# dryman/HashMergeJoin

Measured on AMD Instinct MI355X. Metric: probe-side tuples/s + achieved HBM GB/s, |R|=|S|=2^28 u64 keys, higher is better.
Workload: dtype u64

## Files before the change

hashmergejoin_amd/__init__.py:

```python
from ._lib import (HMJ_BUILD_ANTI, HMJ_BUILD_OUTER, HMJ_BUILD_SEMI, HMJ_CHECKSUM, HMJ_COLS_HASHED, HMJ_COLS_NO_ROW, HMJ_COLS_PACKED, HMJ_FIRST_WINS, HMJ_FULL_OUTER, HMJ_JOIN_ANTI, HMJ_JOIN_INNER, HMJ_JOIN_PROBE_OUTER, HMJ_JOIN_SEMI, HMJ_KIND_BUILD_SIDE, HMJ_KIND_PROBE_SIDE, HMJ_MATERIALIZE, HMJ_ORDERED, HMJ_PATH_CHUNKED_BUILD, HMJ_PATH_DENSE_BUILD,
                   HMJ_PATH_EXACT, HMJ_PATH_GLOBAL_TABLE, HMJ_PATH_HOST_PIPELINE, HMJ_PATH_HOT_KEY_HINT, HMJ_PATH_LOOKBACK_TIMEOUT, HMJ_PATH_ORDER_BY_KEY, HMJ_PATH_ORDER_BY_RANK_SORT, HMJ_PATH_ORDER_DEFERRED, HMJ_PATH_ORDERED_EXPANSION, HMJ_PATH_LDS_TABLE,
                   HMJ_PATH_KEY_RANGES, HMJ_PATH_PREPARED, HMJ_PATH_PRESORTED, HMJ_PATH_RANK_RUNS, HMJ_PATH_SORT_MSD, HMJ_PATH_SLAB, HMJ_PATH_SLAB_ONE_PASS, HMJ_PATH_SLAB_PROBE, HMJ_PATH_SORTED_FK, HMJ_PATH_SORTED_FK_HALF, HMJ_PATH_SORTED_FK_WIDE, HMJ_PATH_SORTED_WRITE, HMJ_PATH_SPLIT, HMJ_PATH_UNIQ_WRITE, HMJ_PATH_WINDOW,
                   HMJ_KEY_FIXED, HMJ_KEY_LARGE_STRING, HMJ_MAX_KEY_COLS, HMJ_MAX_TAKE_COLS, HMJ_STR_NO_ROW, HMJ_SUM_PROBE, HMJ_TAKE_NO_ROW, BuildJoinOpts, ColsJoinOpts, ColsKindOpts, ColsRel, ColsResult, ExchangeKindOpts, HmjError, JoinOpts, JoinResult, KeyCol, KindCounts, MixedCol, MixedOpts, MixedRel, StrJoinOpts, StrKindOpts, StrRel, StrResult, TakeDst, TakeOpts, TakeSrc, TakeStrDst, TakeStrOpts, TakeStrSrc, Timing, Validity,
                   lib_path, load_library)
from .join import Executor, HashMergeJoin, cols_key64, mixed_key64, pack_strings, pack_validity, plan, unpack_strings, unpack_validity

__all__ = ["Executor", "HashMergeJoin", "plan", "HmjError", "JoinResult", "Timing", "load_library",
           "lib_path", "HMJ_MATERIALIZE", "HMJ_ORDERED", "HMJ_FIRST_WINS", "HMJ_CHECKSUM",
           "HMJ_SUM_PROBE", "JoinOpts", "HMJ_JOIN_INNER", "HMJ_JOIN_SEMI", "HMJ_JOIN_ANTI", "HMJ_JOIN_PROBE_OUTER",
           "BuildJoinOpts", "HMJ_BUILD_SEMI", "HMJ_BUILD_ANTI", "HMJ_BUILD_OUTER", "HMJ_FULL_OUTER",
           "ExchangeKindOpts", "KindCounts", "HMJ_KIND_PROBE_SIDE", "HMJ_KIND_BUILD_SIDE",
           "pack_strings", "StrRel", "StrJoinOpts", "StrResult", "StrKindOpts", "HMJ_STR_NO_ROW",
           "KeyCol", "ColsRel", "ColsJoinOpts", "ColsResult", "HMJ_COLS_PACKED", "HMJ_COLS_HASHED", "HMJ_MAX_KEY_COLS",
           "cols_key64", "ColsKindOpts", "HMJ_COLS_NO_ROW", "Validity", "pack_validity",
           "TakeSrc", "TakeDst", "TakeOpts", "HMJ_TAKE_NO_ROW", "HMJ_MAX_TAKE_COLS", "unpack_validity",
           "TakeStrSrc", "TakeStrDst", "TakeStrOpts", "unpack_strings",
           "MixedCol", "MixedRel", "MixedOpts", "HMJ_KEY_FIXED", "HMJ_KEY_LARGE_STRING", "mixed_key64"]
```

hashmergejoin_amd/_lib.py:

```python
import ctypes as C
import os

HMJ_MATERIALIZE = 0x01
HMJ_ORDERED = 0x02
HMJ_FIRST_WINS = 0x04
HMJ_CHECKSUM = 0x08
HMJ_SUM_PROBE = 0x10
HMJ_E_RCCL, HMJ_E_PEER, HMJ_E_TIMEOUT = -6, -7, -8
HMJ_PATH_SLAB, HMJ_PATH_EXACT, HMJ_PATH_UNIQ_WRITE, HMJ_PATH_SPLIT, HMJ_PATH_WINDOW = 0x1, 0x2, 0x4, 0x8, 0x10
HMJ_PATH_ORDER_DEFERRED, HMJ_PATH_ORDER_BY_KEY, HMJ_PATH_PREPARED, HMJ_PATH_CHUNKED_BUILD = 0x20, 0x40, 0x80, 0x100
HMJ_PATH_HOT_KEY_HINT = 0x200
HMJ_PATH_SLAB_PROBE = 0x400
HMJ_PATH_SORTED_WRITE = 0x800
HMJ_PATH_SORTED_FK = 0x1000
HMJ_PATH_DENSE_BUILD = 0x2000
HMJ_PATH_GLOBAL_TABLE = 0x100000
HMJ_PATH_ORDER_BY_RANK_SORT = 0x200000
HMJ_PATH_ORDERED_EXPANSION = 0x400000
HMJ_PATH_LDS_TABLE = 0x800000
HMJ_PATH_RANK_RUNS = 0x1000000
HMJ_PATH_RANK_LOOKUP_IN_PASS = 0x2000000
HMJ_PATH_SORT_MSD = 0x4000000
HMJ_PATH_KEY_RANGES = 0x8000000
HMJ_PATH_SLAB_ONE_PASS = 0x80000
HMJ_PATH_HOST_PIPELINE = 0x4000
HMJ_PATH_SORTED_FK_HALF = 0x8000
HMJ_PATH_LOOKBACK_TIMEOUT = 0x10000
HMJ_PATH_SORTED_FK_WIDE = 0x20000
HMJ_PATH_PRESORTED = 0x40000

_HERE = os.path.dirname(os.path.abspath(__file__))
_U64P = C.POINTER(C.c_uint64)


class HmjError(RuntimeError):
    def __init__(self, code, msg):
        super().__init__("hmj error %d: %s" % (code, msg))
        self.code = code


class JoinResult(C.Structure):
    _fields_ = [("n_matches", C.c_uint64), ("sum_r", C.c_uint64), ("sum_s", C.c_uint64),
                ("xor_fold", C.c_uint64), ("mix_sum", C.c_uint64), ("sum_probe_all", C.c_uint64),
                ("key", C.c_void_p), ("rval", C.c_void_p), ("sval", C.c_void_p)]

    def checks(self):
        return {k: int(getattr(self, k)) for k in ("n_matches", "sum_r", "sum_s", "xor_fold", "mix_sum")}


HMJ_JOIN_INNER, HMJ_JOIN_SEMI, HMJ_JOIN_ANTI, HMJ_JOIN_PROBE_OUTER = 0, 1, 2, 3


class JoinOpts(C.Structure):
    _fields_ = [("struct_size", C.c_uint32), ("kind", C.c_uint32), ("outer_fill", C.c_uint64),
                ("n_probe_matched", C.c_uint64), ("n_probe_unmatched", C.c_uint64)]


HMJ_BUILD_SEMI, HMJ_BUILD_ANTI, HMJ_BUILD_OUTER, HMJ_FULL_OUTER = 1, 2, 3, 4


class BuildJoinOpts(C.Structure):
    _fields_ = [("struct_size", C.c_uint32), ("kind", C.c_uint32), ("build_fill", C.c_uint64), ("probe_fill", C.c_uint64),
# ... 150 lines not shown
                ("radix_bits", C.c_int), ("radix_passes", C.c_int),
                ("n_scatter_launches", C.c_int), ("n_split_retries", C.c_int),
                ("bytes_scatter", C.c_uint64), ("bytes_hist", C.c_uint64),
                ("bytes_probe_count", C.c_uint64), ("bytes_probe_write", C.c_uint64),
                ("path", C.c_uint32), ("key_prefix_bits", C.c_int32), ("key_window_low", C.c_int32),
                ("n_probe_items", C.c_uint32), ("ms_scatter_pass0", C.c_float), ("ms_scatter_pass1", C.c_float)]

    def as_dict(self):
        return {n: getattr(self, n) for n, _ in self._fields_}


class PlanDesc(C.Structure):
    _fields_ = [("struct_size", C.c_uint32), ("path", C.c_uint32), ("radix_bits", C.c_int32), ("radix_passes", C.c_int32),
                ("pass_bits", C.c_int32 * 4), ("key_prefix_bits", C.c_int32), ("key_window_low", C.c_int32),
                ("n_partitions", C.c_uint32), ("probe_items", C.c_uint32), ("attempts", C.c_uint32), ("refused", C.c_uint32),
                ("cooling", C.c_uint32), ("workload", C.c_uint64)]

    def as_dict(self):
        d = {n: getattr(self, n) for n, _ in self._fields_}
        d["pass_bits"] = list(self.pass_bits)
        return d


HMJ_REFUSED_GTABLE_SHAPE, HMJ_REFUSED_GTABLE_COOLING, HMJ_REFUSED_GTABLE_GAVE_UP = 0x1, 0x2, 0x4
HMJ_REFUSED_RANK_SORT_MODEL, HMJ_REFUSED_RANK_SORT_COOLING, HMJ_REFUSED_RANK_SORT_GAVE_UP = 0x8, 0x10, 0x20
HMJ_REFUSED_SLAB_SHAPE, HMJ_REFUSED_SLAB_COOLING, HMJ_REFUSED_SLAB_SORTED_INPUT, HMJ_REFUSED_SLAB_OVERFLOW = 0x40, 0x80, 0x100, 0x200
HMJ_REFUSED_FAST_WRITE_COOLING, HMJ_REFUSED_FAST_WRITE_GAVE_UP = 0x400, 0x800
HMJ_REFUSED_SLAB_PROBE_COOLING, HMJ_REFUSED_SLAB_PROBE_OVERFLOW = 0x1000, 0x2000
HMJ_REFUSED_PREFIX_VIOLATED, HMJ_REFUSED_EXPANSION_GAVE_UP = 0x4000, 0x8000
HMJ_COOL_UNIQ_WRITE, HMJ_COOL_SORTED_WRITE, HMJ_COOL_GTABLE, HMJ_COOL_GTABLE_WRITE = 0x1, 0x2, 0x4, 0x8
HMJ_COOL_RANK_SORT, HMJ_COOL_RANK_SORT_SLAB, HMJ_COOL_EXPANSION, HMJ_COOL_SORT_SLAB = 0x10, 0x20, 0x40, 0x80
HMJ_COOL_SLAB, HMJ_COOL_SLAB_PROBE, HMJ_COOL_ONE_PASS_WRITE, HMJ_COOL_EXACT_PREFIX = 0x100, 0x200, 0x400, 0x800
HMJ_COOL_RANK_RUNS = 0x1000


class PlaceInfo(C.Structure):
    _fields_ = [("name", C.c_char * 16), ("bytes", C.c_uint64), ("fill_TBps", C.c_float), ("candidates", C.c_int),
                ("ms_search", C.c_float), ("searched", C.c_int), ("aborted", C.c_int), ("budget_ms", C.c_float),
                ("cand_ms_alloc", C.c_float * 4), ("cand_ms_fill", C.c_float * 4), ("cand_TBps", C.c_float * 4)]


def lib_path():
    return os.environ.get("HMJ_LIB") or os.path.join(_HERE, "libhmj_hip.so")


class ExchangeInfo(C.Structure):
    _fields_ = [("n_ranks", C.c_int), ("owner_mode", C.c_int), ("rounds_build", C.c_uint32), ("rounds_probe", C.c_uint32),
                ("recv_build", C.c_uint64), ("recv_probe", C.c_uint64), ("ms_split", C.c_float),
                ("ms_exchange_build", C.c_float), ("ms_exchange_probe", C.c_float), ("ms_local", C.c_float),
                ("ms_total", C.c_float), ("digit_bits", C.c_int32), ("digit_low", C.c_int32), ("n_subjoins", C.c_uint32),
                ("fallback", C.c_uint32), ("sample_max_share", C.c_float), ("ms_kernels", C.c_float),
                ("ms_exposed", C.c_float)]

    def as_dict(self):
        return {n: getattr(self, n) for n, _ in self._fields_}


HMJ_MAX_RANKS, HMJ_MAX_ROUNDS = 16, 16


class DigitPlan(C.Structure):
    _fields_ = [("usable", C.c_int32), ("digit_bits", C.c_int32), ("digit_low", C.c_int32), ("n_rounds", C.c_uint32),
                ("owner_first", C.c_uint32 * (HMJ_MAX_RANKS + 1)),
                ("round_first", (C.c_uint32 * (HMJ_MAX_ROUNDS + 1)) * HMJ_MAX_RANKS), ("max_share", C.c_float)]


# ... 149 lines not shown
```

hashmergejoin_amd/csrc/api.hip:

```cpp
#include <hip/hip_runtime.h>
#include <sys/mman.h>

#include <algorithm>
#include <cstdio>
#include <cstdlib>
#include <chrono>
#include <cmath>
#include <cstring>
#include <mutex>
#include <string>
#include <thread>
#include <vector>

#include "hmj_ctx.h"

using hmj::u32;
using hmj::u64;
using namespace hmj_host;

namespace hmj_host {

constexpr int kMaxEvents = 1024;

int fail(hmj_ctx* c, int code, const char* what, hipError_t e) {
// ... 29 lines not shown
  acc->ms_scatter_pass[0] += t.ms_scatter_pass[0];
  acc->ms_scatter_pass[1] += t.ms_scatter_pass[1];
  if (t.radix_passes) {
    acc->radix_bits = t.radix_bits;
    acc->radix_passes = t.radix_passes;
    acc->key_prefix_bits = t.key_prefix_bits;
    acc->key_window_low = t.key_window_low;
  }
  acc->n_probe_items += t.n_probe_items;
}

static int ilog2_u64(uint64_t v) { return v ? 63 - __builtin_clzll(v) : 0; }
uint64_t workload_signature(uint64_t n_build, uint64_t n_probe, uint32_t flags, int kind) {
  const uint32_t mode = ((flags & HMJ_ORDERED) ? 4u : 0u) | ((flags & (HMJ_MATERIALIZE | HMJ_ORDERED)) ? 2u : 0u) |
                        ((flags & HMJ_FIRST_WINS) ? 1u : 0u);
  return ((uint64_t)(kind & 31) << 20) | ((uint64_t)mode << 16) | ((uint64_t)ilog2_u64(n_build) << 8) | (uint64_t)ilog2_u64(n_probe);
}
WorkloadMemo* memo_for(hmj_ctx* c, uint64_t sig) {
  auto it = c->memos.find(sig);
  if (it == c->memos.end()) {
    if (c->memos.size() >= 1024) c->memos.clear();
    it = c->memos.emplace(sig, c->memo_init).first;
  }
  c->wm = &it->second;
  c->wm_sig = sig;
  return c->wm;
}
uint32_t WorkloadMemo::cooling() const {
  return (uniq_cooldown ? HMJ_COOL_UNIQ_WRITE : 0u) | (sorted_cooldown ? HMJ_COOL_SORTED_WRITE : 0u) | (gtable_cooldown ? HMJ_COOL_GTABLE : 0u) |
         (gtable_write_cooldown ? HMJ_COOL_GTABLE_WRITE : 0u) | (gtable_sort_cooldown ? HMJ_COOL_RANK_SORT : 0u) |
         (gtable_sort_slab_cooldown ? HMJ_COOL_RANK_SORT_SLAB : 0u) | (expand_cooldown ? HMJ_COOL_EXPANSION : 0u) |
         (sort_slab_cooldown ? HMJ_COOL_SORT_SLAB : 0u) | (slab_cooldown ? HMJ_COOL_SLAB : 0u) | (slab_probe_cooldown ? HMJ_COOL_SLAB_PROBE : 0u) |
         (one_pass_write_cooldown ? HMJ_COOL_ONE_PASS_WRITE : 0u) | (exact_prefix_joins ? HMJ_COOL_EXACT_PREFIX : 0u) |
         (rank_runs_cooldown ? HMJ_COOL_RANK_RUNS : 0u) | (sort_msd_cooldown ? HMJ_COOL_SORT_MSD : 0u);
}

int wait_arrival(hmj_ctx* c, hipEvent_t ev) {
  if (c->arrive_wait) return c->arrive_wait(c, ev);
  HIP_TRY(hipStreamWaitEvent(c->stream, ev, 0));
  return HMJ_OK;
}

int ensure_dev(hmj_ctx* c, DevBuf& b, size_t bytes) {
  if (bytes <= b.cap) return HMJ_OK;
  if (c && (&b == &c->rbuf[0] || &b == &c->rbuf[1] || &b == &c->r_off || &b == &c->slab_br || &b == &c->cnt_br))
    c->prep.valid = false;
  if (b.p) {
    hipError_t e = hipFree(b.p);
    b.p = nullptr;
    b.cap = 0;
    if (e != hipSuccess) return fail(c, HMJ_E_HIP, "hipFree", e);
  }
  size_t want = bytes + (bytes >> 4) + 256;
#ifdef HMJ_DEV
  if (const char* e = getenv("HMJ_ALLOC_PAD_KB")) want += (size_t)atoll(e) << 10;
  if (const char* e = getenv("HMJ_ALLOC_ROUND_MB")) {
    const size_t g = (size_t)atoll(e) << 20;
    if (g) want = (want + g - 1) / g * g;
  }
#endif
  const auto t_alloc0 = std::chrono::steady_clock::now();
  hipError_t e = hipMalloc(&b.p, want);
  if (e != hipSuccess) {
    b.p = nullptr;
    (void)hipGetLastError();
    return fail(c, HMJ_E_OOM, "hipMalloc", e);
  }
// ... 357 lines not shown
      size_t it = 0;
      for (size_t ci = t; ci < nchunks; ci += T, it++) {
        const int slot = (int)(it & 1);
        hipEvent_t ev = c->up_events[2 * t + slot];
        char* pin = static_cast<char*>(c->up_slots[2 * t + slot].p);
        if (it >= 2 && hipEventSynchronize(ev) != hipSuccess) { status[t] = 1; return; }
        const size_t off = ci * kUpChunk, len = (bytes - off < kUpChunk) ? bytes - off : kUpChunk;
        std::memcpy(pin, static_cast<const char*>(src_host) + off, len);
        if (hipMemcpyAsync(static_cast<char*>(dst_dev) + off, pin, len, hipMemcpyHostToDevice, st) != hipSuccess ||
            hipEventRecord(ev, st) != hipSuccess) { status[t] = 1; return; }
      }
      if (hipStreamSynchronize(st) != hipSuccess) status[t] = 1;
    });
  }
  for (auto& x : th) x.join();
  for (int t = 0; t < T; t++)
    if (status[t]) return fail(c, HMJ_E_HIP, "staged host-to-device copy failed");
  return HMJ_OK;
}

int check_rel(hmj_ctx* c, const void* p, uint64_t n, const char* name) {
  if (n > 0xFFFFFFFFull) return fail(c, HMJ_E_ARG, "more than 2^32-1 rows in one call");
  if (n && !p) return fail(c, HMJ_E_ARG, name);
  if (((uintptr_t)p & 15) != 0) return fail(c, HMJ_E_ARG, "relation pointer must be 16-byte aligned");
  return HMJ_OK;
}

constexpr int kRetryNoWinOrdered = 1003;
constexpr int kRetryNoFastWrite = 1002;
constexpr int kRetryNoSlab = 1001;
constexpr int kRetryNoSlabProbe = 1004;
constexpr int kRetryMoreBits = 1005;
constexpr int kRetryNoPrefix = 1000;

static int read_accum(hmj_ctx* c, u64** h) {
  u64* hh = (u64*)c->h_accum.p;
  HIP_TRY(hipMemcpyAsync(hh, c->accum.p, 8 * sizeof(u64), hipMemcpyDeviceToHost, c->stream));
  HIP_TRY(hipStreamSynchronize(c->stream));
  *h = hh;
  return HMJ_OK;
}
static void result_sums(hmj_result* out, const u64* h) {
  out->n_matches = h[hmj::ACC_N];
  out->sum_r = h[hmj::ACC_SUM_R];
  out->sum_s = h[hmj::ACC_SUM_S];
  out->xor_fold = h[hmj::ACC_XOR];
  out->mix_sum = h[hmj::ACC_MIX];
  out->sum_probe_all = h[hmj::ACC_SUM_P];
}

static int deliver_columns(hmj_ctx* c, hmj_result* out, bool to_host, const void* key, const void* rval, const void* sval,
                           size_t bytes, bool sync_always) {
  if (to_host) {
    RC_TRY(ensure_host(c, c->h_key, bytes, false));
    if (rval) RC_TRY(ensure_host(c, c->h_rval, bytes, false));
    if (sval) RC_TRY(ensure_host(c, c->h_sval, bytes, false));
    const int s = span_begin(c, K_D2H, -1);
    HIP_TRY(hipMemcpyAsync(c->h_key.p, key, bytes, hipMemcpyDeviceToHost, c->stream));
    if (rval) HIP_TRY(hipMemcpyAsync(c->h_rval.p, rval, bytes, hipMemcpyDeviceToHost, c->stream));
    if (sval) HIP_TRY(hipMemcpyAsync(c->h_sval.p, sval, bytes, hipMemcpyDeviceToHost, c->stream));
    span_end(c, s);
  }
  if (to_host || sync_always) HIP_TRY(hipStreamSynchronize(c->stream));
  out->key = (const uint64_t*)(to_host ? c->h_key.p : key);
  out->rval = rval ? (const uint64_t*)(to_host ? c->h_rval.p : rval) : nullptr;
  out->sval = sval ? (const uint64_t*)(to_host ? c->h_sval.p : sval) : nullptr;
// ... 623 lines not shown

static int run_slab_join(hmj_ctx* c, const JoinCall& j, const JoinPlan& p) {
  const bool materialize = j.materialize(), first = j.first(), extra = j.extra();
  const u32 nb = j.nb, np = j.np, np_plan = p.np_plan, P = p.P;
  const int* pass_bits = p.pass_bits;
  hmj::SlabGeom gr, gs;
  if (p.allow_slab && c->slab_mode && c->wm->slab_cooldown == 0 && !c->prepare_only && !(c->timing.path & HMJ_PATH_SLAB) &&
      !((!materialize || p.fast_write) && p.Q == 1 && p.probe_fits && p.passes == 2 && pass_bits[0] <= hmj::SLAB_MAX_BITS &&
        pass_bits[1] <= hmj::SLAB_MAX_BITS && p.dense_scale <= 2.5))
    c->plan.refused |= HMJ_REFUSED_SLAB_SHAPE;
  if (!(p.allow_slab && c->slab_mode && c->wm->slab_cooldown == 0 && (!materialize || p.fast_write) && p.Q == 1 &&
        p.probe_fits &&
        p.passes == 2 && pass_bits[0] <= hmj::SLAB_MAX_BITS && pass_bits[1] <= hmj::SLAB_MAX_BITS &&
        slab_sizes_ok(c, nb, np_plan, materialize || np_plan < nb) &&
        p.dense_scale <= 2.5 &&
        hmj::slab_geometry(nb, pass_bits[0], pass_bits[1], &gr, 0, 1.0, p.dense_scale) &&
        hmj::slab_geometry(np_plan, pass_bits[0], pass_bits[1], &gs, 0,
                           (nb && np_plan > nb) ? (double)np_plan / (double)nb : 1.0, p.dense_scale)))
    return kPlanNotTaken;
  const bool reuse = c->prep.valid && c->prep.slab && c->prep.ptr == j.R && c->prep.n == nb &&
                     c->prep.low == p.low && c->prep.B == p.B;
  c->prep.valid = false;
  c->timing.path |= HMJ_PATH_SLAB | (reuse ? HMJ_PATH_PREPARED : 0u);
  c->timing.n_probe_items = P;
  const int ba = pass_bits[0], bb = pass_bits[1];
  const u64 rows_a = gr.rows_a > gs.rows_a ? gr.rows_a : gs.rows_a;
  const u32 wa = gr.WA > gs.WA ? gr.WA : gs.WA;
  RC_TRY(ensure_dev(c, c->slab_a, rows_a * 16));
  RC_TRY(ensure_dev(c, c->cnt_a, ((size_t)wa << ba) * 4));
  RC_TRY(ensure_dev(c, c->slab_br, gr.rows_b * 16));
  RC_TRY(ensure_dev(c, c->slab_bs, gs.rows_b * 16));
  RC_TRY(ensure_dev(c, c->cnt_br, (size_t)P * gr.KB * 4));
  RC_TRY(ensure_dev(c, c->cnt_bs, (size_t)P * gs.KB * 4));
  if (!reuse) RC_TRY(slab_passes(c, j.R, nb, 0, p.low, ba, bb, gr, c->slab_br, c->cnt_br, false));
  if (!c->prepare_only) RC_TRY(slab_passes(c, j.S, np, 1, p.low, ba, bb, gs, c->slab_bs, c->cnt_bs, !c->arrive_ev.empty()));
  u64* hh;
  if (c->prepare_only) {
    RC_TRY(read_accum(c, &hh));
    if (hh[hmj::ACC_ERR] & hmj::ERR_SLAB) {
      c->wm->slab_cooldown = 8;
      return kRetryNoSlab;
    }
    c->prep.valid = true;
    c->prep.slab = true;
    c->prep.ptr = j.R;
    c->prep.n = nb;
    c->prep.low = p.low;
    c->prep.B = p.B;
    return HMJ_OK;
  }
  hmj::ProbeArgs sa = slab_probe_args(c, &gr, nullptr, c->slab_bs, c->cnt_bs, gs.CB, P, 1);
  if (p.fast_write)
    return unique_key_write(c, sa, true, nb, np, p.low, extra, p.verify_pfx ? p.prefix : 0, p.pfx_ref, j.ordered(), j.to_host,
                            p.fk_wide_plan, p.dense_scale, j.out);
#ifdef HMJ_DEV
  sa.debug = c->dev_ablate;
#endif
  int sp = span_begin(c, K_PROBE_COUNT, -1);
  if (first || extra) {
    sa.extra = (extra ? 1u : 0u) | (first ? 2u : 0u);
    HIP_TRY(hmj::launch_probe_count_ext(sa, nullptr, nullptr, true, c->num_cus, c->stream));
  } else {
    HIP_TRY(hmj::launch_probe_count_slab(sa, c->num_cus, c->stream));
  }
  span_end(c, sp);
  c->timing.bytes_probe_count = 16ull * ((u64)nb + np);
  RC_TRY(read_accum(c, &hh));
// ... 1170 lines not shown
  p.path = c->timing.path;
  p.radix_bits = c->timing.radix_bits;
  p.radix_passes = c->timing.radix_passes;
  p.key_prefix_bits = c->timing.key_prefix_bits;
  p.key_window_low = c->timing.key_window_low;
  p.n_partitions = (c->timing.path & (HMJ_PATH_GLOBAL_TABLE | HMJ_PATH_LDS_TABLE)) ? 0u : (p.radix_bits < 32 ? 1u << p.radix_bits : 0u);
  p.probe_items = c->timing.n_probe_items;
  p.cooling = c->wm->cooling();
  p.workload = c->wm_sig;
  return rc;
}
static int join_device_planned(hmj_ctx* c, const void* R, uint64_t n_build, const void* S, uint64_t n_probe, uint32_t flags,
                               hmj_result* out, bool to_host) {
  const bool kinds = c->join_kind != 0;
  if (!kinds) {
    bool done = false;
    int rc = try_global_table(c, R, n_build, S, n_probe, flags, out, to_host, &done);
    if (rc != HMJ_OK || done) return rc;
    rc = try_small_build_ordered(c, R, n_build, S, n_probe, flags, out, to_host, &done);
    if (rc != HMJ_OK || done) return rc;
  }
  bool auto_prefix = true, slab = !kinds, fast_write = !kinds, win_ordered = true, prefix_unsafe = false, slab_probe = !kinds;
  if ((flags & HMJ_ORDERED) && c->wm->exact_prefix_joins > 0) {
    c->wm->exact_prefix_joins--;
    prefix_unsafe = true;
  }
  bool forced_here = false;
  struct Unforce {
    hmj_ctx* c;
    bool* on;
    ~Unforce() {
      if (*on) c->force_bits = -1;
      c->expand_allow_rebits = true;
    }
  } unforce{c, &forced_here};
  for (int attempt = 0; attempt < 8; attempt++) {
    c->plan.attempts = (uint32_t)attempt + 1;
    int rc = join_device_impl(c, R, n_build, S, n_probe, flags, out, to_host, auto_prefix, slab, fast_write,
                              win_ordered, prefix_unsafe, slab_probe);
    c->plan.refused |= rc == kRetryNoSlab ? HMJ_REFUSED_SLAB_OVERFLOW : rc == kRetryNoPrefix ? HMJ_REFUSED_PREFIX_VIOLATED
                       : rc == kRetryNoFastWrite ? HMJ_REFUSED_FAST_WRITE_GAVE_UP : rc == kRetryNoSlabProbe ? HMJ_REFUSED_SLAB_PROBE_OVERFLOW
                       : rc == kRetryMoreBits ? HMJ_REFUSED_EXPANSION_GAVE_UP : 0u;
    if (c->trace)
      std::fprintf(stderr, "[hmj] join nb=%llu np=%llu flags=%#x attempt %d: rc=%d bits=%d passes=%d path=%#x prefix=%d low=%d items=%u%s\n",
                   (unsigned long long)n_build, (unsigned long long)n_probe, flags, attempt, rc, c->timing.radix_bits,
                   c->timing.radix_passes, c->timing.path, c->timing.key_prefix_bits, c->timing.key_window_low,
                   c->timing.n_probe_items,
                   rc == kRetryNoSlab ? " -> retry without the slab path (a slab overflowed)"
                   : rc == kRetryNoPrefix ? " -> retry: a row outside the sampled key prefix"
                   : rc == kRetryNoFastWrite ? " -> retry without the unique-key write mode"
                   : rc == kRetryNoWinOrdered ? " -> retry without the key window"
                   : rc == kRetryNoSlabProbe ? " -> retry without probe-side slabs (one overflowed)"
                   : rc == kRetryMoreBits ? " -> retry with one more radix bit (a partition did not fit the ordered expansion)" : "");
    if (rc == kRetryNoSlab || rc == kRetryNoPrefix || rc == kRetryNoFastWrite || rc == kRetryNoWinOrdered || rc == kRetryNoSlabProbe ||
        rc == kRetryMoreBits) {
      std::vector<Span> keep;
      for (const Span& sp : c->spans)
        if (sp.kind == K_TOTAL || sp.kind == K_H2D) keep.push_back(sp);
      c->spans.swap(keep);
      std::memset(&c->timing, 0, sizeof(c->timing));
      if (rc == kRetryNoSlab) slab = false;
      else if (rc == kRetryMoreBits) {
        c->force_bits = c->expand_rebits;
        c->expand_allow_rebits = false;
        forced_here = true;
      }
      else if (rc == kRetryNoSlabProbe) slab_probe = false;
      else if (rc == kRetryNoFastWrite) fast_write = false;
      else if (rc == kRetryNoWinOrdered) win_ordered = false;
      else if (!prefix_unsafe && win_ordered) {
        prefix_unsafe = true;
        c->wm->exact_prefix_joins = 32;
      }
      else auto_prefix = false;
      continue;
    }
    return rc;
  }
  return fail(c, HMJ_E_HIP, "join could not be planned");
}

int prepare_build(hmj_ctx* c, const void* R, uint64_t n_build, uint64_t n_probe_hint) {
  hmj_result dummy;
  c->prepare_only = true;
  c->probe_hint = n_probe_hint;
  c->prep.valid = false;
  const int rc = join_device(c, R, n_build, nullptr, 0, 0, &dummy, false);
  c->prepare_only = false;
  return rc;
}

int join_device_kind(hmj_ctx* c, const JoinKind& k, const void* R, uint64_t n_build, const void* S, uint64_t n_probe,
                     uint32_t flags, hmj_result* out, hmj_kind_counts* counts) {
  std::memset(counts, 0, sizeof(*counts));
// ... 16 lines not shown
    const u64 unmatched = k.kind == HMJ_JOIN_SEMI ? n_probe - out->n_matches : filled;
    counts->n_probe_matched = n_probe - unmatched;
    counts->n_probe_unmatched = unmatched;
  } else {
    const u64 b_unmatched = k.kind == HMJ_BUILD_SEMI ? n_build - swept : swept;
    counts->n_build_matched = n_build - b_unmatched;
    counts->n_build_unmatched = b_unmatched;
    if (k.kind == HMJ_FULL_OUTER) {
      counts->n_probe_matched = n_probe - filled;
      counts->n_probe_unmatched = filled;
    }
  }
  return HMJ_OK;
}

}

extern "C" {

int hmj_create(hmj_ctx** out, int device_id) {
  if (!out) return HMJ_E_ARG;
  *out = nullptr;
  int ndev = 0;
  if (hipGetDeviceCount(&ndev) != hipSuccess || ndev <= 0) {
    (void)hipGetLastError();
    return HMJ_E_NODEV;
  }
  if (device_id < 0 && hipGetDevice(&device_id) != hipSuccess) return HMJ_E_NODEV;
  if (device_id >= ndev) return HMJ_E_ARG;
  if (hipSetDevice(device_id) != hipSuccess) return HMJ_E_NODEV;
  hmj_ctx* c = new hmj_ctx();
  c->device = device_id;
  if (const char* e = getenv("HMJ_SLAB")) c->slab_mode = atoi(e);
  if (const char* e = getenv("HMJ_ONE_PASS_SLAB")) c->one_pass_slab = atoi(e) != 0;
  if (const char* e = getenv("HMJ_GTABLE")) c->gtable_mode = atoi(e) != 0;
  if (const char* e = getenv("HMJ_RANK_RUNS")) c->rank_runs_mode = atoi(e) != 0;
  if (const char* e = getenv("HMJ_RANK_RUNS_MAX_CUT")) c->rank_runs_max_cut = atoi(e) < 0 ? 0 : atoi(e) > 16 ? 16 : atoi(e);
  if (const char* e = getenv("HMJ_RANK_RUNS_MAX_GROUP")) c->rank_runs_max_group = atoi(e) < 0 ? 0 : atoi(e) > 4 ? 4 : atoi(e);
  if (const char* e = getenv("HMJ_PROMOTE_TO_ORDERED")) c->promote_to_ordered = atoi(e) != 0;
  if (const char* e = getenv("HMJ_KEY_RANGES")) c->key_ranges = atoi(e) != 0;
  if (const char* e = getenv("HMJ_KEY_RANGES_FORCE")) c->key_ranges_force = atoi(e) < 0 ? 0 : atoi(e) > 4 ? 4 : atoi(e);
  if (const char* e = getenv("HMJ_RANK_RUNS_WAVE")) c->rank_runs_wave = atoi(e) != 0;
  if (const char* e = getenv("HMJ_RANK_RUNS_MAX_LEVEL")) c->rank_runs_max_level = atoi(e) < 0 ? 0 : atoi(e) > 2 ? 2 : atoi(e);
  if (const char* e = getenv("HMJ_GTABLE_SORT")) c->gtable_sort_mode = atoi(e) != 0;
  if (const char* e = getenv("HMJ_EXPAND_FK_FANOUT")) c->expand_fk_fanout = atoi(e) > 0 ? (u32)atoi(e) : 0u;
  if (const char* e = getenv("HMJ_SORT_MSD")) c->sort_msd = atoi(e) != 0;
  if (const char* e = getenv("HMJ_SORT_MSD_MEAN")) c->sort_msd_mean = atof(e) >= 64.0 ? atof(e) : c->sort_msd_mean;
  if (const char* e = getenv("HMJ_SORT_MSD_MAX_BITS")) c->sort_msd_max_bits = atoi(e) < 2 ? 2 : atoi(e) > 18 ? 18 : atoi(e);
  if (const char* e = getenv("HMJ_SORT_MSD_MIN_LOG2")) {
    const int l = atoi(e);
    if (l >= 16 && l <= 32) c->sort_msd_min = 1ull << l;
  }
  if (const char* e = getenv("HMJ_SORT_SLAB_MIN_LOG2")) {
    const int l = atoi(e);
    if (l >= 12 && l <= 32) c->sort_slab_min = 1ull << l;
  }
  if (const char* e = getenv("HMJ_GTABLE_SORT_SLAB_MIN_LOG2")) {
    const int l = atoi(e);
    if (l >= 12 && l <= 32) c->gtable_sort_slab_min = 1ull << l;
  }
  if (const char* e = getenv("HMJ_GTABLE_SORT_FANOUT")) c->gtable_sort_fanout = atoi(e) > 0 ? (u32)atoi(e) : 1u;
  if (const char* e = getenv("HMJ_PLACE")) {
    c->place_tune = atoi(e) != 0;
    if (atoi(e) > 0) {
      c->place_tries = atoi(e);
      c->place_search_always = true;
// ... 858 lines not shown
```

hashmergejoin_amd/csrc/hmj_ctx.h:

```cpp
#pragma once
#include <hip/hip_runtime.h>

#include <string>
#include <unordered_map>
#include <vector>

#include "../../include/hmj.h"
#include "hmj_dev.h"
#include "hmj_launch.h"

struct hmj_comm;

namespace hmj_host {

struct DevBuf {
  void* p = nullptr;
  size_t cap = 0;
};
struct HostBuf {
  void* p = nullptr;
  size_t cap = 0;
  bool pinned = true;
};

// ... 15 lines not shown
    for (DevBuf* b : {&rows_r, &rows_s, &flags, &blk, &blk_off, &list, &runs, &acc, &mark_r, &mark_s, &amb, &cmp_r, &cmp_s, &vblk}) f(*b);
    each_result_buf(f);
  }
};

enum Kind {
  K_TOTAL = 0, K_H2D, K_D2H, K_HIST, K_SCAN, K_SCATTER, K_OFFSETS, K_PROBE_COUNT, K_OUT_SCAN,
  K_PROBE_WRITE, K_ORDER, K_NKINDS
};
struct Span {
  int kind, rel, e0, e1;
  int pass;
};

struct WorkloadMemo {
  int uniq_cooldown = 0;
  int sorted_cooldown = 0;
  bool sorted_chained = false;
  bool sorted_wide = true;
  bool sorted_fk = false;
  int sorted_fk_age = 0;
  int gtable_cooldown = 0;
  int gtable_write_cooldown = 0;
  int gtable_sort_cooldown = 0;
  int gtable_sort_slab_cooldown = 0;
  int rank_runs_cooldown = 0;
  int rank_lookup_cooldown = 0;
  int expand_cooldown = 0;
  int sort_slab_cooldown = 0;
  int sort_msd_cooldown = 0;
  int slab_cooldown = 0;
  int slab_probe_cooldown = 0;
  int one_pass_write_cooldown = 0;
  int exact_prefix_joins = 0;
  uint32_t cooling() const;
};

}

namespace hmj_host {
struct OrderedCostModel {
  double part_fixed_ms = 0.15;
  double part_ns = 0.030, part_ns_per_f = 0.00023;
  double part_bucket_ns = 0.043, part_bucket_ns_per_f = 0.0001;
  double part_epilogue_ns = 0.25;
  double comp_fixed_ms = 0.65;
  double comp_ns_chain = 0.060, comp_ns_exact = 0.072;
  double comp_ns_wide = 0.145;
  double comp_ns_beyond_l2 = 0.02;
  double runs_fixed_ms = 0.25, runs_ns = 0.0215, runs_ns_per_run = 7.5;
  double runs_ns_per_log2_build = 0.0023;
  double runs_wave_ns_per_run = 1.2, runs_wave_ns = 0.007;
  double runs_range_ns = 0.0;
};
}

struct hmj_ctx {
  using DevBuf = hmj_host::DevBuf;
  using HostBuf = hmj_host::HostBuf;
  using Span = hmj_host::Span;
  using WorkloadMemo = hmj_host::WorkloadMemo;
  using u32 = hmj::u32;
  using u64 = hmj::u64;
  int device = 0, num_cus = 256;
  hipStream_t own_stream = nullptr, stream = nullptr;
  DevBuf rbuf[2], sbuf[2], in_r, in_s, hist, totals, r_off, s_off, part_count, part_out_off, accum,
// ... 54 lines not shown
  uint64_t gtable_max_rows = 1ull << 17;
  u32 gtable_min_fanout = 0;
  uint64_t gtable_min_probe = 1;
  int gtable_wg_per_cu = 8;
  u32 gtable_slots_per_row = 16;
  int gtable_max_log_cap = 18;
  bool ltable_mode = true;
  bool gtable_sort_mode = true;
  u32 gtable_sort_fanout = 128;
  bool rank_runs_mode = true;
  int rank_runs_max_cut = 10;
  int rank_runs_max_group = 3;
  int rank_runs_max_level = 2;
  uint64_t big_join_rows = 1ull << 29;
  bool promote_to_ordered = true;
  bool key_ranges = true;
  int key_ranges_force = 0;
  bool rank_runs_wave = true;
  bool build_sort_msd = true;
  bool gtable_sort_slab = true;
  u64 gtable_sort_slab_min = 1ull << 25;
  bool expand_mode = true;
  u32 fk_payload_buckets = 24;
  u32 expand_fk_fanout = 0;
  bool expand_allow_rebits = true;
  int expand_rebits = 0;
  bool sort_msd = true;
  double sort_msd_mean = 1200.0;
  int sort_msd_max_bits = 18;
  u64 sort_msd_min = 1ull << 22;
  bool sort_slab = true;
  u64 sort_slab_min = 1ull << 25;
  int slab_mode = 1;
  bool staged_upload = false;
  bool host_pipeline = true;
  hipStream_t copy_stream = nullptr;
  std::vector<hipEvent_t> copy_ev;
  bool split_mode = true;
  bool window_mode = true;
  u32 slab_min_rows = 1u << 21;
  u32 slab_probe_kb = 0;
  bool one_pass_slab = true;
  int scatter_variant = 1;
  bool profiling = false;
  bool trace = false;
#ifdef HMJ_DEV
  u32 dev_ablate = 0;
#endif
  std::vector<hipEvent_t> events;
  std::vector<Span> spans;
  int ev_used = 0;
  hmj_timing timing;
  std::string last_error;
  hmj_comm* comm = nullptr;
  std::vector<u64> arrive_rows;
  std::vector<hipEvent_t> arrive_ev;
  bool sample_build_only = false;
  int (*arrive_wait)(hmj_ctx*, hipEvent_t) = nullptr;
};


namespace hmj_host {
int fail(hmj_ctx* c, int code, const char* what, hipError_t e = hipSuccess);
#define HIP_TRY(expr)                                                        \
  do {                                                                       \
    hipError_t _e = (expr);                                                  \
// ... 38 lines not shown
```

hashmergejoin_amd/csrc/hmj_dev.h:

```cpp
#pragma once
#include <hip/hip_runtime.h>
#include <stdint.h>

namespace hmj {

typedef unsigned long long u64;
typedef unsigned int u32;
typedef unsigned short u16;

struct __attribute__((aligned(16))) Tup {
  u64 key;
  u64 val;
};

constexpr int kWave = 64;
#ifndef HMJ_SCAN_DPP
#define HMJ_SCAN_DPP 1
#endif

#ifndef HMJ_STREAM_POLICY
#define HMJ_STREAM_POLICY 2
#endif
typedef u64 u64x2_t __attribute__((ext_vector_type(2)));
__device__ __forceinline__ void store_stream(Tup* p, const Tup& v) {
// ... 51 lines not shown
          slot[r] = (slot[r] + 1) & mask;
          any_live = true;
        }
      }
    }
  }
}

constexpr int RP_THREADS = 512;
constexpr int RP_WAVES = RP_THREADS / kWave;
constexpr int RP_ITEMS = 8;
constexpr int RP_TILE = RP_THREADS * RP_ITEMS;
constexpr int RP_MAX_BITS = 9;
constexpr int RP_MAXD = 1 << RP_MAX_BITS;
constexpr int RP_MAX_BLOCKS = 2048;

constexpr int PB_THREADS = 1024;
constexpr int PB_CAP = 5120;
constexpr int PB_LOG_NB = 12;
constexpr int PB_TARGET_AVG = 4096;
constexpr int PB_PLAN_SLACK = 256;

constexpr int SLAB_KB = 4;
constexpr int SLAB_MAX_BITS = 9;

enum { ACC_N = 0, ACC_SUM_R, ACC_SUM_S, ACC_XOR, ACC_MIX, ACC_SUM_P, ACC_ERR, ACC_PAD };
constexpr u64 ERR_SLAB = 2;
constexpr u64 ERR_ORDER_DEFER = 16;
constexpr u64 ERR_ORDER_FAIL = 32;
constexpr u64 ERR_SORTED = 64;
constexpr u64 ERR_FASTPATH = 8;
constexpr u64 ERR_GTABLE = 128;
constexpr u64 ERR_PREFIX = 4;

__device__ __forceinline__ u64 mix64(u64 x) {
  x ^= x >> 30;
  x *= 0xBF58476D1CE4E5B9ull;
  x ^= x >> 27;
  x *= 0x94D049BB133111EBull;
  x ^= x >> 31;
  return x;
}

__device__ __forceinline__ u64 tmix(u64 key, u64 rval, u64 sval) {
  u64 t = mix64(key);
  t = mix64(t ^ rval);
  t = mix64(t + sval);
  return t;
}

__device__ __forceinline__ int lane_id() {
  return __builtin_amdgcn_mbcnt_hi(~0u, __builtin_amdgcn_mbcnt_lo(~0u, 0u));
}

__device__ __forceinline__ u32 popc_below(u64 m) {
  return __builtin_amdgcn_mbcnt_hi((u32)(m >> 32), __builtin_amdgcn_mbcnt_lo((u32)m, 0u));
}

__device__ __forceinline__ u32 wave_incl_scan_u32(u32 v, int ) {
#if HMJ_SCAN_DPP
  v += (u32)__builtin_amdgcn_update_dpp(0, (int)v, 0x111, 0xF, 0xF, false);
  v += (u32)__builtin_amdgcn_update_dpp(0, (int)v, 0x112, 0xF, 0xF, false);
  v += (u32)__builtin_amdgcn_update_dpp(0, (int)v, 0x114, 0xF, 0xF, false);
  v += (u32)__builtin_amdgcn_update_dpp(0, (int)v, 0x118, 0xF, 0xF, false);
  v += (u32)__builtin_amdgcn_update_dpp(0, (int)v, 0x142, 0xA, 0xF, false);
  v += (u32)__builtin_amdgcn_update_dpp(0, (int)v, 0x143, 0xC, 0xF, false);
// ... 72 lines not shown
```

hashmergejoin_amd/csrc/hmj_launch.h:

```cpp
#pragma once
#include <hip/hip_runtime.h>
#include <stddef.h>
#include <stdint.h>

#include <atomic>

namespace hmj {
typedef unsigned long long u64;
typedef unsigned int u32;

struct SmemAttrOnce {
  std::atomic<unsigned long long> devices{0};
};
inline hipError_t ensure_max_smem(SmemAttrOnce& once, const void* kernel, size_t bytes) {
  int dev = 0;
  hipError_t e = hipGetDevice(&dev);
  if (e != hipSuccess) return e;
  const unsigned long long bit = 1ull << (dev & 63);
  if (dev < 64 && (once.devices.load(std::memory_order_acquire) & bit)) return hipSuccess;
  e = hipFuncSetAttribute(kernel, hipFuncAttributeMaxDynamicSharedMemorySize, (int)bytes);
  if (e != hipSuccess) return e;
  if (dev < 64) once.devices.fetch_or(bit, std::memory_order_release);
  return hipSuccess;
}

constexpr int kMaxRanks = 16;
struct OwnerFn {
  u32 mode;
  u32 G;
  u64 spl[kMaxRanks - 1];
};
int radix_tile_rows(int bits, int variant);
void radix_pass_geometry(u32 n, int tile, u32* nblk, u32* rows_per_block);
size_t radix_scatter_smem_bytes();
hipError_t launch_radix_hist(const void* in, u32 n, int tile, int shift, int bits, u32* hist,
                             u32 nblk, u32 rows_per_block, hipStream_t st, const OwnerFn* own = nullptr);
hipError_t launch_owner_scatter(const void* in, void* out, u32 n, int bits, const OwnerFn& own,
                                const u32* hist_scanned, const u32* totals, u32 nblk, u32 rows_per_block,
                                u64* offsets_out, hipStream_t st);
hipError_t launch_radix_rowscan(u32* hist, u32 nblk, int bits, u32* totals, hipStream_t st);
hipError_t launch_radix_scatter(const void* in, void* out, u32 n, int variant, int shift, int bits,
                                const u32* hist_scanned, const u32* totals, u32 nblk,
                                u32 rows_per_block, u64* offsets_out, hipStream_t st);
struct SlabGeom {
  u32 WA, rpw, CA, CB, KB;
  u64 rows_a, rows_b;
};
bool slab_geometry(u32 n, int bits_a, int bits_b, SlabGeom* g, u32 kb = 0, double fan = 1.0, double density = 1.0);
bool slab_geometry_one_pass(u32 n, int bits, double keys_per_digit, u32 max_workers, SlabGeom* g, double density = 1.0);
u32 slab_capacity(double mean, double fan);
hipError_t launch_slab_a(const void* in, u32 n, int shift, int bits, const SlabGeom& g, void* slab_a, u64 slab_a_rows,
                         u32* cnt_a, u64 cnt_a_n, u64* accum, hipStream_t st, u32 w_begin = 0, u32 w_end = 0xFFFFFFFFu);
hipError_t launch_slab_b(const void* slab_a, const u32* cnt_a, int bits_a, int shift, int bits,
                         const SlabGeom& g, void* slab_b, u64 slab_b_rows, u32* cnt_b, u64 cnt_b_n, u64* accum, hipStream_t st);
hipError_t launch_key_sample(const void* R, u32 nb, const void* S, u32 np, u64* out, hipStream_t st);
hipError_t launch_key_exact(const void* R, u32 nb, const void* S, u32 np, u64 ref, u64* out, int num_cus, hipStream_t st,
                            bool ref_is_first_key = false);
hipError_t launch_check_partitioned(const void* a, u32 n, int low, int bits, u32* flag, int num_cus, hipStream_t st);
hipError_t launch_part_offsets(const void* a, u32 n, int low, int bits, u32* off, hipStream_t st);

struct ProbeArgs {
  const void* R;
  const u32* r_off;
  const void* S;
  const u32* s_off;
  u32 P;
  u32 Q;
  u64* part_count;
  const u64* part_out_off;
  u64* out_key;
  u64* out_rval;
  u64* out_sval;
  u64 out_cap;
  u64* accum;
  const u32* item_list;
  const u32* n_item_list;
  const u32* r_cnt;
  const u32* s_cnt;
  u32 r_cap, s_cap;
  u32 s_wa, s_ppi;
  u64 r_cnt_n, s_cnt_n;
  u64 r_rows, s_rows;
  const u64* item_base;
  const u32* r_end;
  const u32* s_end;
  u32 extra;
  u32 pfx_shift;
  u64 pfx_val;
  u32* matched;
  u32 debug;
};
hipError_t launch_probe(const ProbeArgs& a, int mode, bool first_wins, bool extra, int grid,
                        hipStream_t st);
int probe_default_grid(int num_cus);
hipError_t launch_probe_kind(const ProbeArgs& a, int mode, int kind, bool first_wins, u64 fill, int grid, hipStream_t st);
hipError_t launch_probe_build_kind(const ProbeArgs& a, int mode, int kind, u64 fill, u32* bmark, int grid, hipStream_t st);
hipError_t launch_build_sweep(const ProbeArgs& a, const u32* r_off, u32 P, const u32* vstart, u64* sweep_n, int mode,
                              bool set, u64 fill, int num_cus, hipStream_t st);
hipError_t launch_probe_count_ext(const ProbeArgs& a, u32* irregular, u32* n_irregular, bool slab,
                                  int num_cus, hipStream_t st);
hipError_t launch_probe_count_slab(const ProbeArgs& a, int num_cus, hipStream_t st);
hipError_t launch_probe_write_sorted(const ProbeArgs& a, bool slab, bool fk, int shape, u64* lookback, bool chained, int key_low,
                                     int num_cus, hipStream_t st);
hipError_t launch_probe_write_uniq(const ProbeArgs& a, bool slab, int num_cus, hipStream_t st);
hipError_t launch_slab_np(const u32* cnt, u32 P, u64* out, hipStream_t st);
hipError_t launch_probe_count_fast(const ProbeArgs& a, u32* irregular, u32* n_irregular, bool big,
                                   bool per_partition_counts, int num_cus, hipStream_t st);
hipError_t launch_scan_u64(const u64* in, u64* out_excl, u32 n, hipStream_t st);
hipError_t launch_probe_expand_ordered(const ProbeArgs& a, int key_low, int num_cus, hipStream_t st);
hipError_t launch_order(const u64* part_out_off, const u32* vstart, const u32* in_base32, const u64* in_base64, u32 P, u32 Q,
                        int low, const u64* akey, const u64* arval, const u64* asval, u64* bkey, u64* brval,
                        u64* bsval, u64* accum, u32 defer_rows, bool many_per_key, int grid, hipStream_t st);
hipError_t launch_compact(const u64* part_out_off, const u32* in_base32, const u64* in_base64, u32 P, const u64* akey,
                          const u64* arval, const u64* asval, u64* bkey, u64* brval, u64* bsval, int grid, hipStream_t st);
hipError_t launch_rekey(void* pairs, u64 n, const u64* col, hipStream_t st);

hipError_t launch_gtable_build(const void* R, u32 nb, void* tab, int log_cap, u64* accum, bool first, int num_cus,
                               hipStream_t st);
hipError_t launch_gtable_probe(const void* S, u32 np, const void* tab, int log_cap, const void* R, u64* accum, bool first,
                               bool extra, int num_cus, int wg_per_cu, hipStream_t st);
hipError_t launch_gtable_write(const void* S, u32 np, const void* tab, int log_cap, const void* R, u64* accum, u64* out_key,
                               u64* out_rval, u64* out_sval, bool first, bool extra, int num_cus, int wg_per_cu, hipStream_t st);

hipError_t launch_ltable_probe(const void* R, u32 nb, const void* S, u32 np, u64* accum, bool first, bool extra, int num_cus, hipStream_t st);
int ltable_max_rows();
hipError_t launch_sval_range(const void* S, u32 np, u64* out2 , int num_cus, hipStream_t st,
                             u32 every = 1 );
hipError_t launch_gtable_emit(const void* S, u32 np, const void* tab, int log_cap, u64 svmin, int range_bits, u64* accum,
                              void* pairs, bool extra, bool wide, int num_cus, int wg_per_cu, hipStream_t st);
hipError_t launch_gtable_swap(const void* in, void* out, u64 n, int num_cus, hipStream_t st);
hipError_t launch_gtable_emit_ranks(const void* S, u32 np, const void* tab, int log_cap, u64* accum, void* pairs, bool extra, int num_cus,
                                    int wg_per_cu, hipStream_t st);
int rank_sort_max_run(int level = 0);
hipError_t launch_sort_runs_write(const void* slabs, const u32* cnt, u32 cap, u32 P, const u64* out_off, void* out, u64* accum, int level,
// ... 36 lines not shown
```

hashmergejoin_amd/csrc/probe.hip:

```cpp
#include "hmj_dev.h"
#include "hmj_launch.h"
#include <type_traits>

namespace hmj {

constexpr u32 PB_NB = 1u << PB_LOG_NB;
constexpr u32 NIL = 0xFFFFu;
static_assert(PB_CAP < 0xFFFF, "chain links are 16-bit");

struct ProbeSmem {
  u64 key[PB_CAP];
  u64 val[PB_CAP];
  u32 head[PB_NB];
  u32 aux[PB_CAP];
  u16 next[PB_CAP];
  u32 scratch[PB_THREADS / kWave + 1];
  u64 pcount;
  u64 red[8];
  u64 obase;
  u32 wtot[PB_THREADS / kWave];
  u32 nslot;
};
constexpr u32 PB_BATCH = 2 * PB_THREADS;
static_assert(PB_BATCH <= PB_CAP, "a batch must fit an empty table");
// ... 860 lines not shown
};

template <int LOG_NB>
__device__ __forceinline__ u32 fast_hash(u64 k) {
  u32 x = (u32)k ^ ((u32)(k >> 32) * 0x85EBCA6Bu);
  x *= 0x9E3779B1u;
  return x >> (32 - LOG_NB);
}

template <int THREADS, int ROWS = FP_ROWS>
__device__ __forceinline__ void fp_load(Tup (&t)[ROWS], const Tup* __restrict__ base, u32 n,
                                        int tid) {
#pragma unroll
  for (int k = 0; k < ROWS; k++) {
    u32 i = k * THREADS + tid;
    t[k] = base[i < n ? i : n - 1];
  }
}

static_assert(SLAB_KB == 4, "fp_load_slab / fp_load_pieces / slab_np_kernel unroll exactly four pieces per partition");
template <int THREADS, int ROWS = FP_ROWS>
__device__ __forceinline__ void fp_load_slab(Tup (&t)[ROWS], const Tup* __restrict__ base, u32 cap,
                                             u32 p1, u32 p2, u32 p3, u32 n, int tid) {
#pragma unroll
  for (int k = 0; k < ROWS; k++) {
    u32 i = k * THREADS + tid;
    i = i < n ? i : n - 1;
    const u32 j = (i >= p1) + (i >= p2) + (i >= p3);
    const u32 pre = j == 0 ? 0u : (j == 1 ? p1 : (j == 2 ? p2 : p3));
    t[k] = base[(u64)j * cap + (i - pre)];
  }
}

template <int THREADS>
__device__ __forceinline__ void fp_load_pieces(Tup (&t)[FP_ROWS], const Tup* __restrict__ base, u32 cap, u32 cnt_mine, int tid) {
  constexpr int QT = THREADS / 4;
  const u32 g = (u32)tid / QT, l = (u32)tid % QT;
  const Tup* __restrict__ piece = base + (u64)g * cap;
  const u32 last = cnt_mine ? cnt_mine - 1 : 0;
#pragma unroll
  for (int k = 0; k < FP_ROWS; k++) {
    const u32 r = l + (u32)k * QT;
    t[k] = piece[r < last ? r : last];
  }
}

template <int THREADS, int LOG_NB, bool PCOUNT, bool SLAB, int OUT>
__global__ __launch_bounds__(THREADS, 4) void probe_count_fast_kernel(
    ProbeArgs a, u32* __restrict__ irregular, u32* __restrict__ n_irregular) {
  typedef FastSmem<THREADS, LOG_NB> Smem;
  constexpr u32 CAP = Smem::CAP, NB = 1u << LOG_NB;
  constexpr bool PIECES = SLAB && OUT == 0 && !PCOUNT && HMJ_PROBE_PIECES;
  constexpr u32 QT = THREADS / 4, PIECE_CAP = FP_ROWS * QT;
  extern __shared__ __attribute__((aligned(16))) unsigned char smem_raw[];
  Smem& sm = *reinterpret_cast<Smem*>(smem_raw);
  const Tup* __restrict__ R = static_cast<const Tup*>(a.R);
  const Tup* __restrict__ S = static_cast<const Tup*>(a.S);
  const u32* __restrict__ r_off = a.r_off;
  const u32* __restrict__ s_off = a.s_off;
  const u32* __restrict__ r_end = (SLAB || a.r_end == nullptr) ? a.r_off + 1 : a.r_end;
  const u32* __restrict__ s_end = (SLAB || a.s_end == nullptr) ? a.s_off + 1 : a.s_end;
  const u32 P = a.P;
  const int tid = threadIdx.x;
  u64 acc_n = 0, acc_r = 0, acc_s = 0, acc_x = 0, acc_m = 0, acc_p = 0;
  bool pfx_bad = false, giveup = false;
  for (u32 i = tid; i < NB; i += THREADS) sm.head[i] = 0;
  if (tid < 2) sm.itemcnt[tid] = 0;
  u32 epoch = 0;
  u32 prev_p = 0xFFFFFFFFu, parity = 0;

  u32 p = blockIdx.x;
  u32 rb = 0, nb = 0, sb = 0, np = 0;
  bool regular = false;
  Tup br[FP_ROWS], pr[FP_ROWS], pq[FP_ROWS];
  u32 r1 = 0, r2 = 0, r3 = 0, s1 = 0, s2 = 0, s3 = 0, r1n = 0, r2n = 0, r3n = 0, s1n = 0, s2n = 0, s3n = 0;
  u32 rm = 0, sm_ = 0, rmn = 0, smn = 0;
  const u32 my_piece = (u32)tid / QT;
  bool slab_bad = false;
  if (p < P) {
    if (SLAB) {
      const u32* rc = a.r_cnt + (u64)p * SLAB_KB;
      const u32* sc = a.s_cnt + (u64)p * SLAB_KB;
      r1 = rc[0]; r2 = r1 + rc[1]; r3 = r2 + rc[2]; nb = r3 + rc[3];
      s1 = sc[0]; s2 = s1 + sc[1]; s3 = s2 + sc[2]; np = s3 + sc[3];
      if (nb > CAP || np > CAP) slab_bad = true;
      if (PIECES) {
        rm = my_piece == 0 ? rc[0] : my_piece == 1 ? rc[1] : my_piece == 2 ? rc[2] : rc[3];
        sm_ = my_piece == 0 ? sc[0] : my_piece == 1 ? sc[1] : my_piece == 2 ? sc[2] : sc[3];
        if (rc[0] > PIECE_CAP || rc[1] > PIECE_CAP || rc[2] > PIECE_CAP || rc[3] > PIECE_CAP || sc[0] > PIECE_CAP ||
            sc[1] > PIECE_CAP || sc[2] > PIECE_CAP || sc[3] > PIECE_CAP) {
          slab_bad = true;
          nb = CAP + 1;
        }
      }
    } else {
      rb = r_off[p]; nb = r_end[p] - rb;
      sb = s_off[p]; np = s_end[p] - sb;
    }
    regular = nb && np && nb <= CAP && np <= CAP;
    if (regular) {
      if (PIECES) {
        fp_load_pieces<THREADS>(br, R + (u64)p * SLAB_KB * a.r_cap, a.r_cap, rm, tid);
        fp_load_pieces<THREADS>(pr, S + (u64)p * SLAB_KB * a.s_cap, a.s_cap, sm_, tid);
      } else if (SLAB) {
        fp_load_slab<THREADS>(br, R + (u64)p * SLAB_KB * a.r_cap, a.r_cap, r1, r2, r3, nb, tid);
        if (OUT == 0) fp_load_slab<THREADS>(pr, S + (u64)p * SLAB_KB * a.s_cap, a.s_cap, s1, s2, s3, np, tid);
      } else {
        fp_load<THREADS>(br, R + rb, nb, tid);
        if (OUT == 0) fp_load<THREADS>(pr, S + sb, np, tid);
      }
    }
  }
  const Tup* __restrict__ dummy = reinterpret_cast<const Tup*>(a.accum);
  auto load_build = [&](Tup (&t)[FP_ROWS], bool ok, u32 pp, u32 rb_, u32 nb_, u32 q1, u32 q2, u32 q3, u32 mine) {
    if (PIECES)
      fp_load_pieces<THREADS>(t, ok ? R + (u64)pp * SLAB_KB * a.r_cap : dummy, ok ? a.r_cap : 0u, ok ? mine : 1u, tid);
    else if (SLAB)
      fp_load_slab<THREADS>(t, ok ? R + (u64)pp * SLAB_KB * a.r_cap : dummy, ok ? a.r_cap : 0u, ok ? q1 : 1u, ok ? q2 : 1u,
                            ok ? q3 : 1u, ok ? nb_ : 1u, tid);
    else
      fp_load<THREADS>(t, ok ? R + rb_ : dummy, ok ? nb_ : 1u, tid);
  };
  auto load_probe = [&](Tup (&t)[FP_ROWS], bool ok, u32 pp, u32 sb_, u32 np_, u32 q1, u32 q2, u32 q3, u32 mine) {
    if (PIECES)
      fp_load_pieces<THREADS>(t, ok ? S + (u64)pp * SLAB_KB * a.s_cap : dummy, ok ? a.s_cap : 0u, ok ? mine : 1u, tid);
    else if (SLAB)
      fp_load_slab<THREADS>(t, ok ? S + (u64)pp * SLAB_KB * a.s_cap : dummy, ok ? a.s_cap : 0u, ok ? q1 : 1u, ok ? q2 : 1u,
                            ok ? q3 : 1u, ok ? np_ : 1u, tid);
    else
      fp_load<THREADS>(t, ok ? S + sb_ : dummy, ok ? np_ : 1u, tid);
  };
  const int tid_outer = tid;
  while (p < P) {
    int tid = tid_outer;
    if constexpr (OUT != 0) asm volatile("" : "+v"(tid));
    u64 out_base = (u64)sb;
    if constexpr (OUT == 1 && SLAB) {
      const u64* ibp = a.item_base + p;
      asm volatile("s_load_dwordx2 %0, %1, 0x0\n\ts_waitcnt lgkmcnt(0)" : "=s"(out_base) : "s"(ibp) : "memory");
    }
    const u32 pn = __builtin_amdgcn_readfirstlane(p + gridDim.x);
    u32 rb2 = 0, nb2 = 0, sb2 = 0, np2 = 0;
    bool regular2 = false;
    if (pn < P) {
      if (SLAB) {
        const u32* rc = a.r_cnt + (u64)pn * SLAB_KB;
        const u32* sc = a.s_cnt + (u64)pn * SLAB_KB;
        r1n = rc[0]; r2n = r1n + rc[1]; r3n = r2n + rc[2]; nb2 = r3n + rc[3];
        s1n = sc[0]; s2n = s1n + sc[1]; s3n = s2n + sc[2]; np2 = s3n + sc[3];
        if (nb2 > CAP || np2 > CAP) slab_bad = true;
        if (PIECES) {
          rmn = my_piece == 0 ? rc[0] : my_piece == 1 ? rc[1] : my_piece == 2 ? rc[2] : rc[3];
          smn = my_piece == 0 ? sc[0] : my_piece == 1 ? sc[1] : my_piece == 2 ? sc[2] : sc[3];
          if (rc[0] > PIECE_CAP || rc[1] > PIECE_CAP || rc[2] > PIECE_CAP || rc[3] > PIECE_CAP || sc[0] > PIECE_CAP ||
              sc[1] > PIECE_CAP || sc[2] > PIECE_CAP || sc[3] > PIECE_CAP) {
            slab_bad = true;
            nb2 = CAP + 1;
          }
        }
      } else {
        rb2 = r_off[pn]; nb2 = r_end[pn] - rb2;
        sb2 = s_off[pn]; np2 = s_end[pn] - sb2;
      }
      regular2 = nb2 && np2 && nb2 <= CAP && np2 <= CAP;
    }
    if (OUT == 0) {
      load_probe(pq, regular2, pn, sb2, np2, s1n, s2n, s3n, smn);
    } else if (regular) {
      if (SLAB)
        fp_load_slab<THREADS>(pr, S + (u64)p * SLAB_KB * a.s_cap, a.s_cap, s1, s2, s3, np, tid);
      else
        fp_load<THREADS>(pr, S + sb, np, tid);
    }
    if (regular) {
      lds_barrier();
      if (PCOUNT && prev_p != 0xFFFFFFFFu && tid == 0) {
        a.part_count[prev_p] = sm.itemcnt[parity ^ 1];
        sm.itemcnt[parity ^ 1] = 0;
      }
      if (PCOUNT) prev_p = 0xFFFFFFFFu;
      epoch++;
      if (epoch == 0x10000u) {
        for (u32 i = tid; i < NB; i += THREADS) sm.head[i] = 0;
        epoch = 1;
        lds_barrier();
      }
      const u32 tag = epoch << 16;
      if (!HMJ_ABLATE(1u)) {
        u32 old[FP_ROWS];
#pragma unroll
        for (int k = 0; k < FP_ROWS; k++) {
          const u32 i = k * THREADS + tid;
          old[k] = tag | NIL;
          if (PIECES ? ((u32)tid % QT + (u32)k * QT < rm) : (i < nb)) {
            if (a.pfx_shift && (br[k].key >> a.pfx_shift) != a.pfx_val) pfx_bad = true;
            sm.key[i] = br[k].key;
            sm.val[i] = br[k].val;
            old[k] = atomicExch(&sm.head[fast_hash<LOG_NB>(br[k].key)], tag | i);
          }
        }
#pragma unroll
        for (int k = 0; k < FP_ROWS; k++) {
          const u32 i = k * THREADS + tid;
          if (PIECES ? ((u32)tid % QT + (u32)k * QT < rm) : (i < nb)) sm.next[i] = ((old[k] >> 16) == epoch) ? (u16)old[k] : (u16)NIL;
        }
      } else {
#pragma unroll
        for (int k = 0; k < FP_ROWS; k++) acc_r += br[k].key;
      }
      load_build(br, regular2, pn, rb2, nb2, r1n, r2n, r3n, rmn);
      lds_barrier();
      const u64 n_before = acc_n;
      if (!HMJ_ABLATE(1u)) {
        u32 cur[FP_ROWS];
        u32 cnt[FP_ROWS], first[FP_ROWS];
#pragma unroll
        for (int k = 0; k < FP_ROWS; k++) {
          const u32 j = k * THREADS + tid;
          cur[k] = NIL;
          cnt[k] = 0;
          first[k] = OUT == 2 ? NIL : 0;
          if (PIECES ? ((u32)tid % QT + (u32)k * QT < sm_) : (j < np)) {
            if (a.pfx_shift && (pr[k].key >> a.pfx_shift) != a.pfx_val) pfx_bad = true;
            if (OUT >= 1 && (a.extra & 1u)) acc_p += pr[k].val;
            const u32 hv = sm.head[fast_hash<LOG_NB>(pr[k].key)];
            cur[k] = ((hv >> 16) == epoch) ? (hv & 0xFFFFu) : NIL;
          }
        }
        for (; !HMJ_ABLATE(2u);) {
          bool any = false;
#pragma unroll
          for (int k = 0; k < FP_ROWS; k++) any |= (cur[k] != NIL);
          if (!__any(any)) break;
#pragma unroll
          for (int k = 0; k < FP_ROWS; k++) {
            if (cur[k] != NIL) {
              const u32 i = cur[k];
              const u64 kk = sm.key[i], vv = sm.val[i];
              cur[k] = sm.next[i];
              if (kk == pr[k].key) {
                if (OUT == 2 && (a.extra & 2u)) {
                  first[k] = i < first[k] ? i : first[k];
                } else {
                  acc_n++;
                  acc_r += vv;
                  acc_s += pr[k].val;
                  if (OUT == 1) {
                    if (cnt[k] == 0) first[k] = i;
                    cnt[k]++;
                  }
                  if (OUT >= 1 && (a.extra & 1u)) {
                    const u64 m = tmix(kk, vv, pr[k].val);
                    acc_x ^= m;
                    acc_m += m;
                  }
                }
              }
            }
          }
        }
        if (OUT == 2 && (a.extra & 2u)) {
#pragma unroll
          for (int k = 0; k < FP_ROWS; k++) {
            if (first[k] != NIL) {
              const u64 vv = sm.val[first[k]];
              acc_n++;
              acc_r += vv;
              acc_s += pr[k].val;
              if (a.extra & 1u) {
                const u64 m = tmix(pr[k].key, vv, pr[k].val);
                acc_x ^= m;
                acc_m += m;
              }
            }
          }
        }
        if (OUT == 1) {
          u64 packed = 0;
          bool cx = false;
#pragma unroll
          for (int k = 0; k < FP_ROWS; k++) {
            cx |= cnt[k] > 1;
            packed |= (u64)(cnt[k] ? 1u : 0u) << (12 * k);
          }
          const int lane = tid & 63, wv = tid >> 6;
          const bool wave_dup = __any(cx);
          u64 incl = packed;
#pragma unroll
          for (int o = 1; o < kWave; o <<= 1) {
            u64 t = __shfl_up(incl, o, kWave);
            if (lane >= o) incl += t;
          }
          if (lane == 63) {
            sm.wscan[wv] = incl;
            sm.wdup[wv] = wave_dup ? 1u : 0u;
          }
          lds_barrier();
          u64 pre = 0, tot = 0;
          u32 dup = 0;
#pragma unroll
          for (int q = 0; q < THREADS / kWave; q++) {
            const u64 ws = sm.wscan[q];
            dup |= sm.wdup[q];
            if (q < wv) pre += ws;
            tot += ws;
          }
          const u64 ex = pre + incl - packed;
          if (dup) {
            giveup = true;
          } else {
            u64 o = out_base;
            u32 total = 0;
#pragma unroll
            for (int k = 0; k < FP_ROWS; k++) {
              if (cnt[k]) {
                const u64 d = o + ((ex >> (12 * k)) & 0xFFFu);
                a.out_key[d] = pr[k].key;
                a.out_rval[d] = sm.val[first[k]];
                a.out_sval[d] = pr[k].val;
              }
              const u32 tk = (u32)((tot >> (12 * k)) & 0xFFFu);
              o += tk;
              total += tk;
            }
            if (tid == 0) a.part_count[p] = total;
          }
        }
      } else {
#pragma unroll
        for (int k = 0; k < FP_ROWS; k++) acc_r += pr[k].key;
      }
      if (PCOUNT) {
        const u32 mine = (u32)(acc_n - n_before);
        const u32 ws = (u32)wave_sum_u64(mine);
        if ((tid & 63) == 0 && ws) atomicAdd(&sm.itemcnt[parity], ws);
        prev_p = p;
        parity ^= 1;
      }
    } else {
      if ((PCOUNT || OUT == 1) && tid == 0 && !(nb && np)) a.part_count[p] = 0;
      if (OUT == 1 && nb && np) giveup = true;
      if (OUT >= 1 && (a.extra & 1u) && !nb) {
        if (SLAB) {
          const Tup* base = S + (u64)p * SLAB_KB * a.s_cap;
          for (u32 j = tid; j < np; j += THREADS) {
            const u32 pc = (j >= s1) + (j >= s2) + (j >= s3);
            const u32 pre = pc == 0 ? 0 : pc == 1 ? s1 : pc == 2 ? s2 : s3;
            acc_p += base[(u64)pc * a.s_cap + (j - pre)].val;
          }
        } else {
          for (u32 j = tid; j < np; j += THREADS) acc_p += S[sb + j].val;
        }
      }
      if (OUT != 1 && !SLAB && tid == 0 && nb && np) irregular[atomicAdd(n_irregular, 1u)] = p;
      load_build(br, regular2, pn, rb2, nb2, r1n, r2n, r3n, rmn);
    }
    if (OUT == 0) {
#pragma unroll
      for (int k = 0; k < FP_ROWS; k++) pr[k] = pq[k];
    }
    p = pn; rb = rb2; nb = nb2; sb = sb2; np = np2; regular = regular2;
    r1 = r1n; r2 = r2n; r3 = r3n; s1 = s1n; s2 = s2n; s3 = s3n;
    rm = rmn; sm_ = smn;
  }
  if (SLAB && slab_bad && tid == 0) atomicOr(&a.accum[ACC_ERR], ERR_SLAB);
  if (OUT == 1 && __any(giveup) && (tid & 63) == 0) atomicOr(&a.accum[ACC_ERR], ERR_FASTPATH);
  if (__any(pfx_bad) && (tid & 63) == 0) atomicOr(&a.accum[ACC_ERR], ERR_PREFIX);
  lds_barrier();
  if (PCOUNT && prev_p != 0xFFFFFFFFu && tid == 0) a.part_count[prev_p] = sm.itemcnt[parity ^ 1];
  if (tid < 8) sm.red[tid] = 0;
  lds_barrier();
  const u64 v[6] = {acc_n, acc_r, acc_s, acc_x, acc_m, acc_p};
  block_accumulate(sm.red, a.accum, v, 1u << ACC_XOR);
}

constexpr int SW_LOGB = 12, SW_NB = 1 << SW_LOGB, SW_MAXBUCKET = 32;
constexpr u64 LB_AGG = 1ull << 62, LB_PFX = 2ull << 62, LB_MASK = (1ull << 62) - 1;
constexpr u32 LB_SPIN_LIMIT = 1u << 22;

template <int THREADS>
struct SortedSmem {
  static constexpr int CAP = THREADS * FP_ROWS, CAPB = CAP, LOGB = SW_LOGB;
  u64 key[CAP];
  u64 val[CAP];
  u64 sval[CAP];
  u32 cnt[SW_NB];
  u16 bstart[SW_NB + 2];
  u16 perm[CAP];
  u32 mbits[2][CAP / 32];
  u32 scratch[THREADS / kWave + 1];
  u32 tick[2];
  u32 flag;
  u64 obase;
  u64 red[8];
};

constexpr int SWF_LOGB = 11, SWF_CAPB = 4608, SWF_MAXDUP = 1024;
constexpr int SWF_HALF_THREADS = 512, SWF_HALF_ROWS = 6, SWF_HALF_CAPB = 2048, SWF_HALF_LOGB = 10;
constexpr int SWF_WIDE_ROWS = 6, SWF_WIDE_CAPB = 2560;
template <int THREADS, int ROWS = FP_ROWS, int CAPB_ = SWF_CAPB, int LOGB_ = SWF_LOGB>
// ... 1094 lines not shown
      vr_beg[v] = rb + b;
      vr_end[v] = rb + e;
    }
    if (ns == 1) {
      vs_beg[v] = sb;
      vs_end[v] = sb + np;
    } else {
      const u32 step = (np + ns - 1) / ns;
      const u32 b = qs * step, e = (b + step < np) ? b + step : np;
      vs_beg[v] = sb + (b < np ? b : np);
      vs_end[v] = sb + e;
    }
  }
}
hipError_t launch_split_parts(const u32* r_off, const u32* s_off, u32 P, u32 thr_rows, u32 slice_rows, u32 build_thr,
                              u32 build_slice, u32 cap_v, u32* vstart, u32* vr_beg, u32* vr_end, u32* vs_beg,
                              u32* vs_end, u32* nv_out, hipStream_t st) {
  hipLaunchKernelGGL(split_count_kernel, dim3(1), dim3(1024), 0, st, r_off, s_off, P, thr_rows, slice_rows, build_thr,
                     build_slice, cap_v, vstart, nv_out);
  hipLaunchKernelGGL(split_fill_kernel, dim3((cap_v + 255) / 256), dim3(256), 0, st, r_off, s_off, P, thr_rows,
                     slice_rows, build_thr, build_slice, cap_v, vstart, vr_beg, vr_end, vs_beg, vs_end);
  return hipGetLastError();
}

template <int MODE, bool FIRST, bool EXTRA>
static hipError_t launch_probe_t(const ProbeArgs& a, int grid, hipStream_t st) {
  static SmemAttrOnce attr_once;
  if (hipError_t e = ensure_max_smem(attr_once, reinterpret_cast<const void*>(probe_kernel<MODE, FIRST, EXTRA>), (size_t)sizeof(ProbeSmem)); e != hipSuccess) return e;
  hipLaunchKernelGGL((probe_kernel<MODE, FIRST, EXTRA>), dim3(grid), dim3(PB_THREADS),
                     sizeof(ProbeSmem), st, a);
  return hipGetLastError();
}

template <int THREADS, int LOG_NB, bool PCOUNT, bool SLAB = false, int OUT = 0>
static hipError_t launch_fast_t(const ProbeArgs& a, u32* irregular, u32* n_irregular, int grid,
                                hipStream_t st) {
  typedef FastSmem<THREADS, LOG_NB> Smem;
  static SmemAttrOnce attr_once;
  if (hipError_t e = ensure_max_smem(attr_once, reinterpret_cast<const void*>(probe_count_fast_kernel<THREADS, LOG_NB, PCOUNT, SLAB, OUT>), (size_t)sizeof(Smem)); e != hipSuccess) return e;
  if ((u32)grid > a.P) grid = (int)a.P;
  if (grid < 1) grid = 1;
  hipLaunchKernelGGL((probe_count_fast_kernel<THREADS, LOG_NB, PCOUNT, SLAB, OUT>), dim3(grid), dim3(THREADS),
                     sizeof(Smem), st, a, irregular, n_irregular);
  return hipGetLastError();
}

hipError_t launch_probe_count_fast(const ProbeArgs& a, u32* irregular, u32* n_irregular, bool big,
                                   bool per_partition_counts, int num_cus, hipStream_t st) {
  if (per_partition_counts) {
    if (big) return launch_fast_t<1024, BIG_LOG_NB, true>(a, irregular, n_irregular, num_cus * 4, st);
    return launch_fast_t<512, 11, true>(a, irregular, n_irregular, num_cus * 3 * 4, st);
  }
  if (big) return launch_fast_t<1024, BIG_LOG_NB, false>(a, irregular, n_irregular, num_cus * 4, st);
  return launch_fast_t<512, 11, false>(a, irregular, n_irregular, num_cus * 3 * 4, st);
}

static bool slab_operands_ok(const ProbeArgs& a) {
  const u64 pieces = (u64)a.P * SLAB_KB;
  return a.r_cnt && a.s_cnt && a.r_cnt_n >= pieces && a.s_cnt_n >= pieces && a.r_rows >= pieces * a.r_cap &&
         a.s_rows >= pieces * a.s_cap;
}

hipError_t launch_probe_write_uniq(const ProbeArgs& a, bool slab, int num_cus, hipStream_t st) {
  if (slab && !slab_operands_ok(a)) return hipErrorInvalidValue;
  if (slab) return launch_fast_t<1024, BIG_LOG_NB, false, true, 1>(a, nullptr, nullptr, num_cus * 4, st);
  return launch_fast_t<1024, BIG_LOG_NB, false, false, 1>(a, nullptr, nullptr, num_cus * 4, st);
}

template <bool SLAB, bool FK, bool EXTRA, bool PB = false>
static hipError_t launch_sorted_t(const ProbeArgs& a, u64* lookback, bool chained, int key_low, int grid, hipStream_t st) {
  typedef typename std::conditional<FK, SortedFkSmem<1024>, SortedSmem<1024>>::type Smem;
  static_assert(sizeof(Smem) <= 160 * 1024, "one workgroup's LDS");
  if constexpr (FK && !PB) {
    if (a.extra & 4u) return launch_sorted_t<SLAB, FK, EXTRA, true>(a, lookback, chained, key_low, grid, st);
  }
// ... 38 lines not shown
  if (grid < 1) grid = 1;
  if (fk && shape == 1)
    return launch_sorted_shape<SWF_HALF_THREADS, SWF_HALF_ROWS, SWF_HALF_CAPB, SWF_HALF_LOGB>(a, slab, lookback, chained, key_low, grid, st);
  if (fk && shape == 2)
    return launch_sorted_shape<1024, SWF_WIDE_ROWS, SWF_WIDE_CAPB, SWF_LOGB>(a, slab, lookback, chained, key_low, grid, st);
  if (slab) return fk ? launch_sorted_x<true, true>(a, lookback, chained, key_low, grid, st)
                      : launch_sorted_x<true, false>(a, lookback, chained, key_low, grid, st);
  return fk ? launch_sorted_x<false, true>(a, lookback, chained, key_low, grid, st)
            : launch_sorted_x<false, false>(a, lookback, chained, key_low, grid, st);
}

__global__ void slab_np_kernel(const u32* __restrict__ cnt, u32 P, u64* __restrict__ out) {
  u32 p = blockIdx.x * blockDim.x + threadIdx.x;
  if (p < P) {
    const u32* q = cnt + (u64)p * SLAB_KB;
    out[p] = (u64)q[0] + q[1] + q[2] + q[3];
  }
}
hipError_t launch_slab_np(const u32* cnt, u32 P, u64* out, hipStream_t st) {
  hipLaunchKernelGGL(slab_np_kernel, dim3((P + 255) / 256), dim3(256), 0, st, cnt, P, out);
  return hipGetLastError();
}

hipError_t launch_probe_count_ext(const ProbeArgs& a, u32* irregular, u32* n_irregular, bool slab,
                                  int num_cus, hipStream_t st) {
  if (slab && !slab_operands_ok(a)) return hipErrorInvalidValue;
  if (slab) return launch_fast_t<1024, BIG_LOG_NB, false, true, 2>(a, nullptr, nullptr, num_cus * 4, st);
  return launch_fast_t<1024, BIG_LOG_NB, false, false, 2>(a, irregular, n_irregular, num_cus * 4, st);
}

hipError_t launch_probe_count_slab(const ProbeArgs& a, int num_cus, hipStream_t st) {
  if (!slab_operands_ok(a)) return hipErrorInvalidValue;
  return launch_fast_t<1024, BIG_LOG_NB, false, true>(a, nullptr, nullptr, num_cus * 4, st);
}

hipError_t launch_probe(const ProbeArgs& a, int mode, bool first_wins, bool extra, int grid,
                        hipStream_t st) {
  if (!a.item_list && (u64)grid > (u64)a.P * a.Q) grid = (int)((u64)a.P * a.Q);
  if (grid < 1) grid = 1;
  if (a.s_ppi) {
    if (!a.s_cnt || (mode != 0 && mode != 3) || (mode == 3 && (!a.out_key || !a.out_rval || !a.out_sval || a.out_cap == 0)) || (first_wins && !a.matched) || a.s_wa == 0 || (u64)a.P * a.s_wa * a.s_cap > 0xFFFFFFFFull || (u64)a.Q * a.s_ppi < a.s_wa || (u64)(a.Q - 1) * a.s_ppi >= a.s_wa ||
        a.s_cnt_n < (u64)a.P * a.s_wa || a.s_rows < (u64)a.P * a.s_wa * a.s_cap)
      return hipErrorInvalidValue;
  } else if (a.s_cnt && (a.s_cnt_n < (u64)a.P * a.Q || a.s_rows < (u64)a.P * a.Q * a.s_cap || (u64)a.P * a.Q * a.s_cap > 0xFFFFFFFFull))
    return hipErrorInvalidValue;
#define HMJ_DISPATCH(M)                                                          \
  if (first_wins)                                                                \
    return extra ? launch_probe_t<M, true, true>(a, grid, st)                    \
                 : launch_probe_t<M, true, false>(a, grid, st);                  \
  else                                                                           \
    return extra ? launch_probe_t<M, false, true>(a, grid, st)                   \
                 : launch_probe_t<M, false, false>(a, grid, st);
  if (mode == 3 && !a.s_ppi) return hipErrorInvalidValue;
  if (mode == 0) {
    HMJ_DISPATCH(0)
  } else if (mode == 3) {
    HMJ_DISPATCH(3)
  } else if (mode == 1) {
    HMJ_DISPATCH(1)
  } else {
    if (first_wins) return launch_probe_t<2, true, false>(a, grid, st);
    return launch_probe_t<2, false, false>(a, grid, st);
  }
#undef HMJ_DISPATCH
}

// ... 426 lines not shown
```

hashmergejoin_amd/csrc/radix.hip:

```cpp
#include <cstdlib>
#include <cstring>

#include <type_traits>

#include "hmj_dev.h"
#include "hmj_launch.h"

namespace hmj {

template <int OWN>
__device__ __forceinline__ u32 owner_digit(u64 key, int shift, u32 mask, const OwnerFn& f) {
  if (OWN == 1) return (u32)__umul64hi(mix64(key), (u64)f.G);
  if (OWN == 2) {
    u32 d = 0;
#pragma unroll
    for (int i = 0; i < kMaxRanks - 1; i++) d += ((u32)i + 1 < f.G && key >= f.spl[i]) ? 1u : 0u;
    return d;
  }
  return (u32)(key >> shift) & mask;
}

template <int OWN>
__global__ __launch_bounds__(RP_THREADS) void radix_hist_kernel(const Tup* __restrict__ in, u32 n,
                                                                int shift, u32 mask,
// ... 176 lines not shown
#pragma unroll
    for (int h = 0; h < 2; h++) {
      Tup v[RP_ITEMS / 2];
#pragma unroll
      for (int r = 0; r < RP_ITEMS / 2; r++) {
        const u32 i = (h * (RP_ITEMS / 2) + r) * RP_THREADS + tid;
        if (FULL || i < tile_n) v[r] = sm.stage[i];
      }
      if (h == 0) {
#pragma unroll
        for (int r = 0; r < RP_ITEMS / 2; r++) {
          Tup z;
          z.key = 0;
          z.val = 0;
          sm.stage[r * RP_THREADS + tid] = z;
        }
      }
#pragma unroll
      for (int r = 0; r < RP_ITEMS / 2; r++) {
        const u32 i = (h * (RP_ITEMS / 2) + r) * RP_THREADS + tid;
        if (FULL || i < tile_n) {
          const u32 d = OWN ? owner_digit<OWN>(v[r].key, shift, mask, own) : digit_of<HI>(v[r].key, shift, mask);
          store_stream(&out[sm.delta[d] + i], v[r]);
        }
      }
    }
    for (int i = tid; i < RP_WAVES * RP_MAXD / 2; i += RP_THREADS)
      reinterpret_cast<u32*>(&sm.wcnt[0][0])[i] = 0;
    lds_barrier();
  }
}

constexpr int WC_ITEMS = 4;
constexpr int WC_LINE = 8;

#ifndef HMJ_WC_PLAN1
#define HMJ_WC_PLAN1 0
#endif
#ifndef HMJ_WC_FULLTILE
#define HMJ_WC_FULLTILE 1
#endif
#ifndef HMJ_WC_NOBAR5
#define HMJ_WC_NOBAR5 1
#endif
#ifdef HMJ_STAMPS
__device__ unsigned long long g_wc_stamps[32];
struct WcStamps {
  u32 acc[14];
  u64 last;
  int base;
  __device__ __forceinline__ void begin() {
    asm volatile("s_waitcnt vmcnt(0)" ::: "memory");
    last = __builtin_amdgcn_s_memtime();
  }
  __device__ __forceinline__ void mark(int i) {
    const u64 now = __builtin_amdgcn_s_memtime();
    acc[i] += (u32)(now - last);
    last = now;
  }
  __device__ __forceinline__ void flush() {
    if ((threadIdx.x & 63) == 0)
      for (int i = 0; i < 14; i++) atomicAdd(&g_wc_stamps[base + i], (unsigned long long)acc[i]);
  }
};
#define WC_STAMP_ARG , WcStamps& stamps
#define WC_STAMP_PASS , stamps
#define WC_MARK(i) stamps.mark(i)
#define WC_VMWAIT() asm volatile("s_waitcnt vmcnt(0)" ::: "memory")
#else
#define WC_STAMP_ARG
#define WC_STAMP_PASS
#define WC_MARK(i)
#define WC_VMWAIT()
#endif

template <int THREADS, int MAXD>
struct WcSmem {
  static constexpr int TILE = THREADS * WC_ITEMS;
  static constexpr int WAVES = THREADS / kWave;
  static constexpr int ZROWS = WAVES * MAXD * 8 / 16;
  static constexpr int MAXLINES = TILE / WC_LINE + 2 * MAXD;
  static_assert(ZROWS <= TILE && ZROWS % THREADS == 0, "lane masks must alias whole row slabs");
  static_assert(MAXD <= THREADS && MAXD * WC_LINE == TILE, "one digit per thread; carry == tile slots");
  union {
    Tup stage[TILE];
    u64 lanemask[WAVES][MAXD];
  };
  Tup carry[MAXD][WC_LINE];
  u16 wcnt[WAVES][MAXD];
  u32 tile_off[MAXD];
  u32 cflush[MAXD];
  static constexpr bool HAS_CF_TILE = MAXD <= 256;
  u32 cf_tile[HAS_CF_TILE ? MAXD : 1];
  u32 plan[MAXD];
  u32 pend[MAXD];
  u32 line_off[MAXD];
  u16 line_tab[MAXLINES];
  u32 total_lines;
  u32 scratch[WAVES + 1];
};

struct NoLimit {
  __device__ __forceinline__ u32 operator()(u32) const { return 0xFFFFFFFFu; }
};
template <int THREADS, int MAXD, bool HI, bool ALLVALID, bool LIMIT, typename Prefetch, typename Limit>
__device__ __forceinline__ void wc_tile(WcSmem<THREADS, MAXD>& sm, Tup (&t)[WC_ITEMS], u32 tile_n,
                                        Tup* __restrict__ out, int shift, u32 mask, u32 D,
                                        Prefetch&& prefetch, const Limit& limit, bool* ovf WC_STAMP_ARG) {
  typedef WcSmem<THREADS, MAXD> Smem;
  constexpr int WAVES = Smem::WAVES;
  const int tid = threadIdx.x, lane = tid & 63, w = tid >> 6;
  u16* wc = &sm.wcnt[w][0];
  u64* lm = &sm.lanemask[w][0];
  const u64 lanebit = 1ull << lane;
  const u32 wbase = (u32)w * (WC_ITEMS * 64) + lane;

  u32 dr[WC_ITEMS];
#ifdef HMJ_STAMPS
  stamps.last = __builtin_amdgcn_s_memtime();
  WC_VMWAIT();
  WC_MARK(0);
  stamps.acc[11]++;
#endif
#pragma unroll
  for (int r = 0; r < WC_ITEMS; r++) {
    u32 d = 0, rank = 0;
    if (ALLVALID || wbase + r * 64 < tile_n) {
      d = digit_of<HI>(t[r].key, shift, mask);
      __hip_atomic_fetch_or(&lm[d], lanebit, __ATOMIC_RELAXED, __HIP_MEMORY_SCOPE_WORKGROUP);
      const u64 m = __hip_atomic_load(&lm[d], __ATOMIC_RELAXED, __HIP_MEMORY_SCOPE_WORKGROUP);
      const u32 old = __hip_atomic_load(&wc[d], __ATOMIC_RELAXED, __HIP_MEMORY_SCOPE_WORKGROUP);
      const u32 below = popc_below(m);
      if (below == 0) {
        __hip_atomic_store(&lm[d], 0ull, __ATOMIC_RELAXED, __HIP_MEMORY_SCOPE_WORKGROUP);
        __hip_atomic_store(&wc[d], (u16)(old + (u32)__popcll(m)), __ATOMIC_RELAXED,
                           __HIP_MEMORY_SCOPE_WORKGROUP);
      }
      rank = old + below;
    }
    dr[r] = (d << 16) | rank;
  }
  WC_MARK(1);
  lds_barrier();
  WC_MARK(2);

#if HMJ_WC_PLAN1
  if (w == 0) {
    constexpr int DPL = MAXD / kWave;
    u32 cnt[DPL], nl[DPL], pd[DPL], cf[DPL], fl[DPL];
#pragma unroll
    for (int j = 0; j < DPL; j++) {
      const u32 d = (u32)j * kWave + lane;
      cnt[j] = nl[j] = pd[j] = cf[j] = fl[j] = 0;
      if (d < D) {
        u32 c[WAVES];
#pragma unroll
        for (int k = 0; k < WAVES; k++) c[k] = sm.wcnt[k][d];
        u32 run = 0;
#pragma unroll
        for (int k = 0; k < WAVES; k++) {
          sm.wcnt[k][d] = (u16)run;
          run += c[k];
        }
        cnt[j] = run;
        pd[j] = sm.pend[d];
        cf[j] = sm.cflush[d];
        u32 avail = pd[j] + run;
        if (LIMIT && cf[j] + avail > limit(d)) {
          *ovf = true;
          avail = 0;
          pd[j] = 0;
        }
        const u32 tail = (cf[j] + avail) & (WC_LINE - 1);
        fl[j] = (tail >= avail) ? 0u : avail - tail;
        nl[j] = fl[j] ? (((cf[j] & (WC_LINE - 1)) + fl[j] + WC_LINE - 1) >> 3) : 0u;
        sm.pend[d] = avail - fl[j];
        sm.cflush[d] = cf[j] + fl[j];
      }
    }
    u32 running = 0;
#pragma unroll
    for (int j = 0; j < DPL; j++) {
      const u32 d = (u32)j * kWave + lane;
      const u32 v = (nl[j] << 16) | cnt[j];
      const u32 incl = wave_incl_scan_u32(v, lane);
      const u32 sc = running + incl - v;
      running += (u32)__builtin_amdgcn_readlane((int)incl, 63);
      if (d < D) {
        const u32 loff = sc >> 16;
        sm.tile_off[d] = sc & 0xFFFFu;
        if constexpr (Smem::HAS_CF_TILE) sm.cf_tile[d] = cf[j];
        sm.plan[d] = (fl[j] << 8) | pd[j];
        sm.line_off[d] = loff;
        for (u32 l = 0; l < nl[j]; l++) sm.line_tab[loff + l] = (u16)d;
      }
    }
    if (lane == 0) sm.total_lines = running >> 16;
  }
#else
  {
    u32 cnt = 0, nl = 0, pd = 0, cf = 0, fl = 0;
    if ((u32)tid < D) {
#pragma unroll
      for (int k = 0; k < WAVES; k++) {
        u32 c = sm.wcnt[k][tid];
        sm.wcnt[k][tid] = (u16)cnt;
        cnt += c;
      }
      pd = sm.pend[tid];
      cf = sm.cflush[tid];
      u32 avail = pd + cnt;
      if (LIMIT && cf + avail > limit((u32)tid)) {
        *ovf = true;
        avail = 0;
        pd = 0;
      }
      const u32 tail = (cf + avail) & (WC_LINE - 1);
      fl = (tail >= avail) ? 0u : avail - tail;
      nl = fl ? (((cf & (WC_LINE - 1)) + fl + WC_LINE - 1) >> 3) : 0u;
      sm.pend[tid] = avail - fl;
      sm.cflush[tid] = cf + fl;
    }
    u32 tot;
    const u32 sc = block_excl_scan_u32<THREADS, false>((nl << 16) | cnt, sm.scratch, &tot);
    if ((u32)tid < D) {
      const u32 loff = sc >> 16;
      sm.tile_off[tid] = sc & 0xFFFFu;
      if constexpr (Smem::HAS_CF_TILE) sm.cf_tile[tid] = cf;
      sm.plan[tid] = (fl << 8) | pd;
      sm.line_off[tid] = loff;
      for (u32 l = 0; l < nl; l++) sm.line_tab[loff + l] = (u16)tid;
    }
    if (tid == 0) sm.total_lines = tot >> 16;
  }
#endif
  WC_MARK(3);
  lds_barrier();
  WC_MARK(4);

#pragma unroll
  for (int r = 0; r < WC_ITEMS; r++) {
    if (ALLVALID || wbase + r * 64 < tile_n) {
      const u32 d = dr[r] >> 16;
      sm.stage[sm.tile_off[d] + sm.wcnt[w][d] + (dr[r] & 0xFFFFu)] = t[r];
    }
  }
  WC_MARK(5);
  prefetch();
  WC_MARK(12);
  lds_barrier();
  WC_MARK(6);

  {
    const u32 TL = sm.total_lines, k = (u32)tid & (WC_LINE - 1);
    for (u32 L = (u32)tid >> 3; L < TL; L += THREADS / WC_LINE) {
      const u32 d = sm.line_tab[L];
      const u32 pl = sm.plan[d], fl = pl >> 8, pd = pl & 0xFFu;
      u32 cfd;
      if constexpr (Smem::HAS_CF_TILE) cfd = sm.cf_tile[d];
      else cfd = sm.cflush[d] - fl;
      const u32 grow = (cfd & ~(u32)(WC_LINE - 1)) + (L - sm.line_off[d]) * WC_LINE + k;
      const u32 j = grow - cfd;
      if (j < fl) store_stream(&out[grow], (j < pd) ? sm.carry[d][j] : sm.stage[sm.tile_off[d] + j - pd]);
    }
  }
  u64 keep_k[WC_ITEMS], keep_v[WC_ITEMS];
  u32 has = 0;
#pragma unroll
  for (int q = 0; q < WC_ITEMS; q++) {
    const u32 s = q * THREADS + tid, d = s >> 3, k = s & (WC_LINE - 1);
    u32 idx = 0;
    if (d < D && k < sm.pend[d]) {
      const u32 pl = sm.plan[d], fl = pl >> 8, pd = pl & 0xFFu;
      if (fl != 0 || k >= pd) {
        idx = sm.tile_off[d] + (fl ? fl - pd + k : k - pd);
        has |= 1u << q;
      }
    }
    const Tup kv = sm.stage[idx];
    keep_k[q] = kv.key;
    keep_v[q] = kv.val;
  }
  WC_MARK(7);
  lds_barrier();
  WC_MARK(8);
#pragma unroll
  for (int q = 0; q < WC_ITEMS; q++) {
    const u32 s = q * THREADS + tid;
    if (has & (1u << q)) {
      Tup kv;
      kv.key = keep_k[q];
      kv.val = keep_v[q];
      sm.carry[s >> 3][s & (WC_LINE - 1)] = kv;
    }
  }
#if HMJ_WC_NOBAR5
  {
    constexpr int ZR = MAXD * 8 / 16;
    Tup z;
    z.key = 0;
    z.val = 0;
#pragma unroll
    for (int r = 0; r < ZR / kWave; r++) sm.stage[w * ZR + r * kWave + lane] = z;
    u32* wz = reinterpret_cast<u32*>(&sm.wcnt[w][0]);
#pragma unroll
    for (int r = 0; r < MAXD / 2 / kWave; r++) wz[r * kWave + lane] = 0;
  }
  WC_MARK(9);
  WC_MARK(10);
#else
#pragma unroll
  for (int r = 0; r < WC_ITEMS; r++) {
    if (r * THREADS < Smem::ZROWS) {
      Tup z;
      z.key = 0;
      z.val = 0;
      sm.stage[r * THREADS + tid] = z;
    }
  }
  for (int i = tid; i < WAVES * MAXD / 2; i += THREADS) reinterpret_cast<u32*>(&sm.wcnt[0][0])[i] = 0;
  WC_MARK(9);
  lds_barrier();
  WC_MARK(10);
#endif
}

template <int THREADS, int MAXD>
__device__ __forceinline__ void wc_flush_carry(WcSmem<THREADS, MAXD>& sm, Tup* __restrict__ out, u32 D) {
  const int tid = threadIdx.x;
  lds_barrier();
#pragma unroll
  for (int q = 0; q < WC_ITEMS; q++) {
    const u32 s = q * THREADS + tid, d = s >> 3, k = s & (WC_LINE - 1);
    if (d < D && k < sm.pend[d]) store_stream(&out[sm.cflush[d] + k], sm.carry[d][k]);
  }
}

template <int THREADS, int MAXD>
__device__ __forceinline__ void wc_clear(WcSmem<THREADS, MAXD>& sm) {
  constexpr int WAVES = WcSmem<THREADS, MAXD>::WAVES;
  const int tid = threadIdx.x;
  for (int i = tid; i < WAVES * MAXD / 2; i += THREADS) reinterpret_cast<u32*>(&sm.wcnt[0][0])[i] = 0;
  for (int i = tid; i < WAVES * MAXD; i += THREADS) (&sm.lanemask[0][0])[i] = 0;
}

template <int THREADS, int MAXD, bool HI, bool FULL>
__global__ __launch_bounds__(THREADS, (THREADS * (MAXD <= 256 ? 2 : 1)) / 256) void radix_scatter_wc_kernel(
    const Tup* __restrict__ in, Tup* __restrict__ out, u32 n, u32 n_full, int shift, int bits,
    u32 rows_per_block, u32 worker_base, const u32* __restrict__ hist_scanned,
    const u32* __restrict__ totals, u32 nblk, u64* __restrict__ offsets_out) {
  typedef WcSmem<THREADS, MAXD> Smem;
  constexpr int TILE = Smem::TILE;
  extern __shared__ __attribute__((aligned(16))) unsigned char smem_raw[];
  Smem& sm = *reinterpret_cast<Smem*>(smem_raw);
  const u32 D = 1u << bits, mask = D - 1;
  const int tid = threadIdx.x, lane = tid & 63, w = tid >> 6;
  const u32 worker = worker_base + blockIdx.x;

  {
    u32 t = ((u32)tid < D) ? totals[tid] : 0, tot;
    u32 base = block_excl_scan_u32<THREADS>(t, sm.scratch, &tot);
    if ((u32)tid < D) {
      sm.cflush[tid] = base + hist_scanned[(u64)tid * nblk + worker];
      sm.pend[tid] = 0;
      if (offsets_out && worker == 0) {
        offsets_out[tid] = base;
        if ((u32)tid == D - 1) offsets_out[D] = n;
      }
    }
    wc_clear(sm);
  }
  __syncthreads();

// ... 123 lines not shown
          for (int r = 0; r < WC_ITEMS; r++) {
            const u32 q = wbase + r * 64;
            t[r] = load_stream(&src[q < tn ? q : tn - 1]);
          }
        }
      };
      if constexpr (!std::is_same<Xform, NoXform>::value) xf(t, tile_n, wbase);
      if (HMJ_WC_FULLTILE && tile_n == (u32)TILE)
        wc_tile<THREADS, MAXD, HI, true, true>(sm, t, tile_n, slab, shift, mask, D, prefetch, limit, &ovf WC_STAMP_PASS);
      else
        wc_tile<THREADS, MAXD, HI, false, true>(sm, t, tile_n, slab, shift, mask, D, prefetch, limit, &ovf WC_STAMP_PASS);
    }
    wc_flush_carry(sm, slab, D);
  }
  if ((u32)tid < D) cnt_out[(u32)tid * WA + worker] = sm.cflush[tid] + sm.pend[tid] - ((u32)tid * WA + worker) * CA;
  if (ovf) atomicOr(&accum[ACC_ERR], ERR_SLAB);
#ifdef HMJ_STAMPS
  stamps.flush();
#endif
}

#ifndef HMJ_B_ADDR
#define HMJ_B_ADDR 2
#endif
#ifndef HMJ_B_NT
#define HMJ_B_NT 0
#endif
#ifdef HMJ_DEV
__device__ u32 g_b_ablate;
static bool g_b_addr_alt = false;
#endif
constexpr int SLAB_MAXSEG = 512;

template <int THREADS, int MAXD, bool HI, int ADDR>
__global__ __launch_bounds__(THREADS, (THREADS * (MAXD <= 256 ? 2 : 1)) / 256) void radix_slab_b_kernel(
    const Tup* __restrict__ slab_a, const u32* __restrict__ cnt_a, u32 CA, u32 WA, int bits_a, int shift,
    int bits, Tup* __restrict__ slab_b, u32 CB, u32* __restrict__ cnt_b, u64* __restrict__ accum, u32 KB) {
  typedef WcSmem<THREADS, MAXD> Smem;
  constexpr int TILE = Smem::TILE;
  static_assert(SLAB_MAXSEG <= THREADS, "one A-slab count per thread in the prologue scan");
  extern __shared__ __attribute__((aligned(16))) unsigned char smem_raw[];
  Smem& sm = *reinterpret_cast<Smem*>(smem_raw);
  u32* pre = reinterpret_cast<u32*>(smem_raw + sizeof(Smem));
  const u32 D = 1u << bits, mask = D - 1;
  const int tid = threadIdx.x, lane = tid & 63, w = tid >> 6;
  const u32 dA = blockIdx.x / KB, k = blockIdx.x % KB;
  const auto limit = [=](u32 d) { return (((d << bits_a) | dA) * KB + k) * CB + CB; };
  const u32 w0 = (u32)((u64)k * WA / KB), w1 = (u32)((u64)(k + 1) * WA / KB), ns = w1 - w0;
  {
    const u32 c = ((u32)tid < ns) ? cnt_a[dA * WA + w0 + tid] : 0;
    u32 tot;
    const u32 ex = block_excl_scan_u32<THREADS>(c, sm.scratch, &tot);
    if ((u32)tid < ns) pre[tid] = ex;
    if (tid == 0) pre[ns] = tot;
    if ((u32)tid < D) {
      sm.cflush[tid] = ((((u32)tid << bits_a) | dA) * KB + k) * CB;
      sm.pend[tid] = 0;
    }
    wc_clear(sm);
  }
  __syncthreads();
  const u32 total = pre[ns];
#ifdef HMJ_DEV
  const u32 abl = g_b_ablate;
#else
  constexpr u32 abl = 0;
#endif
  const u32 wbase = (u32)w * (WC_ITEMS * 64) + lane;
  (void)wbase;
  const Tup* __restrict__ bucket = slab_a + (u64)(dA * WA + w0) * CA;
  bool ovf = false;
#ifdef HMJ_STAMPS
  WcStamps stamps = {};
  stamps.base = 16;
#endif
  if (total) {
    Tup t[WC_ITEMS];
    if constexpr (ADDR != 0) {
    u32 d_s0 = 0, d_b0 = 0, d_b1 = 0, d_b2 = 0, d_b3 = 0;
    const float slabs_per_row = (float)ns / (float)total;
    auto plan1 = [&](u32 tile_begin) {
      u32 q0 = tile_begin + (u32)w * (WC_ITEMS * 64) + (u32)(lane & 3) * 64;
      q0 = q0 < total ? q0 : total - 1;
      u32 g = (u32)((float)q0 * slabs_per_row);
      g = g < ns ? g : ns - 1;
      u32 lo = g >= 3 ? g - 3 : 0;
      u32 pw[8];
#pragma unroll
      for (int i = 0; i < 8; i++) pw[i] = pre[lo + i < ns ? lo + i : ns];
      u32 j = 0;
#pragma unroll
      for (int i = 1; i < 8; i++) j += pw[i] <= q0 ? 1u : 0u;
      const bool bracketed = pw[0] <= q0 && pw[7] > q0;
      lo += j;
      if (__any(!bracketed)) {
        u32 hi = ns;
        lo = 0;
#pragma unroll
        for (int it = 0; it < 9; it++) {
          const u32 mid = (lo + hi) >> 1;
          const bool le = pre[mid] <= q0, act = hi - lo > 1;
          lo = (act && le) ? mid : lo;
          hi = (act && !le) ? mid : hi;
        }
      }
      d_s0 = lo;
      d_b0 = pre[lo];
      d_b1 = pre[lo + 1 < ns ? lo + 1 : ns];
      d_b2 = pre[lo + 2 < ns ? lo + 2 : ns];
      d_b3 = pre[lo + 3 < ns ? lo + 3 : ns];
    };
    auto issue1 = [&](u32 tile_begin) {
      u64 off[WC_ITEMS];
      const u32 wq0 = tile_begin + (u32)w * (WC_ITEMS * 64);
      u32 wlast = wq0 + WC_ITEMS * 64 - 1;
      wlast = wlast < total ? wlast : total - 1;
      const u32 s00 = (u32)__builtin_amdgcn_readlane((int)d_s0, 0), b00 = (u32)__builtin_amdgcn_readlane((int)d_b0, 0),
                b10 = (u32)__builtin_amdgcn_readlane((int)d_b1, 0);
      if (abl == 4) {
#pragma unroll
        for (int r = 0; r < WC_ITEMS; r++) {
          u32 q = wq0 + lane + r * 64;
          off[r] = q < total ? q : total - 1;
        }
      } else if (b10 > wlast) {
        const u64 o0 = (u64)s00 * CA;
#pragma unroll
        for (int r = 0; r < WC_ITEMS; r++) {
          u32 q = wq0 + lane + r * 64;
          q = q < total ? q : total - 1;
          off[r] = abl == 1 ? (u64)q : o0 + (q - (abl == 2 ? b00 & ~7u : b00));
        }
      } else {
#pragma unroll
        for (int r = 0; r < WC_ITEMS; r++) {
          const u32 s0 = (u32)__builtin_amdgcn_readlane((int)d_s0, r), b0 = (u32)__builtin_amdgcn_readlane((int)d_b0, r),
                    b1 = (u32)__builtin_amdgcn_readlane((int)d_b1, r), b2 = (u32)__builtin_amdgcn_readlane((int)d_b2, r),
                    b3 = (u32)__builtin_amdgcn_readlane((int)d_b3, r);
          u32 q = wq0 + lane + r * 64;
          q = q < total ? q : total - 1;
          u32 qlast = wq0 + r * 64 + 63;
          qlast = qlast < total ? qlast : total - 1;
          if (b3 > qlast) {
            const u32 j = (q >= b1 ? 1u : 0u) + (q >= b2 ? 1u : 0u);
            const u32 base = j == 0 ? b0 : (j == 1 ? b1 : b2);
            off[r] = abl == 1 ? (u64)q : (u64)(s0 + j) * CA + (q - (abl == 2 ? base & ~7u : base));
          } else {
            u32 sx = s0;
            while (sx + 1 < ns && pre[sx + 1] <= q) sx++;
            off[r] = (u64)sx * CA + (q - pre[sx]);
          }
        }
      }
#pragma unroll
      for (int r = 0; r < WC_ITEMS; r++) t[r] = HMJ_B_NT ? load_stream(&bucket[off[r]]) : bucket[off[r]];
    };
    u32 u_s0 = 0, u_b0 = 0, u_b1 = 0, u_b2 = 0, u_b3 = 0, u_b4 = 0;
    const u32 wq = (u32)__builtin_amdgcn_readfirstlane(w) * (WC_ITEMS * 64);
    u32 win_lo = 0;
    u32 win_v = pre[(u32)lane < ns ? (u32)lane : ns];
    auto plan2 = [&](u32 tile_begin) {
      u32 q0 = tile_begin + wq;
      q0 = q0 < total ? q0 : total - 1;
      u64 m = __ballot(win_v <= q0);
      u32 j = (u32)__popcll(m) - 1;
      if (!(m & 1) || j > 59) {
        u32 g = (u32)__builtin_amdgcn_readfirstlane((int)(u32)((float)q0 * slabs_per_row));
        g = g < ns ? g : ns - 1;
        win_lo = g >= 8 ? g - 8 : 0;
        win_v = pre[win_lo + (u32)lane < ns ? win_lo + (u32)lane : ns];
        m = __ballot(win_v <= q0);
        j = (u32)__popcll(m) - 1;
        if (!(m & 1) || j > 59) {
          u32 lo = 0, hi = ns;
#pragma unroll
          for (int it = 0; it < 9; it++) {
            const u32 mid = (lo + hi) >> 1;
            const bool le = pre[mid] <= q0, act = hi - lo > 1;
            lo = (act && le) ? mid : lo;
            hi = (act && !le) ? mid : hi;
          }
          win_lo = (u32)__builtin_amdgcn_readfirstlane((int)lo);
          win_v = pre[win_lo + (u32)lane < ns ? win_lo + (u32)lane : ns];
          m = __ballot(win_v <= q0);
          j = (u32)__popcll(m) - 1;
          j = j > 59 ? 59 : j;
        }
      }
      u_s0 = win_lo + j;
      u_b0 = (u32)__builtin_amdgcn_readlane((int)win_v, (int)j);
      u_b1 = (u32)__builtin_amdgcn_readlane((int)win_v, (int)j + 1);
      u_b2 = (u32)__builtin_amdgcn_readlane((int)win_v, (int)j + 2);
      u_b3 = (u32)__builtin_amdgcn_readlane((int)win_v, (int)j + 3);
      u_b4 = (u32)__builtin_amdgcn_readlane((int)win_v, (int)j + 4);
    };
    auto issue2 = [&](u32 tile_begin) {
      u64 off[WC_ITEMS];
      const u32 wq0 = tile_begin + wq;
      u32 wlast = wq0 + WC_ITEMS * 64 - 1;
      wlast = wlast < total ? wlast : total - 1;
      if (abl == 4) {
#pragma unroll
        for (int r = 0; r < WC_ITEMS; r++) {
          u32 q = wq0 + lane + r * 64;
          off[r] = q < total ? q : total - 1;
        }
      } else if (u_b1 > wlast) {
        const u64 o0 = (u64)u_s0 * CA;
#pragma unroll
        for (int r = 0; r < WC_ITEMS; r++) {
          u32 q = wq0 + lane + r * 64;
          q = q < total ? q : total - 1;
          off[r] = o0 + (q - u_b0);
        }
      } else if (u_b4 > wlast) {
#pragma unroll
        for (int r = 0; r < WC_ITEMS; r++) {
          u32 q = wq0 + lane + r * 64;
          q = q < total ? q : total - 1;
          const u32 j = (q >= u_b1 ? 1u : 0u) + (q >= u_b2 ? 1u : 0u) + (q >= u_b3 ? 1u : 0u);
          const u32 base = j == 0 ? u_b0 : (j == 1 ? u_b1 : (j == 2 ? u_b2 : u_b3));
          off[r] = (u64)(u_s0 + j) * CA + (q - base);
        }
      } else {
#pragma unroll
        for (int r = 0; r < WC_ITEMS; r++) {
          u32 q = wq0 + lane + r * 64;
          q = q < total ? q : total - 1;
          u32 sx = u_s0;
          while (sx + 1 < ns && pre[sx + 1] <= q) sx++;
          off[r] = (u64)sx * CA + (q - pre[sx]);
        }
      }
#pragma unroll
      for (int r = 0; r < WC_ITEMS; r++) t[r] = HMJ_B_NT ? load_stream(&bucket[off[r]]) : bucket[off[r]];
    };
    auto plan = [&](u32 tb) {
      if constexpr (ADDR == 2) plan2(tb); else plan1(tb);
    };
    auto issue = [&](u32 tb) {
      if constexpr (ADDR == 2) issue2(tb); else issue1(tb);
    };
    if (abl != 4) plan(0);
    issue(0);
    if ((u32)TILE < total && abl != 4) plan(TILE);
    for (u32 tile = 0; tile < total; tile += TILE) {
      const u32 tile_n = (total - tile < (u32)TILE) ? total - tile : (u32)TILE;
      auto prefetch = [&]() {
        if (tile + TILE < total) {
          issue(tile + TILE);
#ifdef HMJ_STAMPS
          stamps.mark(13);
#endif
          if (tile + 2 * TILE < total && abl != 4) plan(tile + 2 * TILE);
        }
      };
#ifdef HMJ_DEV
      if (abl == 1 || abl == 4) {
#pragma unroll
        for (int r = 0; r < WC_ITEMS; r++)
          if (t[r].key == 0) t[r].key = (u64)(tile + (u32)tid + r * THREADS + blockIdx.x * 7919u + 1) * 0x9E3779B97F4A7C15ull;
      }
#endif
      if (HMJ_WC_FULLTILE && tile_n == (u32)TILE)
        wc_tile<THREADS, MAXD, HI, true, true>(sm, t, tile_n, slab_b, shift, mask, D, prefetch, limit, &ovf WC_STAMP_PASS);
      else
        wc_tile<THREADS, MAXD, HI, false, true>(sm, t, tile_n, slab_b, shift, mask, D, prefetch, limit, &ovf WC_STAMP_PASS);
    }
    } else {
    u32 seg = 0;
    auto load = [&](u32 tile_begin) {
      const u32 tn = (total - tile_begin < (u32)TILE) ? total - tile_begin : (u32)TILE;
      while (seg + 1 < ns && pre[seg + 1] <= tile_begin) seg++;
      u32 s = seg;
      u64 off[WC_ITEMS];
#pragma unroll
      for (int r = 0; r < WC_ITEMS; r++) {
        u32 q = wbase + r * 64;
        q = tile_begin + (q < tn ? q : tn - 1);
        while (s + 1 < ns && pre[s + 1] <= q) s++;
        off[r] = (u64)s * CA + (q - pre[s]);
      }
#pragma unroll
      for (int r = 0; r < WC_ITEMS; r++) t[r] = HMJ_B_NT ? load_stream(&bucket[off[r]]) : bucket[off[r]];
    };
    load(0);
    for (u32 tile = 0; tile < total; tile += TILE) {
      const u32 tile_n = (total - tile < (u32)TILE) ? total - tile : (u32)TILE;
      wc_tile<THREADS, MAXD, HI, false, true>(
          sm, t, tile_n, slab_b, shift, mask, D,
          [&]() {
            if (tile + TILE < total) load(tile + TILE);
          },
          limit, &ovf WC_STAMP_PASS);
    }
    }
    wc_flush_carry(sm, slab_b, D);
  }
#ifdef HMJ_STAMPS
  stamps.flush();
#endif
  if ((u32)tid < D) {
    const u32 pid = (((u32)tid << bits_a) | dA) * KB + k;
    cnt_b[pid] = sm.cflush[tid] + sm.pend[tid] - pid * CB;
  }
  if (ovf && !abl) atomicOr(&accum[ACC_ERR], ERR_SLAB);
}

__global__ void part_offsets_kernel(const Tup* __restrict__ a, u32 n, int low, int bits,
                                    u32* __restrict__ off, u32 P) {
  u32 p = blockIdx.x * blockDim.x + threadIdx.x;
  if (p > P) return;
  if (p == P || bits == 0) {
    off[p] = (p == P) ? n : 0;
    return;
  }
  const u64* keys = reinterpret_cast<const u64*>(a);
// ... 76 lines not shown
  }
  if (eq_r) atomicAdd(&same[0], eq_r);
  if (eq_s) atomicAdd(&same[1], eq_s);
  if (up_r) atomicAdd(&order[0], up_r);
  if (dn_r) atomicAdd(&order[1], dn_r);
  if (up_s) atomicAdd(&order[2], up_s);
  if (dn_s) atomicAdd(&order[3], dn_s);
  __syncthreads();
  {
    const u64 lo = rng[0], span = rng[1] - rng[0];
#pragma unroll
    for (int k = 0; k < 2; k++)
      if (myvalid[k] && span) atomicAdd(&bins[(u32)((mykey[k] - lo) / ((span >> 6) + 1)) & 63u], 1u);
  }
  __syncthreads();
  if (tid == 0) {
    out[0] = acc;
    out[1] = ref;
    out[2] = (u64)same[0] | ((u64)order[0] << 16) | ((u64)order[1] << 32);
    out[3] = (u64)same[1] | ((u64)order[2] << 16) | ((u64)order[3] << 32);
    out[4] = rng[0];
    out[5] = rng[1];
    u32 nonempty = 0, big = 0;
    for (int i = 0; i < 64; i++) {
      nonempty += bins[i] ? 1u : 0u;
      big = bins[i] > big ? bins[i] : big;
    }
    out[6] = nonempty;
    out[7] = big;
  }
}

template <int THREADS, int MAXD, bool HI>
__global__ __launch_bounds__(THREADS, (THREADS * (MAXD <= 256 ? 2 : 1)) / 256) void radix_slab_a_kernel(
    const Tup* __restrict__ in, u32 n, int shift, int bits, u32 rows_per_worker, Tup* __restrict__ slab,
    u32 CA, u32 WA, u32* __restrict__ cnt_out, u64* __restrict__ accum, u32 worker_base) {
  NoXform xf;
  slab_a_body<THREADS, MAXD, HI, NoXform>(in, n, shift, bits, rows_per_worker, slab, CA, WA, cnt_out, accum, worker_base, xf);
}

template <bool CUT>
struct RankXform {
  static constexpr bool kStrided = CUT;
  u32 slot_mult;
  const Tup* __restrict__ tab;
  u32 mask;
  int hshift;
  int tb, pre;
  u64 svmin, svrange, mult;
  u64 acc_s;
  u64 n_rows;
  bool miss;
  __device__ __forceinline__ void operator()(Tup (&t)[WC_ITEMS], u32 tile_n, u32 wbase) {
    u32 slot[WC_ITEMS];
    bool live[WC_ITEMS], want[WC_ITEMS];
    u32 found = 0;
#pragma unroll
    for (int r = 0; r < WC_ITEMS; r++) {
      want[r] = wbase + (u32)r * 64 < tile_n;
      slot[r] = gt_hash(t[r].key, hshift);
      if (want[r]) acc_s += t[r].val;
      if (want[r]) n_rows++;
      live[r] = want[r] && t[r].key != GT_EMPTY;
    }
    u64 rank[WC_ITEMS] = {};
    gt_walk<WC_ITEMS>(tab, mask, slot, live, [&](int r, const Tup& e) {
      const bool eq = e.key == t[r].key;
      if (eq) {
        rank[r] = e.val;
        found |= 1u << r;
      }
// ... 167 lines not shown
    while (gcd(slot_mult, g.WA) != 1) slot_mult++;
  }
#define HMJ_SLAB_AR(T, M, C)                                                                                                          \
  {                                                                                                                                   \
    typedef WcSmem<T, M> Smem;                                                                                                        \
    static SmemAttrOnce once;                                                                                                         \
    if (hipError_t e = ensure_max_smem(once, reinterpret_cast<const void*>(radix_slab_a_rank_kernel<T, M, C>), sizeof(Smem)); e != hipSuccess) \
      return e;                                                                                                                       \
    hipLaunchKernelGGL((radix_slab_a_rank_kernel<T, M, C>), dim3(g.WA), dim3(T), sizeof(Smem), st, static_cast<const Tup*>(in), n, shift, bits, g.rpw, \
                       static_cast<Tup*>(slab_a), g.CA, g.WA, cnt_a, accum, static_cast<const Tup*>(tab), log_cap, extra, tb, svmin, svrange, pre, mult, \
                       slot_mult);                                                                                                    \
  }
  if (tb > 0) {
    if (bits > 8) HMJ_SLAB_AR(1024, 512, true) else HMJ_SLAB_AR(512, 256, true)
  } else {
    if (bits > 8) HMJ_SLAB_AR(1024, 512, false) else HMJ_SLAB_AR(512, 256, false)
  }
#undef HMJ_SLAB_AR
  return hipGetLastError();
}

hipError_t launch_slab_b(const void* slab_a, const u32* cnt_a, int bits_a, int shift, int bits,
                         const SlabGeom& g, void* slab_b, u64 slab_b_rows, u32* cnt_b, u64 cnt_b_n, u64* accum, hipStream_t st) {
  if (bits < 1 || bits > SLAB_MAX_BITS || bits_a < 1 || bits_a > SLAB_MAX_BITS || g.KB == 0 || g.WA < g.KB ||
      (g.WA + g.KB - 1) / g.KB > (u32)SLAB_MAXSEG)
    return hipErrorInvalidValue;
  const u64 pieces = ((u64)g.KB << (bits_a + bits));
  if (slab_b_rows < pieces * g.CB || cnt_b_n < pieces || pieces * g.CB >= 0xFFFFFFF0ull) return hipErrorInvalidValue;
  const bool hi = shift >= 32;
#define HMJ_SLAB_B(T, M, H) launch_slab_b_t<T, M, H>(slab_a, cnt_a, g.CA, g.WA, bits_a, shift, bits, slab_b, g.CB, cnt_b, accum, st, g.KB)
  if (bits > 8) return hi ? HMJ_SLAB_B(1024, 512, true) : HMJ_SLAB_B(1024, 512, false);
  return hi ? HMJ_SLAB_B(512, 256, true) : HMJ_SLAB_B(512, 256, false);
#undef HMJ_SLAB_B
}

__global__ __launch_bounds__(256) void key_exact_kernel(const Tup* __restrict__ R, u32 nb, const Tup* __restrict__ S, u32 np,
                                                        u64 ref, bool ref_is_first_key, u64* __restrict__ out) {
  if (ref_is_first_key) ref = nb ? R[0].key : (np ? S[0].key : 0);
  u64 x = 0, mn = ~0ull, mx = 0;
  const u64 stride = (u64)gridDim.x * blockDim.x;
  for (u64 i = (u64)blockIdx.x * blockDim.x + threadIdx.x; i < nb; i += stride) {
    const u64 k = R[i].key;
    x |= k ^ ref;
    mn = k < mn ? k : mn;
    mx = k > mx ? k : mx;
  }
  for (u64 i = (u64)blockIdx.x * blockDim.x + threadIdx.x; i < np; i += stride) x |= S[i].key ^ ref;
#pragma unroll
  for (int o = kWave / 2; o > 0; o >>= 1) {
    x |= __shfl_xor(x, o, kWave);
    const u64 a2 = __shfl_xor(mn, o, kWave), b2 = __shfl_xor(mx, o, kWave);
    mn = a2 < mn ? a2 : mn;
    mx = b2 > mx ? b2 : mx;
  }
  __shared__ u64 wx[4], wmn[4], wmx[4];
  if ((threadIdx.x & 63) == 0) {
    wx[threadIdx.x >> 6] = x;
    wmn[threadIdx.x >> 6] = mn;
    wmx[threadIdx.x >> 6] = mx;
  }
  __syncthreads();
  if (threadIdx.x == 0) {
    for (int w = 1; w < 4; w++) {
      x |= wx[w];
      mn = wmn[w] < mn ? wmn[w] : mn;
      mx = wmx[w] > mx ? wmx[w] : mx;
// ... 227 lines not shown
```

include/hmj.h:

```cpp
#ifndef HMJ_H
#define HMJ_H

#include <stddef.h>
#include <stdint.h>

#ifdef __cplusplus
extern "C" {
#endif

typedef struct hmj_ctx hmj_ctx;

#define HMJ_OK 0
#define HMJ_E_ARG (-1)
#define HMJ_E_NODEV (-2)
#define HMJ_E_OOM (-3)
#define HMJ_E_HIP (-4)
#define HMJ_E_UNSUPPORTED (-5)

#define HMJ_E_RCCL (-6)
#define HMJ_E_PEER (-7)
#define HMJ_E_TIMEOUT (-8)

#define HMJ_MATERIALIZE 0x01u
#define HMJ_ORDERED 0x02u
// ... 35 lines not shown
  uint32_t path;
  int32_t key_prefix_bits;
  int32_t key_window_low;
  uint32_t n_probe_items;
  float ms_scatter_pass[2];
} hmj_timing;
#define HMJ_PATH_SLAB 0x001u
#define HMJ_PATH_EXACT 0x002u
#define HMJ_PATH_UNIQ_WRITE 0x004u
#define HMJ_PATH_SPLIT 0x008u
#define HMJ_PATH_WINDOW 0x010u
#define HMJ_PATH_ORDER_DEFERRED 0x020u
#define HMJ_PATH_ORDER_BY_KEY 0x040u
#define HMJ_PATH_PREPARED 0x080u
#define HMJ_PATH_CHUNKED_BUILD 0x100u
#define HMJ_PATH_HOT_KEY_HINT 0x200u
#define HMJ_PATH_SLAB_PROBE 0x400u
#define HMJ_PATH_SORTED_WRITE 0x800u
#define HMJ_PATH_SORTED_FK 0x1000u
#define HMJ_PATH_DENSE_BUILD 0x2000u
#define HMJ_PATH_SORTED_FK_HALF 0x8000u
#define HMJ_PATH_SORTED_FK_WIDE 0x20000u
#define HMJ_PATH_LOOKBACK_TIMEOUT 0x10000u
#define HMJ_PATH_PRESORTED 0x40000u
#define HMJ_PATH_SLAB_ONE_PASS 0x80000u
#define HMJ_PATH_ORDER_BY_RANK_SORT 0x200000u
#define HMJ_PATH_RANK_RUNS 0x1000000u
#define HMJ_PATH_RANK_LOOKUP_IN_PASS 0x2000000u
#define HMJ_PATH_SORT_MSD 0x4000000u
#define HMJ_PATH_KEY_RANGES 0x8000000u
#define HMJ_PATH_ORDERED_EXPANSION 0x400000u
#define HMJ_PATH_LDS_TABLE 0x800000u
#define HMJ_PATH_GLOBAL_TABLE 0x100000u
#define HMJ_PATH_HOST_PIPELINE 0x4000u

typedef struct {
  uint32_t struct_size;
  uint32_t path;
  int32_t radix_bits, radix_passes, pass_bits[4];
  int32_t key_prefix_bits, key_window_low;
  uint32_t n_partitions;
  uint32_t probe_items;
  uint32_t attempts;
  uint32_t refused;
  uint32_t cooling;
  uint64_t workload;
} hmj_plan_desc;
#define HMJ_REFUSED_GTABLE_SHAPE 0x0001u
#define HMJ_REFUSED_GTABLE_COOLING 0x0002u
#define HMJ_REFUSED_GTABLE_GAVE_UP 0x0004u
#define HMJ_REFUSED_RANK_SORT_MODEL 0x0008u
#define HMJ_REFUSED_RANK_SORT_COOLING 0x0010u
#define HMJ_REFUSED_RANK_SORT_GAVE_UP 0x0020u
#define HMJ_REFUSED_SLAB_SHAPE 0x0040u
#define HMJ_REFUSED_SLAB_COOLING 0x0080u
#define HMJ_REFUSED_SLAB_SORTED_INPUT 0x0100u
#define HMJ_REFUSED_SLAB_OVERFLOW 0x0200u
#define HMJ_REFUSED_FAST_WRITE_COOLING 0x0400u
#define HMJ_REFUSED_FAST_WRITE_GAVE_UP 0x0800u
#define HMJ_REFUSED_SLAB_PROBE_COOLING 0x1000u
#define HMJ_REFUSED_SLAB_PROBE_OVERFLOW 0x2000u
#define HMJ_REFUSED_PREFIX_VIOLATED 0x4000u
#define HMJ_REFUSED_EXPANSION_GAVE_UP 0x8000u
#define HMJ_COOL_UNIQ_WRITE 0x001u
#define HMJ_COOL_SORTED_WRITE 0x002u
#define HMJ_COOL_GTABLE 0x004u
#define HMJ_COOL_GTABLE_WRITE 0x008u
#define HMJ_COOL_RANK_SORT 0x010u
#define HMJ_COOL_RANK_SORT_SLAB 0x020u
#define HMJ_COOL_EXPANSION 0x040u
#define HMJ_COOL_SORT_SLAB 0x080u
#define HMJ_COOL_SLAB 0x100u
#define HMJ_COOL_SLAB_PROBE 0x200u
#define HMJ_COOL_ONE_PASS_WRITE 0x400u
#define HMJ_COOL_EXACT_PREFIX 0x800u
#define HMJ_COOL_RANK_RUNS 0x1000u
#define HMJ_COOL_SORT_MSD 0x2000u

int hmj_create(hmj_ctx** out, int device_id);
void hmj_destroy(hmj_ctx* ctx);
#define HMJ_STREAM_OWN ((void*)(intptr_t)-1)
int hmj_set_stream(hmj_ctx* ctx, void* hip_stream);
int hmj_reserve(hmj_ctx* ctx, uint64_t n_build, uint64_t n_probe, uint64_t max_matches,
                uint32_t flags);
int hmj_set_radix_bits(hmj_ctx* ctx, int total_bits);
int hmj_autotune_radix_bits(hmj_ctx* ctx, uint64_t n_build, uint64_t n_probe, int apply, int* best_bits,
                            double ms[3]);
int hmj_set_key_prefix_bits(hmj_ctx* ctx, int bits);
int hmj_plan(uint64_t n_build, int* total_bits, int* n_passes, int pass_bits[4]);
#define HMJ_ABI_VERSION 5
int hmj_abi_version(void);
#define HMJ_PLACE_MAX_CAND 4
typedef struct {
  char name[16];
  uint64_t bytes;
  float fill_TBps;
  int candidates;
  float ms_search;
  int searched;
  int aborted;
  float budget_ms;
  float cand_ms_alloc[HMJ_PLACE_MAX_CAND];
  float cand_ms_fill[HMJ_PLACE_MAX_CAND];
  float cand_TBps[HMJ_PLACE_MAX_CAND];
} hmj_place_info;
int hmj_placement_info(hmj_ctx* ctx, hmj_place_info* out, int max_entries);
int hmj_last_plan(hmj_ctx* ctx, hmj_plan_desc* out);
int hmj_forget_workloads(hmj_ctx* ctx);
int hmj_set_profiling(hmj_ctx* ctx, int enabled);
int hmj_last_timing(hmj_ctx* ctx, hmj_timing* out);
// ... 321 lines not shown
```

Measured before the change: 34.30 billion.

## Partition probe side as keys-only slabs and fold probe values into scatter

```diff
diff --git a/hashmergejoin_amd/__init__.py b/hashmergejoin_amd/__init__.py
--- a/hashmergejoin_amd/__init__.py
+++ b/hashmergejoin_amd/__init__.py
@@ -1,13 +1,13 @@
 from ._lib import (HMJ_BUILD_ANTI, HMJ_BUILD_OUTER, HMJ_BUILD_SEMI, HMJ_CHECKSUM, HMJ_COLS_HASHED, HMJ_COLS_NO_ROW, HMJ_COLS_PACKED, HMJ_FIRST_WINS, HMJ_FULL_OUTER, HMJ_JOIN_ANTI, HMJ_JOIN_INNER, HMJ_JOIN_PROBE_OUTER, HMJ_JOIN_SEMI, HMJ_KIND_BUILD_SIDE, HMJ_KIND_PROBE_SIDE, HMJ_MATERIALIZE, HMJ_ORDERED, HMJ_PATH_CHUNKED_BUILD, HMJ_PATH_DENSE_BUILD,
                    HMJ_PATH_EXACT, HMJ_PATH_GLOBAL_TABLE, HMJ_PATH_HOST_PIPELINE, HMJ_PATH_HOT_KEY_HINT, HMJ_PATH_LOOKBACK_TIMEOUT, HMJ_PATH_ORDER_BY_KEY, HMJ_PATH_ORDER_BY_RANK_SORT, HMJ_PATH_ORDER_DEFERRED, HMJ_PATH_ORDERED_EXPANSION, HMJ_PATH_LDS_TABLE,
-                   HMJ_PATH_KEY_RANGES, HMJ_PATH_PREPARED, HMJ_PATH_PRESORTED, HMJ_PATH_RANK_RUNS, HMJ_PATH_SORT_MSD, HMJ_PATH_SLAB, HMJ_PATH_SLAB_ONE_PASS, HMJ_PATH_SLAB_PROBE, HMJ_PATH_SORTED_FK, HMJ_PATH_SORTED_FK_HALF, HMJ_PATH_SORTED_FK_WIDE, HMJ_PATH_SORTED_WRITE, HMJ_PATH_SPLIT, HMJ_PATH_UNIQ_WRITE, HMJ_PATH_WINDOW,
+                   HMJ_PATH_KEY_RANGES, HMJ_PATH_NARROW_PROBE, HMJ_PATH_PREPARED, HMJ_PATH_PRESORTED, HMJ_PATH_RANK_RUNS, HMJ_PATH_SORT_MSD, HMJ_PATH_SLAB, HMJ_PATH_SLAB_ONE_PASS, HMJ_PATH_SLAB_PROBE, HMJ_PATH_SORTED_FK, HMJ_PATH_SORTED_FK_HALF, HMJ_PATH_SORTED_FK_WIDE, HMJ_PATH_SORTED_WRITE, HMJ_PATH_SPLIT, HMJ_PATH_UNIQ_WRITE, HMJ_PATH_WINDOW,
                    HMJ_KEY_FIXED, HMJ_KEY_LARGE_STRING, HMJ_MAX_KEY_COLS, HMJ_MAX_TAKE_COLS, HMJ_STR_NO_ROW, HMJ_SUM_PROBE, HMJ_TAKE_NO_ROW, BuildJoinOpts, ColsJoinOpts, ColsKindOpts, ColsRel, ColsResult, ExchangeKindOpts, HmjError, JoinOpts, JoinResult, KeyCol, KindCounts, MixedCol, MixedOpts, MixedRel, StrJoinOpts, StrKindOpts, StrRel, StrResult, TakeDst, TakeOpts, TakeSrc, TakeStrDst, TakeStrOpts, TakeStrSrc, Timing, Validity,
                    lib_path, load_library)
 from .join import Executor, HashMergeJoin, cols_key64, mixed_key64, pack_strings, pack_validity, plan, unpack_strings, unpack_validity
 
 __all__ = ["Executor", "HashMergeJoin", "plan", "HmjError", "JoinResult", "Timing", "load_library",
            "lib_path", "HMJ_MATERIALIZE", "HMJ_ORDERED", "HMJ_FIRST_WINS", "HMJ_CHECKSUM",
-           "HMJ_SUM_PROBE", "JoinOpts", "HMJ_JOIN_INNER", "HMJ_JOIN_SEMI", "HMJ_JOIN_ANTI", "HMJ_JOIN_PROBE_OUTER",
+           "HMJ_SUM_PROBE", "HMJ_PATH_NARROW_PROBE", "JoinOpts", "HMJ_JOIN_INNER", "HMJ_JOIN_SEMI", "HMJ_JOIN_ANTI", "HMJ_JOIN_PROBE_OUTER",
            "BuildJoinOpts", "HMJ_BUILD_SEMI", "HMJ_BUILD_ANTI", "HMJ_BUILD_OUTER", "HMJ_FULL_OUTER",
            "ExchangeKindOpts", "KindCounts", "HMJ_KIND_PROBE_SIDE", "HMJ_KIND_BUILD_SIDE",
            "pack_strings", "StrRel", "StrJoinOpts", "StrResult", "StrKindOpts", "HMJ_STR_NO_ROW",
diff --git a/hashmergejoin_amd/_lib.py b/hashmergejoin_amd/_lib.py
--- a/hashmergejoin_amd/_lib.py
+++ b/hashmergejoin_amd/_lib.py
@@ -28,6 +28,7 @@
 HMJ_PATH_LOOKBACK_TIMEOUT = 0x10000
 HMJ_PATH_SORTED_FK_WIDE = 0x20000
 HMJ_PATH_PRESORTED = 0x40000
+HMJ_PATH_NARROW_PROBE = 0x10000000
 
 _HERE = os.path.dirname(os.path.abspath(__file__))
 _U64P = C.POINTER(C.c_uint64)
@@ -244,6 +245,9 @@
 HMJ_COOL_RANK_SORT, HMJ_COOL_RANK_SORT_SLAB, HMJ_COOL_EXPANSION, HMJ_COOL_SORT_SLAB = 0x10, 0x20, 0x40, 0x80
 HMJ_COOL_SLAB, HMJ_COOL_SLAB_PROBE, HMJ_COOL_ONE_PASS_WRITE, HMJ_COOL_EXACT_PREFIX = 0x100, 0x200, 0x400, 0x800
 HMJ_COOL_RANK_RUNS = 0x1000
+HMJ_COOL_SORT_MSD = 0x2000
+HMJ_REFUSED_NARROW_PROBE_GAVE_UP, HMJ_REFUSED_NARROW_PROBE_COOLING = 0x10000, 0x20000
+HMJ_COOL_NARROW_PROBE = 0x4000
 
 
 class PlaceInfo(C.Structure):
diff --git a/hashmergejoin_amd/csrc/api.hip b/hashmergejoin_amd/csrc/api.hip
--- a/hashmergejoin_amd/csrc/api.hip
+++ b/hashmergejoin_amd/csrc/api.hip
@@ -85,7 +85,8 @@
          (gtable_sort_slab_cooldown ? HMJ_COOL_RANK_SORT_SLAB : 0u) | (expand_cooldown ? HMJ_COOL_EXPANSION : 0u) |
          (sort_slab_cooldown ? HMJ_COOL_SORT_SLAB : 0u) | (slab_cooldown ? HMJ_COOL_SLAB : 0u) | (slab_probe_cooldown ? HMJ_COOL_SLAB_PROBE : 0u) |
          (one_pass_write_cooldown ? HMJ_COOL_ONE_PASS_WRITE : 0u) | (exact_prefix_joins ? HMJ_COOL_EXACT_PREFIX : 0u) |
-         (rank_runs_cooldown ? HMJ_COOL_RANK_RUNS : 0u) | (sort_msd_cooldown ? HMJ_COOL_SORT_MSD : 0u);
+         (rank_runs_cooldown ? HMJ_COOL_RANK_RUNS : 0u) | (sort_msd_cooldown ? HMJ_COOL_SORT_MSD : 0u) |
+         ((narrow_probe_cooldown || narrow_probe_failures >= 2) ? HMJ_COOL_NARROW_PROBE : 0u);
 }
 
 int wait_arrival(hmj_ctx* c, hipEvent_t ev) {
@@ -509,6 +510,7 @@
 constexpr int kRetryNoSlabProbe = 1004;
 constexpr int kRetryMoreBits = 1005;
 constexpr int kRetryNoPrefix = 1000;
+constexpr int kRetryNoNarrowProbe = 1007;
 
 static int read_accum(hmj_ctx* c, u64** h) {
   u64* hh = (u64*)c->h_accum.p;
@@ -1198,7 +1200,61 @@
   RC_TRY(ensure_dev(c, c->slab_bs, gs.rows_b * 16));
   RC_TRY(ensure_dev(c, c->cnt_br, (size_t)P * gr.KB * 4));
   RC_TRY(ensure_dev(c, c->cnt_bs, (size_t)P * gs.KB * 4));
+  hmj::SlabGeom gk = gs;
+  gk.CA = (gs.CA + 15u) & ~15u;
+  gk.CB = (gs.CB + 15u) & ~15u;
+  const bool narrow_shape = j.flags == 0 && !c->prepare_only && c->narrow_probe && c->narrow_probe_allowed && c->arrive_ev.empty() &&
+                            !c->sample_build_only && c->min_prefix_bits == 0 && c->join_kind == 0 && ba <= 8 && bb <= 8 && np > 0 &&
+                            ((u64)gk.WA << ba) * gk.CA < 0xFFFFFFF0ull && ((u64)P * gk.KB) * gk.CB < 0xFFFFFFF0ull &&
+                            ((uintptr_t)c->slab_a.p & 127u) == 0 && ((uintptr_t)c->slab_bs.p & 127u) == 0;
+  bool narrow = false;
+  if (narrow_shape) {
+    if (c->wm->narrow_probe_failures >= 2) {
+      c->plan.refused |= HMJ_REFUSED_NARROW_PROBE_COOLING;
+    } else if (c->wm->narrow_probe_cooldown > 0) {
+      c->wm->narrow_probe_cooldown--;
+      c->plan.refused |= HMJ_REFUSED_NARROW_PROBE_COOLING;
+    } else {
+      narrow = true;
+    }
+  }
   if (!reuse) RC_TRY(slab_passes(c, j.R, nb, 0, p.low, ba, bb, gr, c->slab_br, c->cnt_br, false));
+  if (narrow) {
+    u64* acc = (u64*)c->accum.p;
+    int sk = span_begin(c, K_SCATTER, 1, 0);
+    HIP_TRY(hmj::launch_slab_a_keys(j.S, np, p.low, ba, gk, c->slab_a.p, c->slab_a.cap, (u32*)c->cnt_a.p, c->cnt_a.cap / 4, acc, c->stream));
+    span_end(c, sk);
+    c->timing.bytes_scatter += 24ull * np;
+    sk = span_begin(c, K_SCATTER, 1, 1);
+    HIP_TRY(hmj::launch_slab_b_keys(c->slab_a.p, (const u32*)c->cnt_a.p, ba, p.low + ba, bb, gk, c->slab_bs.p, c->slab_bs.cap, (u32*)c->cnt_bs.p,
+                                    c->cnt_bs.cap / 4, acc, c->stream));
+    span_end(c, sk);
+    c->timing.bytes_scatter += 16ull * np;
+    hmj::ProbeArgs ka = slab_probe_args(c, &gr, nullptr, c->slab_bs, c->cnt_bs, gk.CB, P, 1);
+    ka.s_rows = c->slab_bs.cap / 8;
+    const int sp = span_begin(c, K_PROBE_COUNT, -1);
+    HIP_TRY(hmj::launch_probe_count_slab_keys(ka, c->num_cus, c->stream));
+    span_end(c, sp);
+    c->timing.bytes_probe_count = 16ull * nb + 8ull * np;
+    u64* kh;
+    RC_TRY(read_accum(c, &kh));
+    if (kh[hmj::ACC_ERR] & hmj::ERR_SLAB) {
+      c->wm->slab_cooldown = 8;
+      return kRetryNoSlab;
+    }
+    if (kh[hmj::ACC_ERR] & hmj::ERR_NARROW) {
+      c->wm->narrow_probe_failures++;
+      c->wm->narrow_probe_cooldown = 64;
+      if (reuse) c->prep.valid = true;
+      return kRetryNoNarrowProbe;
+    }
+    c->wm->narrow_probe_failures = 0;
+    c->timing.path |= HMJ_PATH_NARROW_PROBE;
+    result_sums(j.out, kh);
+    j.out->sum_s = kh[hmj::ACC_SUM_P];
+    j.out->sum_probe_all = 0;
+    return HMJ_OK;
+  }
   if (!c->prepare_only) RC_TRY(slab_passes(c, j.S, np, 1, p.low, ba, bb, gs, c->slab_bs, c->cnt_bs, !c->arrive_ev.empty()));
   u64* hh;
   if (c->prepare_only) {
@@ -2435,15 +2491,17 @@
     ~Unforce() {
       if (*on) c->force_bits = -1;
       c->expand_allow_rebits = true;
+      c->narrow_probe_allowed = true;
     }
   } unforce{c, &forced_here};
+  c->narrow_probe_allowed = true;
   for (int attempt = 0; attempt < 8; attempt++) {
     c->plan.attempts = (uint32_t)attempt + 1;
     int rc = join_device_impl(c, R, n_build, S, n_probe, flags, out, to_host, auto_prefix, slab, fast_write,
                               win_ordered, prefix_unsafe, slab_probe);
     c->plan.refused |= rc == kRetryNoSlab ? HMJ_REFUSED_SLAB_OVERFLOW : rc == kRetryNoPrefix ? HMJ_REFUSED_PREFIX_VIOLATED
                        : rc == kRetryNoFastWrite ? HMJ_REFUSED_FAST_WRITE_GAVE_UP : rc == kRetryNoSlabProbe ? HMJ_REFUSED_SLAB_PROBE_OVERFLOW
-                       : rc == kRetryMoreBits ? HMJ_REFUSED_EXPANSION_GAVE_UP : 0u;
+                       : rc == kRetryMoreBits ? HMJ_REFUSED_EXPANSION_GAVE_UP : rc == kRetryNoNarrowProbe ? HMJ_REFUSED_NARROW_PROBE_GAVE_UP : 0u;
     if (c->trace)
       std::fprintf(stderr, "[hmj] join nb=%llu np=%llu flags=%#x attempt %d: rc=%d bits=%d passes=%d path=%#x prefix=%d low=%d items=%u%s\n",
                    (unsigned long long)n_build, (unsigned long long)n_probe, flags, attempt, rc, c->timing.radix_bits,
@@ -2454,15 +2512,17 @@
                    : rc == kRetryNoFastWrite ? " -> retry without the unique-key write mode"
                    : rc == kRetryNoWinOrdered ? " -> retry without the key window"
                    : rc == kRetryNoSlabProbe ? " -> retry without probe-side slabs (one overflowed)"
-                   : rc == kRetryMoreBits ? " -> retry with one more radix bit (a partition did not fit the ordered expansion)" : "");
+                   : rc == kRetryMoreBits ? " -> retry with one more radix bit (a partition did not fit the ordered expansion)"
+                   : rc == kRetryNoNarrowProbe ? " -> retry with 16-byte probe rows (a probe row without exactly one build row)" : "");
     if (rc == kRetryNoSlab || rc == kRetryNoPrefix || rc == kRetryNoFastWrite || rc == kRetryNoWinOrdered || rc == kRetryNoSlabProbe ||
-        rc == kRetryMoreBits) {
+        rc == kRetryMoreBits || rc == kRetryNoNarrowProbe) {
       std::vector<Span> keep;
       for (const Span& sp : c->spans)
         if (sp.kind == K_TOTAL || sp.kind == K_H2D) keep.push_back(sp);
       c->spans.swap(keep);
       std::memset(&c->timing, 0, sizeof(c->timing));
       if (rc == kRetryNoSlab) slab = false;
+      else if (rc == kRetryNoNarrowProbe) c->narrow_probe_allowed = false;
       else if (rc == kRetryMoreBits) {
         c->force_bits = c->expand_rebits;
         c->expand_allow_rebits = false;
@@ -2545,6 +2605,7 @@
   hmj_ctx* c = new hmj_ctx();
   c->device = device_id;
   if (const char* e = getenv("HMJ_SLAB")) c->slab_mode = atoi(e);
+  if (const char* e = getenv("HMJ_NARROW_PROBE")) c->narrow_probe = atoi(e) != 0;
   if (const char* e = getenv("HMJ_ONE_PASS_SLAB")) c->one_pass_slab = atoi(e) != 0;
   if (const char* e = getenv("HMJ_GTABLE")) c->gtable_mode = atoi(e) != 0;
   if (const char* e = getenv("HMJ_RANK_RUNS")) c->rank_runs_mode = atoi(e) != 0;
diff --git a/hashmergejoin_amd/csrc/hmj_ctx.h b/hashmergejoin_amd/csrc/hmj_ctx.h
--- a/hashmergejoin_amd/csrc/hmj_ctx.h
+++ b/hashmergejoin_amd/csrc/hmj_ctx.h
@@ -71,6 +71,8 @@
   int slab_cooldown = 0;
   int slab_probe_cooldown = 0;
   int one_pass_write_cooldown = 0;
+  int narrow_probe_cooldown = 0;
+  int narrow_probe_failures = 0;
   int exact_prefix_joins = 0;
   uint32_t cooling() const;
 };
@@ -191,6 +193,8 @@
   bool sort_slab = true;
   u64 sort_slab_min = 1ull << 25;
   int slab_mode = 1;
+  bool narrow_probe = true;
+  bool narrow_probe_allowed = true;
   bool staged_upload = false;
   bool host_pipeline = true;
   hipStream_t copy_stream = nullptr;
diff --git a/hashmergejoin_amd/csrc/hmj_dev.h b/hashmergejoin_amd/csrc/hmj_dev.h
--- a/hashmergejoin_amd/csrc/hmj_dev.h
+++ b/hashmergejoin_amd/csrc/hmj_dev.h
@@ -107,6 +107,7 @@
 constexpr u64 ERR_FASTPATH = 8;
 constexpr u64 ERR_GTABLE = 128;
 constexpr u64 ERR_PREFIX = 4;
+constexpr u64 ERR_NARROW = 256;
 
 __device__ __forceinline__ u64 mix64(u64 x) {
   x ^= x >> 30;
diff --git a/hashmergejoin_amd/csrc/hmj_launch.h b/hashmergejoin_amd/csrc/hmj_launch.h
--- a/hashmergejoin_amd/csrc/hmj_launch.h
+++ b/hashmergejoin_amd/csrc/hmj_launch.h
@@ -53,6 +53,10 @@
                          u32* cnt_a, u64 cnt_a_n, u64* accum, hipStream_t st, u32 w_begin = 0, u32 w_end = 0xFFFFFFFFu);
 hipError_t launch_slab_b(const void* slab_a, const u32* cnt_a, int bits_a, int shift, int bits,
                          const SlabGeom& g, void* slab_b, u64 slab_b_rows, u32* cnt_b, u64 cnt_b_n, u64* accum, hipStream_t st);
+hipError_t launch_slab_a_keys(const void* in, u32 n, int shift, int bits, const SlabGeom& g, void* slab_a, u64 slab_a_bytes,
+                              u32* cnt_a, u64 cnt_a_n, u64* accum, hipStream_t st);
+hipError_t launch_slab_b_keys(const void* slab_a, const u32* cnt_a, int bits_a, int shift, int bits, const SlabGeom& g, void* slab_b,
+                              u64 slab_b_bytes, u32* cnt_b, u64 cnt_b_n, u64* accum, hipStream_t st);
 hipError_t launch_key_sample(const void* R, u32 nb, const void* S, u32 np, u64* out, hipStream_t st);
 hipError_t launch_key_exact(const void* R, u32 nb, const void* S, u32 np, u64 ref, u64* out, int num_cus, hipStream_t st,
                             bool ref_is_first_key = false);
@@ -100,6 +104,7 @@
 hipError_t launch_probe_count_ext(const ProbeArgs& a, u32* irregular, u32* n_irregular, bool slab,
                                   int num_cus, hipStream_t st);
 hipError_t launch_probe_count_slab(const ProbeArgs& a, int num_cus, hipStream_t st);
+hipError_t launch_probe_count_slab_keys(const ProbeArgs& a, int num_cus, hipStream_t st);
 hipError_t launch_probe_write_sorted(const ProbeArgs& a, bool slab, bool fk, int shape, u64* lookback, bool chained, int key_low,
                                      int num_cus, hipStream_t st);
 hipError_t launch_probe_write_uniq(const ProbeArgs& a, bool slab, int num_cus, hipStream_t st);
diff --git a/hashmergejoin_amd/csrc/probe.hip b/hashmergejoin_amd/csrc/probe.hip
--- a/hashmergejoin_amd/csrc/probe.hip
+++ b/hashmergejoin_amd/csrc/probe.hip
@@ -916,11 +916,15 @@
   }
 }
 
-template <int THREADS>
-__device__ __forceinline__ void fp_load_pieces(Tup (&t)[FP_ROWS], const Tup* __restrict__ base, u32 cap, u32 cnt_mine, int tid) {
+__device__ __forceinline__ u64 fp_key(const Tup& t) { return t.key; }
+__device__ __forceinline__ u64 fp_key(u64 k) { return k; }
+__device__ __forceinline__ u64 fp_val(const Tup& t) { return t.val; }
+__device__ __forceinline__ u64 fp_val(u64) { return 0; }
+template <int THREADS, typename Row>
+__device__ __forceinline__ void fp_load_pieces(Row (&t)[FP_ROWS], const Row* __restrict__ base, u32 cap, u32 cnt_mine, int tid) {
   constexpr int QT = THREADS / 4;
   const u32 g = (u32)tid / QT, l = (u32)tid % QT;
-  const Tup* __restrict__ piece = base + (u64)g * cap;
+  const Row* __restrict__ piece = base + (u64)g * cap;
   const u32 last = cnt_mine ? cnt_mine - 1 : 0;
 #pragma unroll
   for (int k = 0; k < FP_ROWS; k++) {
@@ -929,17 +933,19 @@
   }
 }
 
-template <int THREADS, int LOG_NB, bool PCOUNT, bool SLAB, int OUT>
+template <int THREADS, int LOG_NB, bool PCOUNT, bool SLAB, int OUT, bool NARROW = false>
 __global__ __launch_bounds__(THREADS, 4) void probe_count_fast_kernel(
     ProbeArgs a, u32* __restrict__ irregular, u32* __restrict__ n_irregular) {
   typedef FastSmem<THREADS, LOG_NB> Smem;
+  typedef typename std::conditional<NARROW, u64, Tup>::type PRow;
   constexpr u32 CAP = Smem::CAP, NB = 1u << LOG_NB;
   constexpr bool PIECES = SLAB && OUT == 0 && !PCOUNT && HMJ_PROBE_PIECES;
+  static_assert(!NARROW || PIECES, "the keys-only probe side exists for the plain slab count join");
   constexpr u32 QT = THREADS / 4, PIECE_CAP = FP_ROWS * QT;
   extern __shared__ __attribute__((aligned(16))) unsigned char smem_raw[];
   Smem& sm = *reinterpret_cast<Smem*>(smem_raw);
   const Tup* __restrict__ R = static_cast<const Tup*>(a.R);
-  const Tup* __restrict__ S = static_cast<const Tup*>(a.S);
+  const PRow* __restrict__ S = static_cast<const PRow*>(a.S);
   const u32* __restrict__ r_off = a.r_off;
   const u32* __restrict__ s_off = a.s_off;
   const u32* __restrict__ r_end = (SLAB || a.r_end == nullptr) ? a.r_off + 1 : a.r_end;
@@ -947,7 +953,7 @@
   const u32 P = a.P;
   const int tid = threadIdx.x;
   u64 acc_n = 0, acc_r = 0, acc_s = 0, acc_x = 0, acc_m = 0, acc_p = 0;
-  bool pfx_bad = false, giveup = false;
+  bool pfx_bad = false, giveup = false, narrow_bad = false;
   for (u32 i = tid; i < NB; i += THREADS) sm.head[i] = 0;
   if (tid < 2) sm.itemcnt[tid] = 0;
   u32 epoch = 0;
@@ -956,7 +962,8 @@
   u32 p = blockIdx.x;
   u32 rb = 0, nb = 0, sb = 0, np = 0;
   bool regular = false;
-  Tup br[FP_ROWS], pr[FP_ROWS], pq[FP_ROWS];
+  Tup br[FP_ROWS];
+  PRow pr[FP_ROWS], pq[FP_ROWS];
   u32 r1 = 0, r2 = 0, r3 = 0, s1 = 0, s2 = 0, s3 = 0, r1n = 0, r2n = 0, r3n = 0, s1n = 0, s2n = 0, s3n = 0;
   u32 rm = 0, sm_ = 0, rmn = 0, smn = 0;
   const u32 my_piece = (u32)tid / QT;
@@ -983,7 +990,10 @@
     }
     regular = nb && np && nb <= CAP && np <= CAP;
     if (regular) {
-      if (PIECES) {
+      if constexpr (NARROW) {
+        fp_load_pieces<THREADS>(br, R + (u64)p * SLAB_KB * a.r_cap, a.r_cap, rm, tid);
+        fp_load_pieces<THREADS>(pr, S + (u64)p * SLAB_KB * a.s_cap, a.s_cap, sm_, tid);
+      } else if (PIECES) {
         fp_load_pieces<THREADS>(br, R + (u64)p * SLAB_KB * a.r_cap, a.r_cap, rm, tid);
         fp_load_pieces<THREADS>(pr, S + (u64)p * SLAB_KB * a.s_cap, a.s_cap, sm_, tid);
       } else if (SLAB) {
@@ -996,6 +1006,7 @@
     }
   }
   const Tup* __restrict__ dummy = reinterpret_cast<const Tup*>(a.accum);
+  const PRow* __restrict__ dummy_s = reinterpret_cast<const PRow*>(a.accum);
   auto load_build = [&](Tup (&t)[FP_ROWS], bool ok, u32 pp, u32 rb_, u32 nb_, u32 q1, u32 q2, u32 q3, u32 mine) {
     if (PIECES)
       fp_load_pieces<THREADS>(t, ok ? R + (u64)pp * SLAB_KB * a.r_cap : dummy, ok ? a.r_cap : 0u, ok ? mine : 1u, tid);
@@ -1005,14 +1016,16 @@
     else
       fp_load<THREADS>(t, ok ? R + rb_ : dummy, ok ? nb_ : 1u, tid);
   };
-  auto load_probe = [&](Tup (&t)[FP_ROWS], bool ok, u32 pp, u32 sb_, u32 np_, u32 q1, u32 q2, u32 q3, u32 mine) {
-    if (PIECES)
-      fp_load_pieces<THREADS>(t, ok ? S + (u64)pp * SLAB_KB * a.s_cap : dummy, ok ? a.s_cap : 0u, ok ? mine : 1u, tid);
+  auto load_probe = [&](PRow (&t)[FP_ROWS], bool ok, u32 pp, u32 sb_, u32 np_, u32 q1, u32 q2, u32 q3, u32 mine) {
+    if constexpr (NARROW)
+      fp_load_pieces<THREADS>(t, ok ? S + (u64)pp * SLAB_KB * a.s_cap : dummy_s, ok ? a.s_cap : 0u, ok ? mine : 1u, tid);
+    else if (PIECES)
+      fp_load_pieces<THREADS>(t, ok ? S + (u64)pp * SLAB_KB * a.s_cap : dummy_s, ok ? a.s_cap : 0u, ok ? mine : 1u, tid);
     else if (SLAB)
-      fp_load_slab<THREADS>(t, ok ? S + (u64)pp * SLAB_KB * a.s_cap : dummy, ok ? a.s_cap : 0u, ok ? q1 : 1u, ok ? q2 : 1u,
+      fp_load_slab<THREADS>(t, ok ? S + (u64)pp * SLAB_KB * a.s_cap : dummy_s, ok ? a.s_cap : 0u, ok ? q1 : 1u, ok ? q2 : 1u,
                             ok ? q3 : 1u, ok ? np_ : 1u, tid);
     else
-      fp_load<THREADS>(t, ok ? S + sb_ : dummy, ok ? np_ : 1u, tid);
+      fp_load<THREADS>(t, ok ? S + sb_ : dummy_s, ok ? np_ : 1u, tid);
   };
   const int tid_outer = tid;
   while (p < P) {
@@ -1051,10 +1064,12 @@
     if (OUT == 0) {
       load_probe(pq, regular2, pn, sb2, np2, s1n, s2n, s3n, smn);
     } else if (regular) {
-      if (SLAB)
-        fp_load_slab<THREADS>(pr, S + (u64)p * SLAB_KB * a.s_cap, a.s_cap, s1, s2, s3, np, tid);
-      else
-        fp_load<THREADS>(pr, S + sb, np, tid);
+      if constexpr (!NARROW) {
+        if (SLAB)
+          fp_load_slab<THREADS>(pr, S + (u64)p * SLAB_KB * a.s_cap, a.s_cap, s1, s2, s3, np, tid);
+        else
+          fp_load<THREADS>(pr, S + sb, np, tid);
+      }
     }
     if (regular) {
       lds_barrier();
@@ -1102,12 +1117,13 @@
         for (int k = 0; k < FP_ROWS; k++) {
           const u32 j = k * THREADS + tid;
           cur[k] = NIL;
-          cnt[k] = 0;
+          cnt[k] = NARROW ? 1 : 0;
           first[k] = OUT == 2 ? NIL : 0;
           if (PIECES ? ((u32)tid % QT + (u32)k * QT < sm_) : (j < np)) {
-            if (a.pfx_shift && (pr[k].key >> a.pfx_shift) != a.pfx_val) pfx_bad = true;
-            if (OUT >= 1 && (a.extra & 1u)) acc_p += pr[k].val;
-            const u32 hv = sm.head[fast_hash<LOG_NB>(pr[k].key)];
+            if (NARROW) cnt[k] = 0;
+            if (a.pfx_shift && (fp_key(pr[k]) >> a.pfx_shift) != a.pfx_val) pfx_bad = true;
+            if (OUT >= 1 && (a.extra & 1u)) acc_p += fp_val(pr[k]);
+            const u32 hv = sm.head[fast_hash<LOG_NB>(fp_key(pr[k]))];
             cur[k] = ((hv >> 16) == epoch) ? (hv & 0xFFFFu) : NIL;
           }
         }
@@ -1122,19 +1138,20 @@
               const u32 i = cur[k];
               const u64 kk = sm.key[i], vv = sm.val[i];
               cur[k] = sm.next[i];
-              if (kk == pr[k].key) {
+              if (kk == fp_key(pr[k])) {
                 if (OUT == 2 && (a.extra & 2u)) {
                   first[k] = i < first[k] ? i : first[k];
                 } else {
                   acc_n++;
                   acc_r += vv;
-                  acc_s += pr[k].val;
+                  if (!NARROW) acc_s += fp_val(pr[k]);
+                  if (NARROW) cnt[k]++;
                   if (OUT == 1) {
                     if (cnt[k] == 0) first[k] = i;
                     cnt[k]++;
                   }
                   if (OUT >= 1 && (a.extra & 1u)) {
-                    const u64 m = tmix(kk, vv, pr[k].val);
+                    const u64 m = tmix(kk, vv, fp_val(pr[k]));
                     acc_x ^= m;
                     acc_m += m;
                   }
@@ -1143,6 +1160,10 @@
             }
           }
         }
+        if (NARROW) {
+#pragma unroll
+          for (int k = 0; k < FP_ROWS; k++) narrow_bad |= cnt[k] != 1;
+        }
         if (OUT == 2 && (a.extra & 2u)) {
 #pragma unroll
           for (int k = 0; k < FP_ROWS; k++) {
@@ -1150,9 +1171,9 @@
               const u64 vv = sm.val[first[k]];
               acc_n++;
               acc_r += vv;
-              acc_s += pr[k].val;
+              acc_s += fp_val(pr[k]);
               if (a.extra & 1u) {
-                const u64 m = tmix(pr[k].key, vv, pr[k].val);
+                const u64 m = tmix(fp_key(pr[k]), vv, fp_val(pr[k]));
                 acc_x ^= m;
                 acc_m += m;
               }
@@ -1199,9 +1220,9 @@
             for (int k = 0; k < FP_ROWS; k++) {
               if (cnt[k]) {
                 const u64 d = o + ((ex >> (12 * k)) & 0xFFFu);
-                a.out_key[d] = pr[k].key;
+                a.out_key[d] = fp_key(pr[k]);
                 a.out_rval[d] = sm.val[first[k]];
-                a.out_sval[d] = pr[k].val;
+                a.out_sval[d] = fp_val(pr[k]);
               }
               const u32 tk = (u32)((tot >> (12 * k)) & 0xFFFu);
               o += tk;
@@ -1212,7 +1233,7 @@
         }
       } else {
 #pragma unroll
-        for (int k = 0; k < FP_ROWS; k++) acc_r += pr[k].key;
+        for (int k = 0; k < FP_ROWS; k++) acc_r += fp_key(pr[k]);
       }
       if (PCOUNT) {
         const u32 mine = (u32)(acc_n - n_before);
@@ -1222,18 +1243,19 @@
         parity ^= 1;
       }
     } else {
+      if (NARROW && np && !nb) narrow_bad = true;
       if ((PCOUNT || OUT == 1) && tid == 0 && !(nb && np)) a.part_count[p] = 0;
       if (OUT == 1 && nb && np) giveup = true;
-      if (OUT >= 1 && (a.extra & 1u) && !nb) {
+      if (!NARROW && OUT >= 1 && (a.extra & 1u) && !nb) {
         if (SLAB) {
-          const Tup* base = S + (u64)p * SLAB_KB * a.s_cap;
+          const PRow* base = S + (u64)p * SLAB_KB * a.s_cap;
           for (u32 j = tid; j < np; j += THREADS) {
             const u32 pc = (j >= s1) + (j >= s2) + (j >= s3);
             const u32 pre = pc == 0 ? 0 : pc == 1 ? s1 : pc == 2 ? s2 : s3;
-            acc_p += base[(u64)pc * a.s_cap + (j - pre)].val;
+            acc_p += fp_val(base[(u64)pc * a.s_cap + (j - pre)]);
           }
         } else {
-          for (u32 j = tid; j < np; j += THREADS) acc_p += S[sb + j].val;
+          for (u32 j = tid; j < np; j += THREADS) acc_p += fp_val(S[sb + j]);
         }
       }
       if (OUT != 1 && !SLAB && tid == 0 && nb && np) irregular[atomicAdd(n_irregular, 1u)] = p;
@@ -1250,6 +1272,12 @@
   if (SLAB && slab_bad && tid == 0) atomicOr(&a.accum[ACC_ERR], ERR_SLAB);
   if (OUT == 1 && __any(giveup) && (tid & 63) == 0) atomicOr(&a.accum[ACC_ERR], ERR_FASTPATH);
   if (__any(pfx_bad) && (tid & 63) == 0) atomicOr(&a.accum[ACC_ERR], ERR_PREFIX);
+  if constexpr (NARROW) {
+    lds_barrier();
+    if (__any(narrow_bad) && (tid & 63) == 0) sm.itemcnt[0] = 1;
+    lds_barrier();
+    if (tid == 0 && sm.itemcnt[0]) atomicOr(&a.accum[ACC_ERR], ERR_NARROW);
+  }
   lds_barrier();
   if (PCOUNT && prev_p != 0xFFFFFFFFu && tid == 0) a.part_count[prev_p] = sm.itemcnt[parity ^ 1];
   if (tid < 8) sm.red[tid] = 0;
@@ -2410,15 +2438,15 @@
   return hipGetLastError();
 }
 
-template <int THREADS, int LOG_NB, bool PCOUNT, bool SLAB = false, int OUT = 0>
+template <int THREADS, int LOG_NB, bool PCOUNT, bool SLAB = false, int OUT = 0, bool NARROW = false>
 static hipError_t launch_fast_t(const ProbeArgs& a, u32* irregular, u32* n_irregular, int grid,
                                 hipStream_t st) {
   typedef FastSmem<THREADS, LOG_NB> Smem;
   static SmemAttrOnce attr_once;
-  if (hipError_t e = ensure_max_smem(attr_once, reinterpret_cast<const void*>(probe_count_fast_kernel<THREADS, LOG_NB, PCOUNT, SLAB, OUT>), (size_t)sizeof(Smem)); e != hipSuccess) return e;
+  if (hipError_t e = ensure_max_smem(attr_once, reinterpret_cast<const void*>(probe_count_fast_kernel<THREADS, LOG_NB, PCOUNT, SLAB, OUT, NARROW>), (size_t)sizeof(Smem)); e != hipSuccess) return e;
   if ((u32)grid > a.P) grid = (int)a.P;
   if (grid < 1) grid = 1;
-  hipLaunchKernelGGL((probe_count_fast_kernel<THREADS, LOG_NB, PCOUNT, SLAB, OUT>), dim3(grid), dim3(THREADS),
+  hipLaunchKernelGGL((probe_count_fast_kernel<THREADS, LOG_NB, PCOUNT, SLAB, OUT, NARROW>), dim3(grid), dim3(THREADS),
                      sizeof(Smem), st, a, irregular, n_irregular);
   return hipGetLastError();
 }
@@ -2523,6 +2551,11 @@
 hipError_t launch_probe_count_slab(const ProbeArgs& a, int num_cus, hipStream_t st) {
   if (!slab_operands_ok(a)) return hipErrorInvalidValue;
   return launch_fast_t<1024, BIG_LOG_NB, false, true>(a, nullptr, nullptr, num_cus * 4, st);
+}
+
+hipError_t launch_probe_count_slab_keys(const ProbeArgs& a, int num_cus, hipStream_t st) {
+  if (!slab_operands_ok(a) || a.extra || a.pfx_shift) return hipErrorInvalidValue;
+  return launch_fast_t<1024, BIG_LOG_NB, false, true, 0, true>(a, nullptr, nullptr, num_cus * 4, st);
 }
 
 hipError_t launch_probe(const ProbeArgs& a, int mode, bool first_wins, bool extra, int grid,
diff --git a/hashmergejoin_amd/csrc/radix.hip b/hashmergejoin_amd/csrc/radix.hip
--- a/hashmergejoin_amd/csrc/radix.hip
+++ b/hashmergejoin_amd/csrc/radix.hip
@@ -232,7 +232,51 @@
 }
 
 constexpr int WC_ITEMS = 4;
-constexpr int WC_LINE = 8;
+__device__ __forceinline__ u64 row_key(const Tup& t) { return t.key; }
+__device__ __forceinline__ u64 row_key(u64 k) { return k; }
+template <typename Row, int N>
+struct WcKeep;
+template <int N>
+struct WcKeep<Tup, N> {
+  u64 k[N], v[N];
+  __device__ __forceinline__ void set(int q, const Tup& t) {
+    k[q] = t.key;
+    v[q] = t.val;
+  }
+  __device__ __forceinline__ Tup get(int q) const {
+    Tup kv;
+    kv.key = k[q];
+    kv.val = v[q];
+    return kv;
+  }
+  static __device__ __forceinline__ Tup zero() {
+    Tup z;
+    z.key = 0;
+    z.val = 0;
+    return z;
+  }
+};
+template <int N>
+struct WcKeep<u64, N> {
+  u64 k[N];
+  __device__ __forceinline__ void set(int q, u64 t) { k[q] = t; }
+  __device__ __forceinline__ u64 get(int q) const { return k[q]; }
+  static __device__ __forceinline__ u64 zero() { return 0ull; }
+};
+__device__ __forceinline__ void store_stream(u64* p, u64 v) {
+#if HMJ_STREAM_POLICY >= 1
+  __builtin_nontemporal_store(v, p);
+#else
+  *p = v;
+#endif
+}
+__device__ __forceinline__ u64 load_stream(const u64* p) {
+#if HMJ_STREAM_POLICY >= 2
+  return __builtin_nontemporal_load(p);
+#else
+  return *p;
+#endif
+}
 
 #ifndef HMJ_WC_PLAN1
 #define HMJ_WC_PLAN1 0
@@ -274,19 +318,26 @@
 #define WC_VMWAIT()
 #endif
 
-template <int THREADS, int MAXD>
+template <int THREADS, int MAXD, typename Row = Tup, int NITEMS = WC_ITEMS>
 struct WcSmem {
-  static constexpr int TILE = THREADS * WC_ITEMS;
+  static constexpr int ITEMS = NITEMS;
+  static constexpr int TILE = THREADS * ITEMS;
   static constexpr int WAVES = THREADS / kWave;
-  static constexpr int ZROWS = WAVES * MAXD * 8 / 16;
-  static constexpr int MAXLINES = TILE / WC_LINE + 2 * MAXD;
+  static constexpr int LINE = 128 / (int)sizeof(Row);
+  static constexpr int LOG_LINE = LINE == 8 ? 3 : 4;
+  static constexpr int CARRY = MAXD * LINE;
+  static constexpr int KEEP = CARRY / THREADS;
+  static constexpr int ZROWS = WAVES * MAXD * 8 / (int)sizeof(Row);
+  static constexpr int MAXLINES = TILE / LINE + 2 * MAXD;
+  static_assert(sizeof(Row) == 16 || sizeof(Row) == 8, "rows of 16 or 8 bytes");
   static_assert(ZROWS <= TILE && ZROWS % THREADS == 0, "lane masks must alias whole row slabs");
-  static_assert(MAXD <= THREADS && MAXD * WC_LINE == TILE, "one digit per thread; carry == tile slots");
+  static_assert(MAXD <= THREADS && CARRY % THREADS == 0 && CARRY >= TILE, "one digit per thread; whole carry slots per thread");
+  static_assert(NITEMS == WC_ITEMS || (NITEMS == 2 * WC_ITEMS && sizeof(Row) == 8), "4 rows per thread, or 8 rows of 8 bytes");
   union {
-    Tup stage[TILE];
+    Row stage[TILE];
     u64 lanemask[WAVES][MAXD];
   };
-  Tup carry[MAXD][WC_LINE];
+  Row carry[MAXD][LINE];
   u16 wcnt[WAVES][MAXD];
   u32 tile_off[MAXD];
   u32 cflush[MAXD];
@@ -303,19 +354,21 @@
 struct NoLimit {
   __device__ __forceinline__ u32 operator()(u32) const { return 0xFFFFFFFFu; }
 };
-template <int THREADS, int MAXD, bool HI, bool ALLVALID, bool LIMIT, typename Prefetch, typename Limit>
-__device__ __forceinline__ void wc_tile(WcSmem<THREADS, MAXD>& sm, Tup (&t)[WC_ITEMS], u32 tile_n,
-                                        Tup* __restrict__ out, int shift, u32 mask, u32 D,
+template <int THREADS, int MAXD, bool HI, bool ALLVALID, bool LIMIT, typename Row, int NITEMS, typename Prefetch, typename Limit>
+__device__ __forceinline__ void wc_tile(WcSmem<THREADS, MAXD, Row, NITEMS>& sm, Row (&t)[NITEMS], u32 tile_n,
+                                        Row* __restrict__ out, int shift, u32 mask, u32 D,
                                         Prefetch&& prefetch, const Limit& limit, bool* ovf WC_STAMP_ARG) {
-  typedef WcSmem<THREADS, MAXD> Smem;
+  typedef WcSmem<THREADS, MAXD, Row, NITEMS> Smem;
   constexpr int WAVES = Smem::WAVES;
+  constexpr int WC_LINE = Smem::LINE;
+  constexpr int ITEMS = Smem::ITEMS;
   const int tid = threadIdx.x, lane = tid & 63, w = tid >> 6;
   u16* wc = &sm.wcnt[w][0];
   u64* lm = &sm.lanemask[w][0];
   const u64 lanebit = 1ull << lane;
-  const u32 wbase = (u32)w * (WC_ITEMS * 64) + lane;
-
-  u32 dr[WC_ITEMS];
+  const u32 wbase = (u32)w * (ITEMS * 64) + lane;
+
+  u32 dr[ITEMS];
 #ifdef HMJ_STAMPS
   stamps.last = __builtin_amdgcn_s_memtime();
   WC_VMWAIT();
@@ -323,10 +376,10 @@
   stamps.acc[11]++;
 #endif
 #pragma unroll
-  for (int r = 0; r < WC_ITEMS; r++) {
+  for (int r = 0; r < ITEMS; r++) {
     u32 d = 0, rank = 0;
     if (ALLVALID || wbase + r * 64 < tile_n) {
-      d = digit_of<HI>(t[r].key, shift, mask);
+      d = digit_of<HI>(row_key(t[r]), shift, mask);
       __hip_atomic_fetch_or(&lm[d], lanebit, __ATOMIC_RELAXED, __HIP_MEMORY_SCOPE_WORKGROUP);
       const u64 m = __hip_atomic_load(&lm[d], __ATOMIC_RELAXED, __HIP_MEMORY_SCOPE_WORKGROUP);
       const u32 old = __hip_atomic_load(&wc[d], __ATOMIC_RELAXED, __HIP_MEMORY_SCOPE_WORKGROUP);
@@ -373,7 +426,7 @@
         }
         const u32 tail = (cf[j] + avail) & (WC_LINE - 1);
         fl[j] = (tail >= avail) ? 0u : avail - tail;
-        nl[j] = fl[j] ? (((cf[j] & (WC_LINE - 1)) + fl[j] + WC_LINE - 1) >> 3) : 0u;
+        nl[j] = fl[j] ? (((cf[j] & (WC_LINE - 1)) + fl[j] + WC_LINE - 1) >> Smem::LOG_LINE) : 0u;
         sm.pend[d] = avail - fl[j];
         sm.cflush[d] = cf[j] + fl[j];
       }
@@ -417,7 +470,7 @@
       }
       const u32 tail = (cf + avail) & (WC_LINE - 1);
       fl = (tail >= avail) ? 0u : avail - tail;
-      nl = fl ? (((cf & (WC_LINE - 1)) + fl + WC_LINE - 1) >> 3) : 0u;
+      nl = fl ? (((cf & (WC_LINE - 1)) + fl + WC_LINE - 1) >> Smem::LOG_LINE) : 0u;
       sm.pend[tid] = avail - fl;
       sm.cflush[tid] = cf + fl;
     }
@@ -439,7 +492,7 @@
   WC_MARK(4);
 
 #pragma unroll
-  for (int r = 0; r < WC_ITEMS; r++) {
+  for (int r = 0; r < ITEMS; r++) {
     if (ALLVALID || wbase + r * 64 < tile_n) {
       const u32 d = dr[r] >> 16;
       sm.stage[sm.tile_off[d] + sm.wcnt[w][d] + (dr[r] & 0xFFFFu)] = t[r];
@@ -453,7 +506,7 @@
 
   {
     const u32 TL = sm.total_lines, k = (u32)tid & (WC_LINE - 1);
-    for (u32 L = (u32)tid >> 3; L < TL; L += THREADS / WC_LINE) {
+    for (u32 L = (u32)tid >> Smem::LOG_LINE; L < TL; L += THREADS / WC_LINE) {
       const u32 d = sm.line_tab[L];
       const u32 pl = sm.plan[d], fl = pl >> 8, pd = pl & 0xFFu;
       u32 cfd;
@@ -464,11 +517,11 @@
       if (j < fl) store_stream(&out[grow], (j < pd) ? sm.carry[d][j] : sm.stage[sm.tile_off[d] + j - pd]);
     }
   }
-  u64 keep_k[WC_ITEMS], keep_v[WC_ITEMS];
+  WcKeep<Row, Smem::KEEP> keep;
   u32 has = 0;
 #pragma unroll
-  for (int q = 0; q < WC_ITEMS; q++) {
-    const u32 s = q * THREADS + tid, d = s >> 3, k = s & (WC_LINE - 1);
+  for (int q = 0; q < Smem::KEEP; q++) {
+    const u32 s = q * THREADS + tid, d = s >> Smem::LOG_LINE, k = s & (WC_LINE - 1);
     u32 idx = 0;
     if (d < D && k < sm.pend[d]) {
       const u32 pl = sm.plan[d], fl = pl >> 8, pd = pl & 0xFFu;
@@ -477,29 +530,21 @@
         has |= 1u << q;
       }
     }
-    const Tup kv = sm.stage[idx];
-    keep_k[q] = kv.key;
-    keep_v[q] = kv.val;
+    const Row kv = sm.stage[idx];
+    keep.set(q, kv);
   }
   WC_MARK(7);
   lds_barrier();
   WC_MARK(8);
 #pragma unroll
-  for (int q = 0; q < WC_ITEMS; q++) {
+  for (int q = 0; q < Smem::KEEP; q++) {
     const u32 s = q * THREADS + tid;
-    if (has & (1u << q)) {
-      Tup kv;
-      kv.key = keep_k[q];
-      kv.val = keep_v[q];
-      sm.carry[s >> 3][s & (WC_LINE - 1)] = kv;
-    }
+    if (has & (1u << q)) sm.carry[s >> Smem::LOG_LINE][s & (WC_LINE - 1)] = keep.get(q);
   }
 #if HMJ_WC_NOBAR5
   {
-    constexpr int ZR = MAXD * 8 / 16;
-    Tup z;
-    z.key = 0;
-    z.val = 0;
+    constexpr int ZR = MAXD * 8 / (int)sizeof(Row);
+    const Row z = WcKeep<Row, 1>::zero();
 #pragma unroll
     for (int r = 0; r < ZR / kWave; r++) sm.stage[w * ZR + r * kWave + lane] = z;
     u32* wz = reinterpret_cast<u32*>(&sm.wcnt[w][0]);
@@ -510,13 +555,8 @@
   WC_MARK(10);
 #else
 #pragma unroll
-  for (int r = 0; r < WC_ITEMS; r++) {
-    if (r * THREADS < Smem::ZROWS) {
-      Tup z;
-      z.key = 0;
-      z.val = 0;
-      sm.stage[r * THREADS + tid] = z;
-    }
+  for (int r = 0; r < ITEMS; r++) {
+    if (r * THREADS < Smem::ZROWS) sm.stage[r * THREADS + tid] = WcKeep<Row, 1>::zero();
   }
   for (int i = tid; i < WAVES * MAXD / 2; i += THREADS) reinterpret_cast<u32*>(&sm.wcnt[0][0])[i] = 0;
   WC_MARK(9);
@@ -525,20 +565,21 @@
 #endif
 }
 
-template <int THREADS, int MAXD>
-__device__ __forceinline__ void wc_flush_carry(WcSmem<THREADS, MAXD>& sm, Tup* __restrict__ out, u32 D) {
+template <int THREADS, int MAXD, typename Row, int NITEMS>
+__device__ __forceinline__ void wc_flush_carry(WcSmem<THREADS, MAXD, Row, NITEMS>& sm, Row* __restrict__ out, u32 D) {
+  typedef WcSmem<THREADS, MAXD, Row, NITEMS> Smem;
   const int tid = threadIdx.x;
   lds_barrier();
 #pragma unroll
-  for (int q = 0; q < WC_ITEMS; q++) {
-    const u32 s = q * THREADS + tid, d = s >> 3, k = s & (WC_LINE - 1);
+  for (int q = 0; q < Smem::KEEP; q++) {
+    const u32 s = q * THREADS + tid, d = s >> Smem::LOG_LINE, k = s & (Smem::LINE - 1);
     if (d < D && k < sm.pend[d]) store_stream(&out[sm.cflush[d] + k], sm.carry[d][k]);
   }
 }
 
-template <int THREADS, int MAXD>
-__device__ __forceinline__ void wc_clear(WcSmem<THREADS, MAXD>& sm) {
-  constexpr int WAVES = WcSmem<THREADS, MAXD>::WAVES;
+template <int THREADS, int MAXD, typename Row, int NITEMS>
+__device__ __forceinline__ void wc_clear(WcSmem<THREADS, MAXD, Row, NITEMS>& sm) {
+  constexpr int WAVES = WcSmem<THREADS, MAXD, Row, NITEMS>::WAVES;
   const int tid = threadIdx.x;
   for (int i = tid; i < WAVES * MAXD / 2; i += THREADS) reinterpret_cast<u32*>(&sm.wcnt[0][0])[i] = 0;
   for (int i = tid; i < WAVES * MAXD; i += THREADS) (&sm.lanemask[0][0])[i] = 0;
@@ -728,16 +769,25 @@
 #endif
 constexpr int SLAB_MAXSEG = 512;
 
-template <int THREADS, int MAXD, bool HI, int ADDR>
+#ifndef HMJ_B_KEY_ITEMS
+#define HMJ_B_KEY_ITEMS 8
+#endif
+template <typename Row>
+struct SLAB_B_ITEMS {
+  static constexpr int value = sizeof(Row) == 8 ? HMJ_B_KEY_ITEMS : WC_ITEMS;
+};
+template <int THREADS, int MAXD, bool HI, int ADDR, typename Row = Tup>
 __global__ __launch_bounds__(THREADS, (THREADS * (MAXD <= 256 ? 2 : 1)) / 256) void radix_slab_b_kernel(
-    const Tup* __restrict__ slab_a, const u32* __restrict__ cnt_a, u32 CA, u32 WA, int bits_a, int shift,
-    int bits, Tup* __restrict__ slab_b, u32 CB, u32* __restrict__ cnt_b, u64* __restrict__ accum, u32 KB) {
-  typedef WcSmem<THREADS, MAXD> Smem;
-  constexpr int TILE = Smem::TILE;
+    const Row* __restrict__ slab_a, const u32* __restrict__ cnt_a, u32 CA, u32 WA, int bits_a, int shift,
+    int bits, Row* __restrict__ slab_b, u32 CB, u32* __restrict__ cnt_b, u64* __restrict__ accum, u32 KB) {
+  typedef WcSmem<THREADS, MAXD, Row, SLAB_B_ITEMS<Row>::value> Smem;
+  constexpr int TILE = Smem::TILE, ITEMS = Smem::ITEMS;
+  static_assert(ADDR == 2 || ITEMS == WC_ITEMS, "the per-round lookups (lanes 0..3) are written for four rounds");
   static_assert(SLAB_MAXSEG <= THREADS, "one A-slab count per thread in the prologue scan");
   extern __shared__ __attribute__((aligned(16))) unsigned char smem_raw[];
   Smem& sm = *reinterpret_cast<Smem*>(smem_raw);
   u32* pre = reinterpret_cast<u32*>(smem_raw + sizeof(Smem));
+  typedef typename std::conditional<sizeof(Row) == 8, u32, u64>::type off_t;
   const u32 D = 1u << bits, mask = D - 1;
   const int tid = threadIdx.x, lane = tid & 63, w = tid >> 6;
   const u32 dA = blockIdx.x / KB, k = blockIdx.x % KB;
@@ -762,21 +812,21 @@
 #else
   constexpr u32 abl = 0;
 #endif
-  const u32 wbase = (u32)w * (WC_ITEMS * 64) + lane;
+  const u32 wbase = (u32)w * (ITEMS * 64) + lane;
   (void)wbase;
-  const Tup* __restrict__ bucket = slab_a + (u64)(dA * WA + w0) * CA;
+  const Row* __restrict__ bucket = slab_a + (u64)(dA * WA + w0) * CA;
   bool ovf = false;
 #ifdef HMJ_STAMPS
   WcStamps stamps = {};
   stamps.base = 16;
 #endif
   if (total) {
-    Tup t[WC_ITEMS];
+    Row t[ITEMS];
     if constexpr (ADDR != 0) {
     u32 d_s0 = 0, d_b0 = 0, d_b1 = 0, d_b2 = 0, d_b3 = 0;
     const float slabs_per_row = (float)ns / (float)total;
     auto plan1 = [&](u32 tile_begin) {
-      u32 q0 = tile_begin + (u32)w * (WC_ITEMS * 64) + (u32)(lane & 3) * 64;
+      u32 q0 = tile_begin + (u32)w * (ITEMS * 64) + (u32)(lane & 3) * 64;
       q0 = q0 < total ? q0 : total - 1;
       u32 g = (u32)((float)q0 * slabs_per_row);
       g = g < ns ? g : ns - 1;
@@ -807,29 +857,29 @@
       d_b3 = pre[lo + 3 < ns ? lo + 3 : ns];
     };
     auto issue1 = [&](u32 tile_begin) {
-      u64 off[WC_ITEMS];
-      const u32 wq0 = tile_begin + (u32)w * (WC_ITEMS * 64);
-      u32 wlast = wq0 + WC_ITEMS * 64 - 1;
+      off_t off[ITEMS];
+      const u32 wq0 = tile_begin + (u32)w * (ITEMS * 64);
+      u32 wlast = wq0 + ITEMS * 64 - 1;
       wlast = wlast < total ? wlast : total - 1;
       const u32 s00 = (u32)__builtin_amdgcn_readlane((int)d_s0, 0), b00 = (u32)__builtin_amdgcn_readlane((int)d_b0, 0),
                 b10 = (u32)__builtin_amdgcn_readlane((int)d_b1, 0);
       if (abl == 4) {
 #pragma unroll
-        for (int r = 0; r < WC_ITEMS; r++) {
+        for (int r = 0; r < ITEMS; r++) {
           u32 q = wq0 + lane + r * 64;
           off[r] = q < total ? q : total - 1;
         }
       } else if (b10 > wlast) {
         const u64 o0 = (u64)s00 * CA;
 #pragma unroll
-        for (int r = 0; r < WC_ITEMS; r++) {
+        for (int r = 0; r < ITEMS; r++) {
           u32 q = wq0 + lane + r * 64;
           q = q < total ? q : total - 1;
-          off[r] = abl == 1 ? (u64)q : o0 + (q - (abl == 2 ? b00 & ~7u : b00));
+          off[r] = (off_t)(abl == 1 ? (u64)q : o0 + (q - (abl == 2 ? b00 & ~7u : b00)));
         }
       } else {
 #pragma unroll
-        for (int r = 0; r < WC_ITEMS; r++) {
+        for (int r = 0; r < ITEMS; r++) {
           const u32 s0 = (u32)__builtin_amdgcn_readlane((int)d_s0, r), b0 = (u32)__builtin_amdgcn_readlane((int)d_b0, r),
                     b1 = (u32)__builtin_amdgcn_readlane((int)d_b1, r), b2 = (u32)__builtin_amdgcn_readlane((int)d_b2, r),
                     b3 = (u32)__builtin_amdgcn_readlane((int)d_b3, r);
@@ -840,19 +890,19 @@
           if (b3 > qlast) {
             const u32 j = (q >= b1 ? 1u : 0u) + (q >= b2 ? 1u : 0u);
             const u32 base = j == 0 ? b0 : (j == 1 ? b1 : b2);
-            off[r] = abl == 1 ? (u64)q : (u64)(s0 + j) * CA + (q - (abl == 2 ? base & ~7u : base));
+            off[r] = (off_t)(abl == 1 ? (u64)q : (u64)(s0 + j) * CA + (q - (abl == 2 ? base & ~7u : base)));
           } else {
             u32 sx = s0;
             while (sx + 1 < ns && pre[sx + 1] <= q) sx++;
-            off[r] = (u64)sx * CA + (q - pre[sx]);
+            off[r] = (off_t)((u64)sx * CA + (q - pre[sx]));
           }
         }
       }
 #pragma unroll
-      for (int r = 0; r < WC_ITEMS; r++) t[r] = HMJ_B_NT ? load_stream(&bucket[off[r]]) : bucket[off[r]];
+      for (int r = 0; r < ITEMS; r++) t[r] = HMJ_B_NT ? load_stream(&bucket[off[r]]) : bucket[off[r]];
     };
     u32 u_s0 = 0, u_b0 = 0, u_b1 = 0, u_b2 = 0, u_b3 = 0, u_b4 = 0;
-    const u32 wq = (u32)__builtin_amdgcn_readfirstlane(w) * (WC_ITEMS * 64);
+    const u32 wq = (u32)__builtin_amdgcn_readfirstlane(w) * (ITEMS * 64);
     u32 win_lo = 0;
     u32 win_v = pre[(u32)lane < ns ? (u32)lane : ns];
     auto plan2 = [&](u32 tile_begin) {
@@ -891,45 +941,45 @@
       u_b4 = (u32)__builtin_amdgcn_readlane((int)win_v, (int)j + 4);
     };
     auto issue2 = [&](u32 tile_begin) {
-      u64 off[WC_ITEMS];
+      off_t off[ITEMS];
       const u32 wq0 = tile_begin + wq;
-      u32 wlast = wq0 + WC_ITEMS * 64 - 1;
+      u32 wlast = wq0 + ITEMS * 64 - 1;
       wlast = wlast < total ? wlast : total - 1;
       if (abl == 4) {
 #pragma unroll
-        for (int r = 0; r < WC_ITEMS; r++) {
+        for (int r = 0; r < ITEMS; r++) {
           u32 q = wq0 + lane + r * 64;
           off[r] = q < total ? q : total - 1;
         }
       } else if (u_b1 > wlast) {
-        const u64 o0 = (u64)u_s0 * CA;
-#pragma unroll
-        for (int r = 0; r < WC_ITEMS; r++) {
+        const off_t o0 = (off_t)((u64)u_s0 * CA);
+#pragma unroll
+        for (int r = 0; r < ITEMS; r++) {
           u32 q = wq0 + lane + r * 64;
           q = q < total ? q : total - 1;
           off[r] = o0 + (q - u_b0);
         }
       } else if (u_b4 > wlast) {
 #pragma unroll
-        for (int r = 0; r < WC_ITEMS; r++) {
+        for (int r = 0; r < ITEMS; r++) {
           u32 q = wq0 + lane + r * 64;
           q = q < total ? q : total - 1;
           const u32 j = (q >= u_b1 ? 1u : 0u) + (q >= u_b2 ? 1u : 0u) + (q >= u_b3 ? 1u : 0u);
           const u32 base = j == 0 ? u_b0 : (j == 1 ? u_b1 : (j == 2 ? u_b2 : u_b3));
-          off[r] = (u64)(u_s0 + j) * CA + (q - base);
+          off[r] = (off_t)((u64)(u_s0 + j) * CA + (q - base));
         }
       } else {
 #pragma unroll
-        for (int r = 0; r < WC_ITEMS; r++) {
+        for (int r = 0; r < ITEMS; r++) {
           u32 q = wq0 + lane + r * 64;
           q = q < total ? q : total - 1;
           u32 sx = u_s0;
           while (sx + 1 < ns && pre[sx + 1] <= q) sx++;
-          off[r] = (u64)sx * CA + (q - pre[sx]);
+          off[r] = (off_t)((u64)sx * CA + (q - pre[sx]));
         }
       }
 #pragma unroll
-      for (int r = 0; r < WC_ITEMS; r++) t[r] = HMJ_B_NT ? load_stream(&bucket[off[r]]) : bucket[off[r]];
+      for (int r = 0; r < ITEMS; r++) t[r] = HMJ_B_NT ? load_stream(&bucket[off[r]]) : bucket[off[r]];
     };
     auto plan = [&](u32 tb) {
       if constexpr (ADDR == 2) plan2(tb); else plan1(tb);
@@ -952,9 +1002,10 @@
         }
       };
 #ifdef HMJ_DEV
+      if constexpr (std::is_same<Row, Tup>::value)
       if (abl == 1 || abl == 4) {
 #pragma unroll
-        for (int r = 0; r < WC_ITEMS; r++)
+        for (int r = 0; r < ITEMS; r++)
           if (t[r].key == 0) t[r].key = (u64)(tile + (u32)tid + r * THREADS + blockIdx.x * 7919u + 1) * 0x9E3779B97F4A7C15ull;
       }
 #endif
@@ -969,16 +1020,16 @@
       const u32 tn = (total - tile_begin < (u32)TILE) ? total - tile_begin : (u32)TILE;
       while (seg + 1 < ns && pre[seg + 1] <= tile_begin) seg++;
       u32 s = seg;
-      u64 off[WC_ITEMS];
-#pragma unroll
-      for (int r = 0; r < WC_ITEMS; r++) {
+      off_t off[ITEMS];
+#pragma unroll
+      for (int r = 0; r < ITEMS; r++) {
         u32 q = wbase + r * 64;
         q = tile_begin + (q < tn ? q : tn - 1);
         while (s + 1 < ns && pre[s + 1] <= q) s++;
-        off[r] = (u64)s * CA + (q - pre[s]);
-      }
-#pragma unroll
-      for (int r = 0; r < WC_ITEMS; r++) t[r] = HMJ_B_NT ? load_stream(&bucket[off[r]]) : bucket[off[r]];
+        off[r] = (off_t)((u64)s * CA + (q - pre[s]));
+      }
+#pragma unroll
+      for (int r = 0; r < ITEMS; r++) t[r] = HMJ_B_NT ? load_stream(&bucket[off[r]]) : bucket[off[r]];
     };
     load(0);
     for (u32 tile = 0; tile < total; tile += TILE) {
@@ -1121,11 +1172,97 @@
 }
 
 template <int THREADS, int MAXD, bool HI>
+__device__ __forceinline__ void slab_a_keys_body(const Tup* __restrict__ in, u32 n, int shift, int bits, u32 rows_per_worker,
+                                                 u64* __restrict__ slab, u32 CA, u32 WA, u32* __restrict__ cnt_out,
+                                                 u64* __restrict__ accum, u32 worker_base) {
+  typedef WcSmem<THREADS, MAXD, u64> Smem;
+  constexpr int TILE = Smem::TILE, ITEMS = Smem::ITEMS;
+  extern __shared__ __attribute__((aligned(16))) unsigned char smem_raw[];
+  Smem& sm = *reinterpret_cast<Smem*>(smem_raw);
+  const u32 D = 1u << bits, mask = D - 1;
+  const int tid = threadIdx.x, lane = tid & 63, w = tid >> 6;
+  const u32 worker = worker_base + blockIdx.x;
+  const auto limit = [=](u32 d) { return (d * WA + worker) * CA + CA; };
+  if ((u32)tid < D) {
+    sm.cflush[tid] = ((u32)tid * WA + worker) * CA;
+    sm.pend[tid] = 0;
+  }
+  wc_clear(sm);
+  __syncthreads();
+  const u64 begin = (u64)worker * rows_per_worker;
+  u64 end = begin + rows_per_worker;
+  if (end > n) end = n;
+  const u32 wbase = (u32)w * (ITEMS * 64) + lane;
+  bool ovf = false;
+  u64 vsum = 0;
+#ifdef HMJ_STAMPS
+  WcStamps stamps = {};
+#endif
+  if (begin < end) {
+    Tup t[ITEMS];
+    u64 key[ITEMS];
+    {
+      const u32 tn = (u32)((end - begin < TILE) ? end - begin : TILE);
+#pragma unroll
+      for (int r = 0; r < ITEMS; r++) {
+        const u32 q = wbase + r * 64;
+        t[r] = load_stream(&in[begin + (q < tn ? q : tn - 1)]);
+      }
+    }
+    for (u64 tile = begin; tile < end; tile += TILE) {
+      const u32 tile_n = (u32)((end - tile < TILE) ? end - tile : TILE);
+      auto prefetch = [&]() {
+        if (tile + TILE < end) {
+          const u64 nt = tile + TILE;
+          const u32 tn = (u32)((end - nt < TILE) ? end - nt : TILE);
+          const Tup* src = in + nt;
+#pragma unroll
+          for (int r = 0; r < ITEMS; r++) {
+            const u32 q = wbase + r * 64;
+            t[r] = load_stream(&src[q < tn ? q : tn - 1]);
+          }
+        }
+      };
+      const bool full = HMJ_WC_FULLTILE && tile_n == (u32)TILE;
+#pragma unroll
+      for (int r = 0; r < ITEMS; r++) {
+        key[r] = t[r].key;
+        if (full || wbase + r * 64 < tile_n) vsum += t[r].val;
+      }
+      if (full)
+        wc_tile<THREADS, MAXD, HI, true, true>(sm, key, tile_n, slab, shift, mask, D, prefetch, limit, &ovf WC_STAMP_PASS);
+      else
+        wc_tile<THREADS, MAXD, HI, false, true>(sm, key, tile_n, slab, shift, mask, D, prefetch, limit, &ovf WC_STAMP_PASS);
+    }
+    wc_flush_carry(sm, slab, D);
+  }
+  if ((u32)tid < D) cnt_out[(u32)tid * WA + worker] = sm.cflush[tid] + sm.pend[tid] - ((u32)tid * WA + worker) * CA;
+  if (ovf) atomicOr(&accum[ACC_ERR], ERR_SLAB);
+#ifdef HMJ_STAMPS
+  stamps.flush();
+#endif
+  u64* wsum = reinterpret_cast<u64*>(&sm.stage[0]);
+  const u64 ws = wave_sum_u64(vsum);
+  lds_barrier();
+  if (lane == 0) wsum[w] = ws;
+  lds_barrier();
+  if (tid == 0) {
+    u64 tot = 0;
+    for (int k = 0; k < Smem::WAVES; k++) tot += wsum[k];
+    if (tot) atomicAdd(reinterpret_cast<unsigned long long*>(&accum[ACC_SUM_P]), (unsigned long long)tot);
+  }
+}
+
+template <int THREADS, int MAXD, bool HI, typename Row = Tup>
 __global__ __launch_bounds__(THREADS, (THREADS * (MAXD <= 256 ? 2 : 1)) / 256) void radix_slab_a_kernel(
-    const Tup* __restrict__ in, u32 n, int shift, int bits, u32 rows_per_worker, Tup* __restrict__ slab,
+    const Tup* __restrict__ in, u32 n, int shift, int bits, u32 rows_per_worker, Row* __restrict__ slab,
     u32 CA, u32 WA, u32* __restrict__ cnt_out, u64* __restrict__ accum, u32 worker_base) {
-  NoXform xf;
-  slab_a_body<THREADS, MAXD, HI, NoXform>(in, n, shift, bits, rows_per_worker, slab, CA, WA, cnt_out, accum, worker_base, xf);
+  if constexpr (std::is_same<Row, Tup>::value) {
+    NoXform xf;
+    slab_a_body<THREADS, MAXD, HI, NoXform>(in, n, shift, bits, rows_per_worker, slab, CA, WA, cnt_out, accum, worker_base, xf);
+  } else {
+    slab_a_keys_body<THREADS, MAXD, HI>(in, n, shift, bits, rows_per_worker, slab, CA, WA, cnt_out, accum, worker_base);
+  }
 }
 
 template <bool CUT>
@@ -1359,6 +1496,51 @@
   if (bits > 8) return hi ? HMJ_SLAB_B(1024, 512, true) : HMJ_SLAB_B(1024, 512, false);
   return hi ? HMJ_SLAB_B(512, 256, true) : HMJ_SLAB_B(512, 256, false);
 #undef HMJ_SLAB_B
+}
+
+hipError_t launch_slab_a_keys(const void* in, u32 n, int shift, int bits, const SlabGeom& g, void* slab_a, u64 slab_a_bytes,
+                              u32* cnt_a, u64 cnt_a_n, u64* accum, hipStream_t st) {
+  if (bits < 1 || bits > 8 || g.WA == 0 || g.CA == 0 || (g.CA & 15u) || (u64)g.WA * g.rpw < n) return hipErrorInvalidValue;
+  if (slab_a_bytes / 8 < ((u64)g.WA << bits) * g.CA || cnt_a_n < ((u64)g.WA << bits)) return hipErrorInvalidValue;
+  if (((u64)g.WA << bits) * g.CA >= 0xFFFFFFF0ull) return hipErrorInvalidValue;
+  if ((reinterpret_cast<uintptr_t>(slab_a) & 127u) != 0) return hipErrorInvalidValue;
+  typedef WcSmem<512, 256, u64> Smem;
+  static_assert(sizeof(Smem) <= 80 * 1024, "narrow slab pass A: two workgroups per CU");
+#define HMJ_SLAB_AK(H)                                                                                                              \
+  {                                                                                                                                 \
+    static SmemAttrOnce once;                                                                                                       \
+    if (hipError_t e = ensure_max_smem(once, reinterpret_cast<const void*>(radix_slab_a_kernel<512, 256, H, u64>), sizeof(Smem)); e != hipSuccess) \
+      return e;                                                                                                                     \
+    hipLaunchKernelGGL((radix_slab_a_kernel<512, 256, H, u64>), dim3(g.WA), dim3(512), sizeof(Smem), st, static_cast<const Tup*>(in), n, shift, \
+                       bits, g.rpw, static_cast<u64*>(slab_a), g.CA, g.WA, cnt_a, accum, 0u);                                       \
+  }
+  if (shift >= 32) HMJ_SLAB_AK(true) else HMJ_SLAB_AK(false)
+#undef HMJ_SLAB_AK
+  return hipGetLastError();
+}
+
+hipError_t launch_slab_b_keys(const void* slab_a, const u32* cnt_a, int bits_a, int shift, int bits, const SlabGeom& g, void* slab_b,
+                              u64 slab_b_bytes, u32* cnt_b, u64 cnt_b_n, u64* accum, hipStream_t st) {
+  if (bits < 1 || bits > 8 || bits_a < 1 || bits_a > 8 || g.KB == 0 || g.WA < g.KB || (g.WA + g.KB - 1) / g.KB > (u32)SLAB_MAXSEG ||
+      (g.CA & 15u) || (g.CB & 15u) || g.CB == 0)
+    return hipErrorInvalidValue;
+  const u64 pieces = ((u64)g.KB << (bits_a + bits));
+  if (slab_b_bytes / 8 < pieces * g.CB || cnt_b_n < pieces || pieces * g.CB >= 0xFFFFFFF0ull) return hipErrorInvalidValue;
+  if ((reinterpret_cast<uintptr_t>(slab_a) & 127u) != 0 || (reinterpret_cast<uintptr_t>(slab_b) & 127u) != 0) return hipErrorInvalidValue;
+  typedef WcSmem<512, 256, u64, SLAB_B_ITEMS<u64>::value> Smem;
+  const size_t smem = sizeof(Smem) + (SLAB_MAXSEG + 1) * sizeof(u32);
+  static_assert(sizeof(Smem) + (SLAB_MAXSEG + 1) * sizeof(u32) <= 80 * 1024, "narrow slab pass B: two workgroups per CU");
+#define HMJ_SLAB_BK(H)                                                                                                              \
+  {                                                                                                                                 \
+    static SmemAttrOnce once;                                                                                                       \
+    if (hipError_t e = ensure_max_smem(once, reinterpret_cast<const void*>(radix_slab_b_kernel<512, 256, H, HMJ_B_ADDR, u64>), smem); e != hipSuccess) \
+      return e;                                                                                                                     \
+    hipLaunchKernelGGL((radix_slab_b_kernel<512, 256, H, HMJ_B_ADDR, u64>), dim3((1u << bits_a) * g.KB), dim3(512), smem, st,       \
+                       static_cast<const u64*>(slab_a), cnt_a, g.CA, g.WA, bits_a, shift, bits, static_cast<u64*>(slab_b), g.CB, cnt_b, accum, g.KB); \
+  }
+  if (shift >= 32) HMJ_SLAB_BK(true) else HMJ_SLAB_BK(false)
+#undef HMJ_SLAB_BK
+  return hipGetLastError();
 }
 
 __global__ __launch_bounds__(256) void key_exact_kernel(const Tup* __restrict__ R, u32 nb, const Tup* __restrict__ S, u32 np,
diff --git a/include/hmj.h b/include/hmj.h
--- a/include/hmj.h
+++ b/include/hmj.h
@@ -91,6 +91,7 @@
 #define HMJ_PATH_ORDERED_EXPANSION 0x400000u
 #define HMJ_PATH_LDS_TABLE 0x800000u
 #define HMJ_PATH_GLOBAL_TABLE 0x100000u
+#define HMJ_PATH_NARROW_PROBE 0x10000000u
 #define HMJ_PATH_HOST_PIPELINE 0x4000u
 
 typedef struct {
@@ -121,6 +122,8 @@
 #define HMJ_REFUSED_SLAB_PROBE_OVERFLOW 0x2000u
 #define HMJ_REFUSED_PREFIX_VIOLATED 0x4000u
 #define HMJ_REFUSED_EXPANSION_GAVE_UP 0x8000u
+#define HMJ_REFUSED_NARROW_PROBE_GAVE_UP 0x10000u
+#define HMJ_REFUSED_NARROW_PROBE_COOLING 0x20000u
 #define HMJ_COOL_UNIQ_WRITE 0x001u
 #define HMJ_COOL_SORTED_WRITE 0x002u
 #define HMJ_COOL_GTABLE 0x004u
@@ -135,6 +138,7 @@
 #define HMJ_COOL_EXACT_PREFIX 0x800u
 #define HMJ_COOL_RANK_RUNS 0x1000u
 #define HMJ_COOL_SORT_MSD 0x2000u
+#define HMJ_COOL_NARROW_PROBE 0x4000u
 
 int hmj_create(hmj_ctx** out, int device_id);
 void hmj_destroy(hmj_ctx* ctx);
```

Result: no change. 34.56 billion, median of 6 (+0.7%).
